# Peilun-Tommy-Li/pHNN-MPC

Measured on AMD Instinct MI355X. Metric: pHNN-MPC rollouts+grads/sec, cartpole H=50 batch=65536, higher is better.
Workload: dtype f32

## Files before the change

### phnn_mpc_amd/csrc/phnn_kernels.hip.h

```cpp
#pragma once
#include <hip/hip_runtime.h>

#include "../../include/phnn_mpc.h"

#define DEV __device__ __forceinline__
#ifdef PHNN_CACHED_TAPE
#define PHNN_NT_STORE(v, p) (*(p) = (v))
#define PHNN_NT_LOAD(p) (*(p))
#else
#define PHNN_NT_STORE(v, p) __builtin_nontemporal_store((v), (p))
#define PHNN_NT_LOAD(p) __builtin_nontemporal_load((p))
#endif

using f32x4 = __attribute__((ext_vector_type(4))) float;
using f32x2 = __attribute__((ext_vector_type(2))) float;

constexpr int kTileB = 16;
#ifndef PHNN_KMAXWAVES
#define PHNN_KMAXWAVES 8
#endif
constexpr int kMaxWaves = PHNN_KMAXWAVES;
constexpr int kScrFloats = 16 * 20;

struct Lane {
// ... 703 lines not shown
  static constexpr int SIZE = oV1T + 4 * LR;
};

constexpr int kRecSmall = 40;
template <int T, int NBIG>
struct WRec {
  static constexpr int VEC = T * 256;
  static constexpr int oSmall = NBIG * VEC;
  static constexpr int SIZE = oSmall + 16 * kRecSmall;
};

#ifdef PHNN_CACHED_RECORDS
#define PHNN_REC_STORE(v, p) (*(p) = (v))
#define PHNN_REC_LOAD(p) (*(p))
#else
#define PHNN_REC_STORE(v, p) __builtin_nontemporal_store((v), (p))
#define PHNN_REC_LOAD(p) __builtin_nontemporal_load((p))
#endif
template <int T>
DEV void store_rec(float* dst, Lane ln, const Act<T>& a) {
#pragma unroll
  for (int t = 0; t < T; ++t) PHNN_REC_STORE(a.v[t], reinterpret_cast<f32x4*>(dst) + t * 64 + ln.lane);
}
template <int T>
DEV void store_rec_scaled(float* dst, Lane ln, const Act<T>& a, float s) {
#pragma unroll
  for (int t = 0; t < T; ++t) PHNN_REC_STORE(a.v[t] * s, reinterpret_cast<f32x4*>(dst) + t * 64 + ln.lane);
}

constexpr int ACT_TANH = 0, ACT_SILU = 2, ACT_RELU = 3, ACT_ELU = 4, ACT_GELU = 5;

DEV float gelu_pdf(float z) { return 0.3989422804014327f * __builtin_amdgcn_exp2f(z * z * -0.7213475204444817f); }
DEV float gelu_cdf(float z) { return __builtin_fmaf(0.5f, erff(z * 0.7071067811865476f), 0.5f); }

template <int ACT>
DEV void act_eval(float z, float& a, float& d1) {
  if (ACT == ACT_RELU) {
    a = fmaxf(z, 0.f);
    d1 = z > 0.f ? 1.0f : 0.0f;
  } else if (ACT == ACT_ELU) {
    a = z > 0.f ? z : expm1f(z);
    d1 = z > 0.f ? 1.0f : __builtin_amdgcn_exp2f(z * 1.4426950408889634f);
  } else if (ACT == ACT_GELU) {
    const float c = gelu_cdf(z);
    a = z * c;
    d1 = __builtin_fmaf(z, gelu_pdf(z), c);
  } else {
    const float s = __builtin_amdgcn_rcpf(1.0f + __builtin_amdgcn_exp2f(z * -1.4426950408889634f));
    a = z * s;
    d1 = __builtin_fmaf(a, 1.0f - s, s);
  }
}
template <int ACT>
DEV float act_d2(float z) {
  if (ACT == ACT_RELU) return 0.0f;
  if (ACT == ACT_ELU) return z > 0.f ? 0.0f : __builtin_amdgcn_exp2f(z * 1.4426950408889634f);
  if (ACT == ACT_GELU) return gelu_pdf(z) * fmaxf(__builtin_fmaf(-z, z, 2.0f), -3.0e38f);
  const float s = __builtin_amdgcn_rcpf(1.0f + __builtin_amdgcn_exp2f(z * -1.4426950408889634f));
  return s * (1.0f - s) * __builtin_fmaf(z, 1.0f - 2.0f * s, 2.0f);
}
template <int ACT, int T>
DEV void act_of(const Act<T>& z, Act<T>& a) {
#pragma unroll
  for (int t = 0; t < T; ++t)
#pragma unroll
    for (int r = 0; r < 4; ++r) {
      float av, d;
      act_eval<ACT>(z.v[t][r], av, d);
      a.v[t][r] = av;
    }
}
template <int ACT, int T>
DEV void mul_d1(Act<T>& g, const Act<T>& z) {
#pragma unroll
  for (int t = 0; t < T; ++t)
#pragma unroll
    for (int r = 0; r < 4; ++r) {
      float a, d;
      act_eval<ACT>(z.v[t][r], a, d);
      g.v[t][r] *= d;
    }
}

template <int HID>
struct HTape {
  Act<HID / 16> a1, a2, q1;
};

template <int HID, bool WANT_H, int ACT>
DEV f32x4 hnet_grad_g(const float* L, Lane ln, f32x4 x, HTape<HID>& tp, float& Hval) {
  using Y = LayH2<HID, MM_F32>;
  constexpr int T = Y::T;
  load_vec<T>(tp.a1, L + Y::oB1, ln);
  in_layer<T>(tp.a1, L + Y::oW1f, ln, sel4(x, ln.q));
  {
    Act<T> a;
    act_of<ACT, T>(tp.a1, a);
    load_vec<T>(tp.a2, L + Y::oB2, ln);
    sq_fwd<T, T>(tp.a2, L + Y::oW2, ln, a);
  }
  Act<T> g;
  float s = 0.f;
  keep_lds_reads_local();
#pragma unroll
  for (int t = 0; t < T; ++t) {
    f32x4 w3 = *reinterpret_cast<const f32x4*>(L + Y::oW3 + 16 * t + 4 * ln.q);
#pragma unroll
    for (int r = 0; r < 4; ++r) {
      float a, d;
      act_eval<ACT>(tp.a2.v[t][r], a, d);
      if (WANT_H) s = __builtin_fmaf(w3[r], a, s);
      g.v[t][r] = w3[r] * d;
    }
  }
  if (WANT_H) Hval = reduce_q(s) + L[Y::oB3];
  zero_act<T>(tp.q1);
  sq_bwd<T, T>(tp.q1, L + Y::oW2, ln, g);
#pragma unroll
  for (int t = 0; t < T; ++t) g.v[t] = tp.q1.v[t];
  mul_d1<ACT, T>(g, tp.a1);
  return to4_rep<T>(L + Y::oW1T, ln, g);
}
template <int HID, int ACT>
DEV void hnet_layer1_g(const float* L, Lane ln, f32x4 x, Act<HID / 16>& z1) {
  using Y = LayH2<HID, MM_F32>;
  load_vec<Y::T>(z1, L + Y::oB1, ln);
  in_layer<Y::T>(z1, L + Y::oW1f, ln, sel4(x, ln.q));
}
template <int HID, int ACT>
DEV f32x4 hnet_hvp_g(const float* L, Lane ln, HTape<HID>& tp, f32x4 v) {
  using Y = LayH2<HID, MM_F32>;
  constexpr int T = Y::T;
  Act<T> ad1, w;
  zero_act<T>(ad1);
  in_layer<T>(ad1, L + Y::oW1f, ln, sel4(v, ln.q));
#pragma unroll
  for (int t = 0; t < T; ++t)
#pragma unroll
    for (int r = 0; r < 4; ++r) {
      const float z = tp.a1.v[t][r], zd = ad1.v[t][r];
      float a, d;
      act_eval<ACT>(z, a, d);
      tp.q1.v[t][r] = tp.q1.v[t][r] * (act_d2<ACT>(z) * zd);
      ad1.v[t][r] = d * zd;
    }
  zero_act<T>(w);
  sq_fwd<T, T>(w, L + Y::oW2, ln, ad1);
  keep_lds_reads_local();
#pragma unroll
  for (int t = 0; t < T; ++t) {
    f32x4 w3 = *reinterpret_cast<const f32x4*>(L + Y::oW3 + 16 * t + 4 * ln.q);
#pragma unroll
    for (int r = 0; r < 4; ++r) w.v[t][r] = w3[r] * (act_d2<ACT>(tp.a2.v[t][r]) * w.v[t][r]);
  }
  Act<T> qd;
  zero_act<T>(qd);
  sq_bwd<T, T>(qd, L + Y::oW2, ln, w);
  mul_d1<ACT, T>(qd, tp.a1);
#pragma unroll
  for (int t = 0; t < T; ++t) qd.v[t] = qd.v[t] + tp.q1.v[t];
  return to4_rep<T>(L + Y::oW1T, ln, qd);
}

template <int HID, bool WANT_H, int MM = MM_F32, int SITE = kInHFwd, int ACT = ACT_TANH>
DEV f32x4 hnet_grad(const float* L, Lane ln, f32x4 z, HTape<HID>& tp, float& Hval) {
  if constexpr (ACT != ACT_TANH) {
    static_assert(MM == MM_F32, "SiLU / ReLU run on the all-f32 kernels");
    return hnet_grad_g<HID, WANT_H, ACT>(L, ln, z, tp, Hval);
  }
  using Y = LayH2<HID, MM>;
  constexpr int T = Y::T;
  load_vec<T>(tp.a1, L + Y::oB1, ln);
  in_layer_mm<T, MM, SITE>(tp.a1, L, Y::oW1f, Y::oW1h, ln, z);
  tanh_act_pre<T>(tp.a1);
  load_vec<T>(tp.a2, L + Y::oB2, ln);
  if (MM == MM_BF16X3) {
    Split3<T> sp;
    split_act<T>(tp.a1, sp);
    sq_fwd_bf<T>(tp.a2, L + Y::oW2, ln, sp);
  } else if (MM == MM_F16X2) {
    Split2<T> sp;
    split_act_h<T>(tp.a1, sp);
    sq_fwd_h<T>(tp.a2, L + Y::oW2, ln, sp);
  } else {
    sq_fwd<T, T>(tp.a2, L + Y::oW2, ln, tp.a1);
  }
  if (MM == MM_F16X2 || kPreScaled<T>) {
    const float c = L[Y::oB3 + 1];
    if (kPreScaled<T> && c == 1.0f) {
      tanh_act_pre<T>(tp.a2);
    } else {
#pragma unroll
      for (int t = 0; t < T; ++t)
#pragma unroll
        for (int r = 0; r < 4; ++r) tp.a2.v[t][r] = tanh_scaled(tp.a2.v[t][r], c);
    }
  } else {
    tanh_act<T>(tp.a2);
  }
  Act<T> g;
  float s = 0.f;
  keep_lds_reads_local();
#pragma unroll
  for (int t = 0; t < T; ++t) {
    if (WANT_H) {
      f32x4 w3 = *reinterpret_cast<const f32x4*>(L + Y::oW3 + 16 * t + 4 * ln.q);
#pragma unroll
      for (int r = 0; r < 4; ++r) s = __builtin_fmaf(w3[r], tp.a2.v[t][r], s);
    }
    f32x4 w3b = *reinterpret_cast<const f32x4*>(L + Y::oW3B + 16 * t + 4 * ln.q);
    g.v[t] = w3b * dtanh(tp.a2.v[t]);
  }
  if (WANT_H) Hval = reduce_q(s) + L[Y::oB3];
  zero_act<T>(tp.q1);
  if (MM == MM_BF16X3) {
    Split3<T> sp;
    split_act<T>(g, sp);
    sq_bwd_bf<T>(tp.q1, L + Y::oW2, ln, sp);
  } else if (MM == MM_F16X2) {
    Split2<T> sp;
    split_act_h<T>(g, sp);
    sq_bwd_h<T>(tp.q1, L + Y::oW2, ln, sp);
  } else {
    sq_bwd<T, T>(tp.q1, L + Y::oW2, ln, g);
  }
#pragma unroll
  for (int t = 0; t < T; ++t) g.v[t] = tp.q1.v[t] * dtanh(tp.a1.v[t]);
  return to4_rep<T>(L + Y::oW1T, ln, g);
}

template <int HID, int MM, int ACT = ACT_TANH>
DEV void hnet_layer1(const float* L, Lane ln, f32x4 z, Act<HID / 16>& a1) {
  if constexpr (ACT != ACT_TANH) return hnet_layer1_g<HID, ACT>(L, ln, z, a1);
  using Y = LayH2<HID, MM>;
  load_vec<Y::T>(a1, L + Y::oB1, ln);
  in_layer_mm<Y::T, MM, kInHRecomp>(a1, L, Y::oW1f, Y::oW1h, ln, z);
  tanh_act_pre<Y::T>(a1);
}

template <int HID, int MM = MM_F32, bool WG = false, int ACT = ACT_TANH, int SITE = kInHHvp>
DEV f32x4 hnet_hvp(const float* L, Lane ln, HTape<HID>& tp, f32x4 v, float* rec = nullptr) {
  if constexpr (ACT != ACT_TANH) {
    static_assert(!WG, "weight-gradient kernels exist for Tanh models only");
    return hnet_hvp_g<HID, ACT>(L, ln, tp, v);
  }
  using Y = LayH2<HID, MM>;
  constexpr int T = Y::T;
  float unscale = 1.0f;
  if (MM == MM_F16X2) {
    float mx = fmaxf(fmaxf(__builtin_fabsf(v[0]), __builtin_fabsf(v[1])), fmaxf(__builtin_fabsf(v[2]), __builtin_fabsf(v[3])));
    int e = 0;
    (void)__builtin_frexpf(mx, &e);
    e = (mx > 0.f && mx < 3.0e38f) ? e : 0;
    v = v * __builtin_ldexpf(1.0f, -e);
    unscale = __builtin_ldexpf(1.0f, e);
  }
  Act<T> ad1, w;
  zero_act<T>(ad1);
  in_layer_mm<T, MM, SITE>(ad1, L, Y::oW1f, Y::oW1h, ln, v);
#pragma unroll
  for (int t = 0; t < T; ++t) ad1.v[t] = dtanh(tp.a1.v[t]) * ad1.v[t];
#pragma unroll
  for (int t = 0; t < T; ++t) tp.q1.v[t] = tp.q1.v[t] * (tp.a1.v[t] * ad1.v[t]);
  zero_act<T>(w);
  if (MM == MM_BF16X3) {
    Split3<T> sp;
    split_act<T>(ad1, sp);
    sq_fwd_bf<T>(w, L + Y::oW2, ln, sp);
  } else if (MM == MM_F16X2) {
    Split2<T> sp;
    split_act_h<T>(ad1, sp);
    sq_fwd_h<T>(w, L + Y::oW2, ln, sp);
  } else {
    sq_fwd<T, T>(w, L + Y::oW2, ln, ad1);
  }
  keep_lds_reads_local();
#pragma unroll
  for (int t = 0; t < T; ++t) {
    f32x4 w3 = *reinterpret_cast<const f32x4*>(L + Y::oW3S + 16 * t + 4 * ln.q);
    f32x4 a2 = tp.a2.v[t];
    f32x4 ad2 = dtanh(a2) * w.v[t];
    if (WG) PHNN_REC_STORE(ad2 * unscale, reinterpret_cast<f32x4*>(rec + 2 * T * 256) + t * 64 + ln.lane);
    w.v[t] = w3 * (a2 * ad2);
  }
  Act<T> qd;
  zero_act<T>(qd);
  if (MM == MM_BF16X3) {
    Split3<T> sp;
    split_act<T>(w, sp);
    sq_bwd_bf<T>(qd, L + Y::oW2, ln, sp);
  } else if (MM == MM_F16X2) {
    Split2<T> sp;
    split_act_h<T>(w, sp);
    sq_bwd_h<T>(qd, L + Y::oW2, ln, sp);
  } else {
    sq_bwd<T, T>(qd, L + Y::oW2, ln, w);
  }
  if (WG) store_rec_scaled<T>(rec + 3 * T * 256, ln, qd, unscale);
#pragma unroll
  for (int t = 0; t < T; ++t) {
    qd.v[t] = __builtin_elementwise_fma(qd.v[t], dtanh(tp.a1.v[t]), tp.q1.v[t]);
  }
  f32x4 Hv = to4_rep<T>(L + Y::oW1T, ln, qd);
  return Hv * (-2.0f * unscale * L[Y::oB3 + 2]);
}

template <int HID, int MM>
DEV f32x4 h1_out_hf(const float* L, Lane ln, const Split2<HID / 16>& sp) {
  using Y = LayH1<HID, MM>;
  constexpr int T = Y::T;
  keep_lds_reads_local();
  const char* base = reinterpret_cast<const char*>(L + Y::oV2) + ln.i * (Y::RS * 2) + ln.q * 16;
  f32x4 o0 = splat4(0.f), o1 = splat4(0.f), o2 = splat4(0.f);
#pragma unroll
  for (int s = 0; s < T / 2; ++s) {
    f16x8 ah = *reinterpret_cast<const f16x8*>(base + s * 64);
    f16x8 al = *reinterpret_cast<const f16x8*>(base + Y::FPART + s * 64);
    o0 = mfma_h(al, sp.h[s], o0);
    o1 = mfma_h(ah, sp.l[s], o1);
    o2 = mfma_h(ah, sp.h[s], o2);
  }
  const float inv = L[Y::oSc];
  f32x4 c2 = *reinterpret_cast<const f32x4*>(L + Y::oC2 + 4 * ln.q);
  return ((o0 + o1) + o2) * inv + c2;
}

template <int HID, int MM>
DEV void h1_bwd_operands(const float* L, Lane ln, const float (&obar)[16], f16x8& b1, f16x8& b2, float& unscale) {
  using Y = LayH1<HID, MM>;
  float mx = 0.f;
#pragma unroll
  for (int k = 0; k < 16; ++k) mx = fmaxf(mx, __builtin_fabsf(obar[k]));
  int e = 0;
  (void)__builtin_frexpf(mx, &e);
  e = (mx > 0.f && mx < 3.0e38f) ? e : 0;
  const float sc = __builtin_ldexpf(1.0f, -e);
  unscale = __builtin_ldexpf(1.0f, e) * L[Y::oSc];
  const bool second = (ln.q & 1) != 0, lo_half = ln.q >= 2;
  u32x4 B1, B2;
#pragma unroll
  for (int p = 0; p < 4; ++p) {
    f32x2 v = {(second ? obar[8 + 2 * p] : obar[2 * p]) * sc, (second ? obar[9 + 2 * p] : obar[2 * p + 1]) * sc};
    f16x2 hb2 = __builtin_convertvector(v, f16x2);
    f32x2 r = residual_h(hb2, v);
    unsigned hbits = __builtin_bit_cast(unsigned, hb2), lbits = __builtin_bit_cast(unsigned, __builtin_convertvector(r, f16x2));
    B1[p] = lo_half ? lbits : hbits;
    B2[p] = lo_half ? 0u : hbits;
  }
  b1 = __builtin_bit_cast(f16x8, B1);
  b2 = __builtin_bit_cast(f16x8, B2);
}

DEV void store_rf(float* dst, Lane ln, f32x4 o) {
  if (ln.w == 0) PHNN_NT_STORE(o, reinterpret_cast<f32x4*>(dst) + ln.i * 4 + ln.q);
}
DEV void load_rf(const float* src, Lane ln, float (&rf)[16]) {
  const f32x4* p = reinterpret_cast<const f32x4*>(src) + ln.i * 4;
#pragma unroll
  for (int k = 0; k < 4; ++k) {
    f32x4 v = PHNN_NT_LOAD(p + k);
#pragma unroll
    for (int e = 0; e < 4; ++e) rf[4 * k + e] = v[e];
  }
}
template <int HID, int MM = MM_F32, int SITE = kInHNet1, int ACT = ACT_TANH>
DEV void h1_hidden(const float* L, Lane ln, f32x4 x, Act<HID / 16>& h) {
  using Y = LayH1<HID, MM>;
  constexpr int T = Y::T;
  load_vec<T>(h, L + Y::oC1, ln);
  in_layer_mm<T, MM, SITE>(h, L, Y::oV1f, Y::oV1h, ln, x);
  if constexpr (ACT == ACT_TANH) tanh_act_pre<T>(h);
}

template <int HID, int MM = MM_F32, int SITE = kInHNet1, int ACT = ACT_TANH>
DEV void h1_fwd(const float* L, float* scr, Lane ln, f32x4 x, Act<HID / 16>& h, float (&out)[16], float* rf_stash = nullptr) {
  using Y = LayH1<HID, MM>;
  constexpr int T = Y::T;
  load_vec<T>(h, L + Y::oC1, ln);
  in_layer_mm<T, MM, SITE>(h, L, Y::oV1f, Y::oV1h, ln, x);
  if constexpr (ACT != ACT_TANH) {
    static_assert(MM == MM_F32, "SiLU / ReLU run on the all-f32 kernels");
    Act<T> a;
    act_of<ACT, T>(h, a);
    Act<1> og;
    og.v[0] = *reinterpret_cast<const f32x4*>(L + Y::oC2 + 4 * ln.q);
    sq_fwd<1, T>(og, L + Y::oV2, ln, a);
// ... 15 lines not shown
  gather16(scr, ln, o.v[0], out);
}

template <int HID, int MM = MM_F32, bool WG = false, int ACT = ACT_TANH>
DEV f32x4 h1_bwd(const float* L, Lane ln, const Act<HID / 16>& h, const float (&obar)[16], float* rec = nullptr) {
  using Y = LayH1<HID, MM>;
  constexpr int T = Y::T;
  Act<T> hb;
  if constexpr (ACT != ACT_TANH) {
    static_assert(MM == MM_F32 && !WG, "SiLU / ReLU: all-f32 kernels, no weight-gradient records");
    Act<1> ob;
#pragma unroll
    for (int r = 0; r < 4; ++r)
      ob.v[0][r] = ln.q == 0 ? obar[r] : (ln.q == 1 ? obar[4 + r] : (ln.q == 2 ? obar[8 + r] : obar[12 + r]));
    zero_act<T>(hb);
    sq_bwd<T, 1>(hb, L + Y::oV2, ln, ob);
    mul_d1<ACT, T>(hb, h);
    return to4_rep<T>(L + Y::oV1T, ln, hb);
  }
  float unscale = 1.0f;
  if (Y::HF) {
    f16x8 b1, b2;
    h1_bwd_operands<HID, MM>(L, ln, obar, b1, b2, unscale);
    keep_lds_reads_local();
    const char* base = reinterpret_cast<const char*>(L + Y::oV2T) + ln.i * 32 + (ln.q & 1) * 16;
#pragma unroll
    for (int nt = 0; nt < T; ++nt) {
      f16x8 ah = *reinterpret_cast<const f16x8*>(base + nt * 512);
      f16x8 al = *reinterpret_cast<const f16x8*>(base + Y::BPART + nt * 512);
      hb.v[nt] = mfma_h(ah, b1, mfma_h(al, b2, splat4(0.f)));
    }
  } else {
    Act<1> ob;
#pragma unroll
    for (int r = 0; r < 4; ++r)
      ob.v[0][r] = ln.q == 0 ? obar[r] : (ln.q == 1 ? obar[4 + r] : (ln.q == 2 ? obar[8 + r] : obar[12 + r]));
    zero_act<T>(hb);
    sq_bwd<T, 1>(hb, L + Y::oV2, ln, ob);
  }
#pragma unroll
  for (int t = 0; t < T; ++t) hb.v[t] = hb.v[t] * dtanh(h.v[t]);
  if (WG) store_rec_scaled<T>(rec, ln, hb, Y::HF ? unscale : 1.0f);
  f32x4 xb = to4_rep<T>(L + Y::oV1T, ln, hb);
  return Y::HF ? xb * unscale : xb;
}

template <int N>
DEV void sym_from_rf(const float (&rf)[16], float (&S)[N][N]) {
#pragma unroll
  for (int i = 0; i < N; ++i) {
    S[i][i] = rf[i * N + i];
#pragma unroll
    for (int j = i + 1; j < N; ++j) S[i][j] = S[j][i] = (rf[i * N + j] + rf[j * N + i]) * 0.5f;
  }
}
template <int N>
DEV void rbar_from(f32x4 lam, f32x4 dH, const float (&Stl)[N], const float (&StdH)[N], float (&rbar)[16]) {
  float m[N][N];
#pragma unroll
  for (int k = 0; k < 16; ++k) rbar[k] = 0.f;
#pragma unroll
  for (int i = 0; i < N; ++i)
#pragma unroll
    for (int j = 0; j < N; ++j) m[i][j] = __builtin_fmaf(lam[i], StdH[j], dH[i] * Stl[j]);
#pragma unroll
  for (int i = 0; i < N; ++i) {
    rbar[i * N + i] = -m[i][i];
#pragma unroll
    for (int j = i + 1; j < N; ++j) rbar[i * N + j] = rbar[j * N + i] = (m[i][j] + m[j][i]) * -0.5f;
  }
}

template <int N_, int HID_, bool FIXG_, int MM_ = MM_F32, int MI_ = 1, int ACT_ = ACT_TANH>
struct PhnnModel {
  static constexpr int N = N_, HID = HID_, T = HID / 16, MM = MM_, MI = MI_, ACT = ACT_;
  static constexpr bool FIXG = FIXG_, SPLIT = false;
  static_assert(N_ * MI_ <= 16 && MI_ <= 4, "G_net output n*m <= 16, m <= 4");
  static constexpr int SCR = kScrFloats;
  static constexpr int oH = 0;
  static constexpr int oR = oH + LayH2<HID, MM>::SIZE;
  static constexpr int oGn = oR + LayH1<HID, MM>::SIZE;
  static constexpr int oJ = oGn + (FIXG ? 0 : LayH1<HID, MM>::SIZE);
  static constexpr int oG = oJ + 16;
  static constexpr int IMG = oG + 16;

  static constexpr int oStashRf = 2 * T * 256 + 64;
  static constexpr int STASH = oStashRf + 256;

  template <bool WANT_H, bool ST = false>
  DEV static f32x4 f(const float* L, float* scr, Lane ln, f32x4 x, f32x4 u, float& Hval, float* stash = nullptr) {
    keep_lds_reads_local();
    HTape<HID> tp;
    f32x4 dH = hnet_grad<HID, WANT_H, MM, kInHFwd, ACT>(L + oH, ln, x, tp, Hval);
    if (ST) {
      store_act<T>(stash, ln, tp.a2);
      store_act<T>(stash + T * 256, ln, tp.q1);
      if (ln.q == 0) PHNN_NT_STORE(dH, reinterpret_cast<f32x4*>(stash + 2 * T * 256) + ln.i);
    }
    Act<T> hR;
    float rf[16];
    h1_fwd<HID, MM, kInHNet1, ACT>(L + oR, scr, ln, x, hR, rf, ST ? stash + oStashRf : nullptr);
    float G[N * MI];
    if (FIXG) {
#pragma unroll
      for (int i = 0; i < N * MI; ++i) G[i] = L[oG + i];
    } else {
      Act<T> hG;
      float gf[16];
      h1_fwd<HID, MM, kInHNet1, ACT>(L + oGn, scr, ln, x, hG, gf);
#pragma unroll
      for (int i = 0; i < N * MI; ++i) G[i] = gf[i];
    }
    return combine(L, rf, dH, G, u);
  }

  DEV static f32x4 combine(const float* L, const float (&rf)[16], f32x4 dH, const float (&G)[N * MI], f32x4 u) {
    float S[N][N], StdH[N];
    sym_from_rf<N>(rf, S);
#pragma unroll
    for (int k = 0; k < N; ++k) {
      float a = 0.f;
#pragma unroll
      for (int i = 0; i < N; ++i) a = __builtin_fmaf(S[i][k], dH[i], a);
      StdH[k] = a;
    }
    f32x4 dx = splat4(0.f);
#pragma unroll
    for (int i = 0; i < N; ++i) {
      float acc = 0.f;
#pragma unroll
      for (int j = 0; j < N; ++j) acc = __builtin_fmaf(L[oJ + i * N + j], dH[j], acc);
#pragma unroll
      for (int k = 0; k < N; ++k) acc = __builtin_fmaf(-S[i][k], StdH[k], acc);
      if (MI == 1) {
        dx[i] = __builtin_fmaf(G[i], u[0], acc);
      } else {
        float gu = 0.f;
#pragma unroll
        for (int k = 0; k < MI; ++k) gu = __builtin_fmaf(G[i * MI + k], u[k], gu);
        dx[i] = acc + gu;
      }
    }
    return dx;
  }

  static constexpr bool RECHB = !LayH1<HID, MM>::HF;
  static constexpr int NBIG = 4 + (RECHB ? (FIXG ? 1 : 2) : 0);
  using Rec = WRec<T, NBIG>;

  template <bool ST = false, bool WG = false, int INH = -1>
  DEV static void vjp(const float* L, float* scr, Lane ln, f32x4 x, f32x4 u, f32x4 lam, f32x4& xbar, f32x4& ubar,
                      const float* stash = nullptr, float* rec = nullptr, float Hbar = 0.f) {
    keep_lds_reads_local();
    HTape<HID> tp;
    float Hdummy;
    f32x4 dH;
    float rf[16];
    if (ST) {
      dH = PHNN_NT_LOAD(reinterpret_cast<const f32x4*>(stash + 2 * T * 256) + ln.i);
      load_rf(stash + oStashRf, ln, rf);
      load_act<T>(stash, ln, tp.a2);
      load_act<T>(stash + T * 256, ln, tp.q1);
    } else {
      dH = hnet_grad<HID, false, MM, INH & kInHRecomp, ACT>(L + oH, ln, x, tp, Hdummy);
    }
    if (WG && !ST) {
      store_rec<T>(rec, ln, tp.a2);
      store_rec<T>(rec + Rec::VEC, ln, tp.q1);
    }
    f32x4 xb = splat4(0.f);
    float S[N][N], Stl[N], StdH[N];
    {
      Act<T> hR;
      if (ST) {
        h1_hidden<HID, MM, INH & kInHNet1Adj, ACT>(L + oR, ln, x, hR);
      } else {
        h1_fwd<HID, MM, INH & kInHNet1Adj, ACT>(L + oR, scr, ln, x, hR, rf);
      }
      sym_from_rf<N>(rf, S);
#pragma unroll
      for (int k = 0; k < N; ++k) {
        float a = 0.f, c = 0.f;
#pragma unroll
        for (int i = 0; i < N; ++i) {
          a = __builtin_fmaf(S[i][k], lam[i], a);
          c = __builtin_fmaf(S[i][k], dH[i], c);
        }
        Stl[k] = a;
        StdH[k] = c;
      }
      float rbar[16];
      rbar_from<N>(lam, dH, Stl, StdH, rbar);
      xb += h1_bwd<HID, MM, WG && RECHB, ACT>(L + oR, ln, hR, rbar, WG && RECHB ? rec + 4 * Rec::VEC : nullptr);
      if (WG && ln.q == 0) {
        f32x4* sm = reinterpret_cast<f32x4*>(rec + Rec::oSmall + ln.i * kRecSmall);
#pragma unroll
        for (int k = 0; k < 4; ++k) sm[4 + k] = f32x4{rbar[4 * k], rbar[4 * k + 1], rbar[4 * k + 2], rbar[4 * k + 3]};
      }
    }
    ubar = splat4(0.f);
    if (FIXG) {
#pragma unroll
      for (int k = 0; k < MI; ++k)
#pragma unroll
        for (int i = 0; i < N; ++i) ubar[k] = __builtin_fmaf(L[oG + i * MI + k], lam[i], ubar[k]);
    } else {
      Act<T> hG;
      float gf[16], gbar[16];
      h1_fwd<HID, MM, INH & kInHNet1Adj, ACT>(L + oGn, scr, ln, x, hG, gf);
#pragma unroll
      for (int k = 0; k < 16; ++k) gbar[k] = 0.f;
#pragma unroll
      for (int i = 0; i < N; ++i)
#pragma unroll
        for (int k = 0; k < MI; ++k) {
          ubar[k] = __builtin_fmaf(gf[i * MI + k], lam[i], ubar[k]);
          gbar[i * MI + k] = lam[i] * u[k];
        }
      xb += h1_bwd<HID, MM, WG && RECHB, ACT>(L + oGn, ln, hG, gbar, WG && RECHB ? rec + 5 * Rec::VEC : nullptr);
    }
    f32x4 v = splat4(0.f);
#pragma unroll
    for (int j = 0; j < N; ++j) {
      float acc = 0.f;
#pragma unroll
      for (int i = 0; i < N; ++i) acc = __builtin_fmaf(L[oJ + i * N + j], lam[i], acc);
#pragma unroll
      for (int k = 0; k < N; ++k) acc = __builtin_fmaf(-S[j][k], Stl[k], acc);
      v[j] = acc;
    }
    if (WG && ln.q == 0) {
      f32x4* sm = reinterpret_cast<f32x4*>(rec + Rec::oSmall + ln.i * kRecSmall);
      sm[0] = x;
      sm[1] = v;
      sm[2] = lam;
      sm[3] = dH;
      sm[8] = u;
      sm[9] = f32x4{Hbar, 0.f, 0.f, 0.f};
    }
    if (ST) hnet_layer1<HID, MM, ACT>(L + oH, ln, x, tp.a1);
    xbar = xb + hnet_hvp<HID, MM, WG, ACT, INH & kInHHvp>(L + oH, ln, tp, v, rec);
    if (WG) xbar = xbar + Hbar * dH;
  }
};

struct LayM {
  static constexpr int HID = 64, T = 4, LD = HID + 4, LR = HID + 8;
  static constexpr int oW1f = 0;
  static constexpr int oB1 = oW1f + T * 64;
  static constexpr int oW2 = oB1 + HID;
  static constexpr int oB2 = oW2 + HID * LD;
  static constexpr int oWo = oB2 + HID;
  static constexpr int oBo = oWo + 4 * LR;
  static constexpr int oWoTf = oBo + 4;
  static constexpr int oW1T = oWoTf + T * 64;
  static constexpr int SIZE = oW1T + 4 * LR;
};

struct MTape {
  Act<4> a1, a2;
  f32x4 o;
};

DEV void mnet_fwd(const float* L, Lane ln, f32x4 q, MTape& tp) {
  using Y = LayM;
  keep_lds_reads_local();
  load_vec<4>(tp.a1, L + Y::oB1, ln);
  in_layer<4>(tp.a1, L + Y::oW1f, ln, sel4(q, ln.q));
  tanh_act<4>(tp.a1);
  load_vec<4>(tp.a2, L + Y::oB2, ln);
  sq_fwd<4, 4>(tp.a2, L + Y::oW2, ln, tp.a1);
  tanh_act<4>(tp.a2);
  tp.o = to4_rep<4>(L + Y::oWo, ln, tp.a2) + *reinterpret_cast<const f32x4*>(L + Y::oBo);
}

DEV f32x4 mnet_bwd(const float* L, Lane ln, const MTape& tp, f32x4 ob) {
  using Y = LayM;
  keep_lds_reads_local();
  Act<4> d, e;
  zero_act<4>(d);
  in_layer<4>(d, L + Y::oWoTf, ln, sel4(ob, ln.q));
#pragma unroll
  for (int t = 0; t < 4; ++t) d.v[t] = d.v[t] * dtanh(tp.a2.v[t]);
  zero_act<4>(e);
  sq_bwd<4, 4>(e, L + Y::oW2, ln, d);
#pragma unroll
  for (int t = 0; t < 4; ++t) e.v[t] = e.v[t] * dtanh(tp.a1.v[t]);
  return to4_rep<4>(L + Y::oW1T, ln, e);
}

DEV float softplus_dev(float x) { return x > 20.f ? x : log1pf(expf(x)); }
DEV float sigmoid_sp_dev(float x) { return x > 20.f ? 1.0f : 1.0f / (1.0f + expf(-x)); }

constexpr int MASS_CARTPOLE = 0, MASS_CONSTANT = 1, MASS_DIAGONAL = 2, MASS_FULL = 3;

template <int MT>
DEV void mass_from_outputs(f32x4 o, float (&m)[3], float (&w)[3]) {
  if (MT == MASS_DIAGONAL) {
    m[0] = expf(o[0]) + 1e-3f;
    m[2] = expf(o[1]) + 1e-3f;
    m[1] = 0.f;
    w[0] = 1.0f / m[0];
    w[2] = 1.0f / m[2];
    w[1] = 0.f;
  } else {
    const float l00 = softplus_dev(o[0]) + 1e-3f, l10 = o[1], l11 = softplus_dev(o[2]) + 1e-3f;
    m[0] = l00 * l00;
    m[1] = l00 * l10;
    m[2] = l10 * l10 + l11 * l11;
    const float det = m[0] * m[2] - m[1] * m[1];
    w[0] = m[2] / det;
    w[1] = -m[1] / det;
    w[2] = m[0] / det;
  }
}

template <int MT>
DEV f32x4 mass_outputs_bar(f32x4 o, const float (&Mb)[4]) {
  if (MT == MASS_DIAGONAL) return f32x4{Mb[0] * expf(o[0]), Mb[3] * expf(o[1]), 0.f, 0.f};
  const float l00 = softplus_dev(o[0]) + 1e-3f, l10 = o[1], l11 = softplus_dev(o[2]) + 1e-3f;
  const float s00 = 2.0f * Mb[0], s01 = Mb[1] + Mb[2], s11 = 2.0f * Mb[3];
  return f32x4{(s00 * l00 + s01 * l10) * sigmoid_sp_dev(o[0]), s01 * l00 + s11 * l10, (s11 * l11) * sigmoid_sp_dev(o[2]), 0.f};
}

template <int HID_, int MM_ = MM_F32, int MI_ = 1, int MT_ = MASS_CARTPOLE, int ACT_ = ACT_TANH>
struct CanonModel {
  static constexpr int N = 4, HID = HID_, T = HID / 16, MM = MM_, MI = MI_, MT = MT_, ACT = ACT_;
  static constexpr bool SPLIT = false;
  static constexpr int SCR = 0;
  static constexpr int oH = 0;
  static constexpr int oC = oH + LayH2<HID, MM>::SIZE;
  static constexpr int oCG = oC + 12;
  static constexpr int oCW = oC + 28;
  static constexpr int oMn = oC + 32;
  static constexpr int IMG = oMn + (MT_ >= MASS_DIAGONAL ? LayM::SIZE : 0);

  DEV static void mass_eval(const float* L, Lane ln, f32x4 y, float (&m)[3], float (&w)[3], MTape& mt) {
    if (MT == MASS_CONSTANT) {
      m[0] = L[oC + 0]; m[1] = L[oC + 1]; m[2] = L[oC + 2];
      w[0] = L[oCW + 0]; w[1] = L[oCW + 1]; w[2] = L[oCW + 2];
    } else {
      mnet_fwd(L + oMn, ln, f32x4{y[0], y[1], 0.f, 0.f}, mt);
      mass_from_outputs<MT>(mt.o, m, w);
    }
  }

  DEV static float Base_Gu(const float* L, int row, f32x4 u) {
    float s = 0.f;
#pragma unroll
    for (int k = 0; k < MI; ++k) s = __builtin_fmaf(L[oCG + row * MI + k], u[k], s);
    return s;
  }
  DEV static f32x4 Base_Gt(const float* L, float dpb0, float dpb1) {
    f32x4 ub = splat4(0.f);
#pragma unroll
    for (int k = 0; k < MI; ++k) ub[k] = L[oCG + 2 * MI + k] * dpb0 + L[oCG + 3 * MI + k] * dpb1;
    return ub;
  }

  static constexpr int STASH = 2 * T * 256 + 64;

  template <bool WANT_H, bool ST = false>
  DEV static f32x4 f(const float* L, float* scr, Lane ln, f32x4 y, f32x4 u, float& Hval, float* stash = nullptr) {
    keep_lds_reads_local();
    if constexpr (MT != MASS_CARTPOLE) {
      float m[3], w[3];
      MTape mt;
      mass_eval(L, ln, y, m, w, mt);
      f32x4 z = {y[0], y[1], m[0] * y[2] + m[1] * y[3], m[1] * y[2] + m[2] * y[3]};
      HTape<HID> tp;
      f32x4 dH = hnet_grad<HID, WANT_H, MM, kInHFwd, ACT>(L + oH, ln, z, tp, Hval);
      if (ST) {
        store_act<T>(stash, ln, tp.a2);
        store_act<T>(stash + T * 256, ln, tp.q1);
        if (ln.q == 0) PHNN_NT_STORE(dH, reinterpret_cast<f32x4*>(stash + 2 * T * 256) + ln.i);
      }
      float dp0 = (-dH[0] - L[oC + 6] * dH[2]) + Base_Gu(L, 2, u);
      float dp1 = (-dH[1] - L[oC + 7] * dH[3]) + Base_Gu(L, 3, u);
      return f32x4{w[0] * z[2] + w[1] * z[3], w[1] * z[2] + w[2] * z[3], w[0] * dp0 + w[1] * dp1, w[1] * dp0 + w[2] * dp1};
    }
    float a = L[oC + 0], b = L[oC + 1], c = L[oC + 2];
    float sn, cs;
    sincos_dev(y[1], sn, cs);
    float bc = b * cs;
    f32x4 z = {y[0], y[1], a * y[2] + bc * y[3], bc * y[2] + c * y[3]};
    HTape<HID> tp;
    f32x4 dH = hnet_grad<HID, WANT_H, MM, kInHFwd, ACT>(L + oH, ln, z, tp, Hval);
    if (ST) {
      store_act<T>(stash, ln, tp.a2);
      store_act<T>(stash + T * 256, ln, tp.q1);
      if (ln.q == 0) PHNN_NT_STORE(dH, reinterpret_cast<f32x4*>(stash + 2 * T * 256) + ln.i);
    }
    float dp0 = (-dH[0] - L[oC + 6] * dH[2]) + Base_Gu(L, 2, u);
    float dp1 = (-dH[1] - L[oC + 7] * dH[3]) + Base_Gu(L, 3, u);
    float det = (a * c - bc * bc) + 1e-6f;
    float mi00 = c / det, mi01 = -bc / det, mi11 = a / det;
    return f32x4{mi00 * z[2] + mi01 * z[3], mi01 * z[2] + mi11 * z[3], mi00 * dp0 + mi01 * dp1,
                 mi01 * dp0 + mi11 * dp1};
  }

  static constexpr int NBIG = 4;
  using Rec = WRec<T, NBIG>;

  template <bool ST = false, bool WG = false, int INH = -1>
  DEV static void vjp(const float* L, float* scr, Lane ln, f32x4 y, f32x4 u, f32x4 lam, f32x4& ybar, f32x4& ubar,
                      const float* stash = nullptr, float* rec = nullptr, float Hbar = 0.f) {
    keep_lds_reads_local();
    if constexpr (MT != MASS_CARTPOLE) {
      float m[3], w[3];
      MTape mt;
      mass_eval(L, ln, y, m, w, mt);
      f32x4 z = {y[0], y[1], m[0] * y[2] + m[1] * y[3], m[1] * y[2] + m[2] * y[3]};
      HTape<HID> tp;
      float Hdummy;
      f32x4 dH;
      if (ST) {
        dH = PHNN_NT_LOAD(reinterpret_cast<const f32x4*>(stash + 2 * T * 256) + ln.i);
        load_act<T>(stash, ln, tp.a2);
        load_act<T>(stash + T * 256, ln, tp.q1);
        hnet_layer1<HID, MM, ACT>(L + oH, ln, z, tp.a1);
      } else {
        dH = hnet_grad<HID, false, MM, INH & kInHRecomp, ACT>(L + oH, ln, z, tp, Hdummy);
      }
      const float Rd2 = L[oC + 6], Rd3 = L[oC + 7];
      const float dp0 = (-dH[0] - Rd2 * dH[2]) + Base_Gu(L, 2, u);
      const float dp1 = (-dH[1] - Rd3 * dH[3]) + Base_Gu(L, 3, u);
      const float pb0 = lam[0] * w[0] + lam[1] * w[1], pb1 = lam[0] * w[1] + lam[1] * w[2];
      const float dpb0 = lam[2] * w[0] + lam[3] * w[1], dpb1 = lam[2] * w[1] + lam[3] * w[2];
      f32x4 v = {-dpb0, -dpb1, -Rd2 * dpb0, -Rd3 * dpb1};
      ubar = Base_Gt(L, dpb0, dpb1);
      if (WG) {
        if (!ST) {
          store_rec<T>(rec, ln, tp.a2);
          store_rec<T>(rec + Rec::VEC, ln, tp.q1);
        }
        if (ln.q == 0) {
          f32x4* sm = reinterpret_cast<f32x4*>(rec + Rec::oSmall + ln.i * kRecSmall);
          sm[0] = z;
          sm[1] = v;
          sm[2] = lam;
          sm[3] = dH;
          sm[4] = f32x4{0.f, 0.f, -dpb0 * dH[2], -dpb1 * dH[3]};
          sm[8] = u;
          sm[9] = f32x4{Hbar, 0.f, 0.f, 0.f};
        }
      }
      f32x4 zb = hnet_hvp<HID, MM, WG, ACT, INH & kInHHvp>(L + oH, ln, tp, v, rec);
      if (WG) zb = zb + Hbar * dH;
      zb[2] += pb0;
      zb[3] += pb1;
      ybar = f32x4{zb[0], zb[1], zb[2] * m[0] + zb[3] * m[1], zb[2] * m[1] + zb[3] * m[2]};
      if (MT >= MASS_DIAGONAL || WG) {
        const float W4[4] = {w[0], w[1], w[1], w[2]};
        const float Wb[4] = {lam[0] * z[2] + lam[2] * dp0, lam[0] * z[3] + lam[2] * dp1,
                             lam[1] * z[2] + lam[3] * dp0, lam[1] * z[3] + lam[3] * dp1};
        float Tm[4], Um[4], Mb[4];
        Tm[0] = W4[0] * Wb[0] + W4[1] * Wb[2]; Tm[1] = W4[0] * Wb[1] + W4[1] * Wb[3];
        Tm[2] = W4[2] * Wb[0] + W4[3] * Wb[2]; Tm[3] = W4[2] * Wb[1] + W4[3] * Wb[3];
        Um[0] = Tm[0] * W4[0] + Tm[1] * W4[2]; Um[1] = Tm[0] * W4[1] + Tm[1] * W4[3];
        Um[2] = Tm[2] * W4[0] + Tm[3] * W4[2]; Um[3] = Tm[2] * W4[1] + Tm[3] * W4[3];
        Mb[0] = zb[2] * y[2] - Um[0];
        Mb[1] = zb[2] * y[3] - Um[1];
        Mb[2] = zb[3] * y[2] - Um[2];
        Mb[3] = zb[3] * y[3] - Um[3];
        if (WG && ln.q == 0) {
          f32x4* sm = reinterpret_cast<f32x4*>(rec + Rec::oSmall + ln.i * kRecSmall);
          sm[5] = f32x4{Mb[0], Mb[1], Mb[2], Mb[3]};
          sm[6] = f32x4{y[0], y[1], 0.f, 0.f};
        }
        if (MT >= MASS_DIAGONAL) {
          f32x4 qb = mnet_bwd(L + oMn, ln, mt, mass_outputs_bar<MT>(mt.o, Mb));
          ybar[0] += qb[0];
          ybar[1] += qb[1];
        }
      }
      return;
    }
    float a = L[oC + 0], b = L[oC + 1], c = L[oC + 2];
    float sn, cs;
    sincos_dev(y[1], sn, cs);
    float bc = b * cs;
    f32x4 z = {y[0], y[1], a * y[2] + bc * y[3], bc * y[2] + c * y[3]};
    HTape<HID> tp;
    float Hdummy;
    f32x4 dH;
    if (ST) {
      dH = PHNN_NT_LOAD(reinterpret_cast<const f32x4*>(stash + 2 * T * 256) + ln.i);
      load_act<T>(stash, ln, tp.a2);
      load_act<T>(stash + T * 256, ln, tp.q1);
      hnet_layer1<HID, MM, ACT>(L + oH, ln, z, tp.a1);
    } else {
      dH = hnet_grad<HID, false, MM, INH & kInHRecomp, ACT>(L + oH, ln, z, tp, Hdummy);
    }
    float Rd2 = L[oC + 6], Rd3 = L[oC + 7];
    float dp0 = (-dH[0] - Rd2 * dH[2]) + Base_Gu(L, 2, u);
    float dp1 = (-dH[1] - Rd3 * dH[3]) + Base_Gu(L, 3, u);
    float det = (a * c - bc * bc) + 1e-6f;
    float rdet = 1.0f / det;
    float mi00 = c * rdet, mi01 = -bc * rdet, mi11 = a * rdet;
    float pb0 = lam[0] * mi00 + lam[1] * mi01, pb1 = lam[0] * mi01 + lam[1] * mi11;
    float dpb0 = lam[2] * mi00 + lam[3] * mi01, dpb1 = lam[2] * mi01 + lam[3] * mi11;
    float mb00 = lam[0] * z[2] + lam[2] * dp0;
    float mb01 = lam[0] * z[3] + lam[1] * z[2] + lam[2] * dp1 + lam[3] * dp0;
    float mb11 = lam[1] * z[3] + lam[3] * dp1;
    f32x4 v = {-dpb0, -dpb1, -Rd2 * dpb0, -Rd3 * dpb1};
    ubar = Base_Gt(L, dpb0, dpb1);
    if (WG) {
      if (!ST) {
        store_rec<T>(rec, ln, tp.a2);
        store_rec<T>(rec + Rec::VEC, ln, tp.q1);
      }
      if (ln.q == 0) {
        f32x4* sm = reinterpret_cast<f32x4*>(rec + Rec::oSmall + ln.i * kRecSmall);
        sm[0] = z;
        sm[1] = v;
        sm[2] = lam;
        sm[3] = dH;
        sm[4] = f32x4{0.f, 0.f, -dpb0 * dH[2], -dpb1 * dH[3]};
        sm[8] = u;
        sm[9] = f32x4{Hbar, 0.f, 0.f, 0.f};
      }
    }
    f32x4 zb = hnet_hvp<HID, MM, WG, ACT, INH & kInHHvp>(L + oH, ln, tp, v, rec);
    if (WG) zb = zb + Hbar * dH;
    zb[2] += pb0;
    zb[3] += pb1;
    float bcb = zb[2] * y[3] + zb[3] * y[2];
    float detb = (-(mb00 * c + mb11 * a) + mb01 * bc) * (rdet * rdet);
    bcb += -mb01 * rdet;
    bcb += -2.0f * bc * detb;
    ybar = f32x4{zb[0], zb[1] + bcb * (-b * sn), zb[2] * a + zb[3] * bc, zb[2] * bc + zb[3] * c};
  }
};

constexpr int kXR0 = 0, kXR1 = 2048, kXR2 = 4096, kXP0 = 6144, kXP1 = 7168, kXchFloats = 8192;
using ActW = Act<2>;

DEV void xch_put(float* region, Lane ln, const Split2<2>& sp) {
  f16x8* p = reinterpret_cast<f16x8*>(region);
  p[ln.w * 64 + ln.lane] = sp.h[0];
  p[(4 + ln.w) * 64 + ln.lane] = sp.l[0];
}
DEV void xch_get(const float* region, Lane ln, Split2<8>& o) {
  const f16x8* p = reinterpret_cast<const f16x8*>(region);
#pragma unroll
  for (int s = 0; s < 4; ++s) {
    o.h[s] = p[s * 64 + ln.lane];
    o.l[s] = p[(4 + s) * 64 + ln.lane];
  }
}
DEV void xch_put_partial(float* set, Lane ln, f32x4 v) { reinterpret_cast<f32x4*>(set)[ln.w * 64 + ln.lane] = v; }
DEV f32x4 xch_sum_partials(const float* set, Lane ln) {
  const f32x4* p = reinterpret_cast<const f32x4*>(set) + ln.lane;
  return to4_kslots(((p[0] + p[64]) + p[128]) + p[192]);
}

DEV void tanh_pre_w(ActW& a) {
#pragma unroll
  for (int t = 0; t < 2; ++t)
#pragma unroll
    for (int r = 0; r < 4; ++r) a.v[t][r] = __builtin_fmaf(-2.0f, __builtin_amdgcn_rcpf(__builtin_amdgcn_exp2f(a.v[t][r]) + 1.0f), 1.0f);
}

DEV void sq_fwd_h_w(ActW& o, const float* Wimg, Lane ln, const Split2<8>& in) {
  using I = HfImg<128>;
  keep_lds_reads_local();
  matrix_phase_begin();
  const char* base = reinterpret_cast<const char*>(Wimg) + ln.i * (I::RS * 2) + ln.q * 16 + (2 * ln.w) * 16 * (I::RS * 2);
#pragma unroll
  for (int s = 0; s < 4; ++s) {
    f16x8 a[2][2];
#pragma unroll
    for (int g = 0; g < 2; ++g)
#pragma unroll
      for (int p = 0; p < 2; ++p) a[g][p] = *reinterpret_cast<const f16x8*>(base + p * I::PART + g * 16 * (I::RS * 2) + s * 64);
    mfma3x2(o.v[0], o.v[1], a, in.h[s], in.l[s]);
  }
  matrix_phase_end();
}

DEV void sq_bwd_h_w(ActW& o, const float* Wimg, Lane ln, const Split2<8>& in) {
  using I = HfImg<128>;
  keep_lds_reads_local();
  matrix_phase_begin();
  typedef fp16x4_t __attribute__((address_space(3))) * lds_h4;
  typedef char __attribute__((address_space(3))) * lds_cp;
  const int a4 = (ln.lane & 15) >> 2, pp = ln.lane & 3;
  lds_cp base = (lds_cp) const_cast<char*>(reinterpret_cast<const char*>(Wimg)) + (4 * ln.q + a4) * (I::RS * 2) + 16 * pp + 64 * ln.w;
#pragma unroll
  for (int s = 0; s < 4; ++s) {
    f16x8 a[2][2];
#pragma unroll
    for (int g = 0; g < 2; ++g)
#pragma unroll
      for (int p = 0; p < 2; ++p) {
        lds_cp off = base + p * I::PART + 32 * s * (I::RS * 2) + 8 * g;
        f16x4 lo = __builtin_bit_cast(f16x4, __builtin_amdgcn_ds_read_tr16_b64_v4f16((lds_h4)off));
        f16x4 hi = __builtin_bit_cast(f16x4, __builtin_amdgcn_ds_read_tr16_b64_v4f16((lds_h4)(off + 16 * (I::RS * 2))));
        a[g][p] = __builtin_shufflevector(lo, hi, 0, 1, 2, 3, 4, 5, 6, 7);
      }
    mfma3x2(o.v[0], o.v[1], a, in.h[s], in.l[s]);
  }
  matrix_phase_end();
}

struct HTapeW {
  ActW a1, a2, q1;
};

template <int SITE = kInHFwd, class PreBarrier>
DEV f32x4 hnet_grad_w(const float* L, Lane ln, f32x4 z, HTapeW& tp, PreBarrier pre_barrier) {
  using Y = LayH2<128, MM_F16X2>;
  const int t0 = 2 * ln.w;
  load_vec<2>(tp.a1, L + Y::oB1 + 16 * t0, ln);
  in_layer_mm<2, MM_F16X2, SITE>(tp.a1, L, Y::oW1f, Y::oW1h, ln, z, t0);
  tanh_pre_w(tp.a1);
  {
    Split2<2> sp;
    split_act_h<2>(tp.a1, sp);
    xch_put(ln.xch + kXR0, ln, sp);
  }
  pre_barrier();
  __syncthreads();
  {
    Split2<8> all;
    xch_get(ln.xch + kXR0, ln, all);
    load_vec<2>(tp.a2, L + Y::oB2 + 16 * t0, ln);
    sq_fwd_h_w(tp.a2, L + Y::oW2, ln, all);
  }
  const float c = L[Y::oB3 + 1];
  if (c == 1.0f) {
    tanh_pre_w(tp.a2);
  } else {
#pragma unroll
    for (int t = 0; t < 2; ++t)
#pragma unroll
      for (int r = 0; r < 4; ++r) tp.a2.v[t][r] = tanh_scaled(tp.a2.v[t][r], c);
  }
  ActW g;
  keep_lds_reads_local();
#pragma unroll
  for (int t = 0; t < 2; ++t) {
    f32x4 w3b = *reinterpret_cast<const f32x4*>(L + Y::oW3B + 16 * (t0 + t) + 4 * ln.q);
    g.v[t] = w3b * dtanh(tp.a2.v[t]);
  }
  {
    Split2<2> sp;
    split_act_h<2>(g, sp);
    xch_put(ln.xch + kXR1, ln, sp);
  }
  __syncthreads();
  {
    Split2<8> all;
    xch_get(ln.xch + kXR1, ln, all);
    zero_act<2>(tp.q1);
    sq_bwd_h_w(tp.q1, L + Y::oW2, ln, all);
  }
#pragma unroll
  for (int t = 0; t < 2; ++t) g.v[t] = tp.q1.v[t] * dtanh(tp.a1.v[t]);
  keep_lds_reads_local();
  return to4_group<2>(L + Y::oW1T + (ln.i & 3) * Y::LR + 16 * t0, ln, g.v);
}

DEV f32x4 hnet_hvp_w(const float* L, Lane ln, HTapeW& tp, f32x4 v, float& scale) {
  using Y = LayH2<128, MM_F16X2>;
  const int t0 = 2 * ln.w;
  float mx = fmaxf(fmaxf(__builtin_fabsf(v[0]), __builtin_fabsf(v[1])), fmaxf(__builtin_fabsf(v[2]), __builtin_fabsf(v[3])));
  int e = 0;
  (void)__builtin_frexpf(mx, &e);
  e = (mx > 0.f && mx < 3.0e38f) ? e : 0;
  v = v * __builtin_ldexpf(1.0f, -e);
  const float unscale = __builtin_ldexpf(1.0f, e);
  ActW ad1, w;
  zero_act<2>(ad1);
  in_layer_mm<2, MM_F16X2, kInHHvp>(ad1, L, Y::oW1f, Y::oW1h, ln, v, t0);
#pragma unroll
  for (int t = 0; t < 2; ++t) ad1.v[t] = dtanh(tp.a1.v[t]) * ad1.v[t];
#pragma unroll
  for (int t = 0; t < 2; ++t) tp.q1.v[t] = tp.q1.v[t] * (tp.a1.v[t] * ad1.v[t]);
  {
    Split2<2> sp;
    split_act_h<2>(ad1, sp);
    xch_put(ln.xch + kXR0, ln, sp);
  }
  __syncthreads();
  {
    Split2<8> all;
    xch_get(ln.xch + kXR0, ln, all);
    zero_act<2>(w);
    sq_fwd_h_w(w, L + Y::oW2, ln, all);
  }
  keep_lds_reads_local();
#pragma unroll
  for (int t = 0; t < 2; ++t) {
    f32x4 w3 = *reinterpret_cast<const f32x4*>(L + Y::oW3S + 16 * (t0 + t) + 4 * ln.q);
    f32x4 a2 = tp.a2.v[t];
    f32x4 ad2 = dtanh(a2) * w.v[t];
    w.v[t] = w3 * (a2 * ad2);
  }
  {
    Split2<2> sp;
    split_act_h<2>(w, sp);
    xch_put(ln.xch + kXR1, ln, sp);
  }
  __syncthreads();
  ActW qd;
  {
    Split2<8> all;
    xch_get(ln.xch + kXR1, ln, all);
    zero_act<2>(qd);
    sq_bwd_h_w(qd, L + Y::oW2, ln, all);
  }
#pragma unroll
  for (int t = 0; t < 2; ++t) qd.v[t] = __builtin_elementwise_fma(qd.v[t], dtanh(tp.a1.v[t]), tp.q1.v[t]);
  scale = -2.0f * unscale * L[Y::oB3 + 2];
  keep_lds_reads_local();
  return to4_group<2>(L + Y::oW1T + (ln.i & 3) * Y::LR + 16 * t0, ln, qd.v);
}

template <int N_>
struct PhnnSplit {
  using Base = PhnnModel<N_, 128, true, MM_F16X2>;
  static constexpr int N = N_, HID = 128, T = 8, MM = MM_F16X2;
  static constexpr bool FIXG = true, SPLIT = true;
  static constexpr int SCR = Base::SCR, IMG = Base::IMG, STASH = Base::STASH, MI = 1;
  static constexpr int oH = Base::oH, oR = Base::oR, oJ = Base::oJ, oG = Base::oG;
  using YR = LayH1<128, MM_F16X2>;

  template <int SITE = kInHNet1>
  DEV static void rnet_hidden(const float* L, Lane ln, f32x4 x, ActW& hR) {
    const int t0 = 2 * ln.w;
    load_vec<2>(hR, L + oR + YR::oC1 + 16 * t0, ln);
    in_layer_mm<2, MM_F16X2, SITE>(hR, L + oR, YR::oV1f, YR::oV1h, ln, x, t0);
    tanh_pre_w(hR);
  }
  template <int SITE = kInHNet1>
  DEV static void rnet_layer1(const float* L, Lane ln, f32x4 x, ActW& hR) {
    rnet_hidden<SITE>(L, ln, x, hR);
    Split2<2> sp;
    split_act_h<2>(hR, sp);
    xch_put(ln.xch + kXR2, ln, sp);
  }
  DEV static void rnet_out(const float* L, float* scr, Lane ln, float (&rf)[16], float* rf_stash = nullptr) {
    Split2<8> all;
    xch_get(ln.xch + kXR2, ln, all);
    f32x4 o = h1_out_hf<128, MM_F16X2>(L + oR, ln, all);
    if (rf_stash) store_rf(rf_stash, ln, o);
    gather16(scr, ln, o, rf);
  }

  template <bool WANT_H, bool ST = false>
  DEV static f32x4 f(const float* L, float* scr, Lane ln, f32x4 x, f32x4 u, float& Hval, float* stash = nullptr) {
    static_assert(!WANT_H, "the split-tile kernels are rollout kernels");
    keep_lds_reads_local();
    HTapeW tp;
    ActW hR;
    f32x4 P = hnet_grad_w(L + oH, ln, x, tp, [&]() { rnet_layer1(L, ln, x, hR); });
    xch_put_partial(ln.xch + kXP0, ln, P);
    float rf[16];
    rnet_out(L, scr, ln, rf, ST ? stash + Base::oStashRf : nullptr);
    if (ST) {
      store_act<2>(stash + 2 * ln.w * 256, ln, tp.a2);
      store_act<2>(stash + T * 256 + 2 * ln.w * 256, ln, tp.q1);
    }
    __syncthreads();
    f32x4 dH = xch_sum_partials(ln.xch + kXP0, ln);
    if (ST && ln.q == 0 && ln.w == 0) PHNN_NT_STORE(dH, reinterpret_cast<f32x4*>(stash + 2 * T * 256) + ln.i);
    float G[N];
#pragma unroll
    for (int i = 0; i < N; ++i) G[i] = L[oG + i];
    return Base::combine(L, rf, dH, G, u);
  }

  template <bool ST = false, bool WG = false, int INH = -1>
  DEV static void vjp(const float* L, float* scr, Lane ln, f32x4 x, f32x4 u, f32x4 lam, f32x4& xbar, f32x4& ubar,
                      const float* stash = nullptr, float* rec = nullptr, float Hbar = 0.f) {
    static_assert(!WG, "weight-gradient records come from the whole-tile kernels");
    keep_lds_reads_local();
    const int t0 = 2 * ln.w;
    HTapeW tp;
    ActW hR;
    f32x4 dH;
    float rf[16];
    if (ST) {
      dH = PHNN_NT_LOAD(reinterpret_cast<const f32x4*>(stash + 2 * T * 256) + ln.i);
      load_rf(stash + Base::oStashRf, ln, rf);
      load_act<2>(stash + t0 * 256, ln, tp.a2);
      load_act<2>(stash + T * 256 + t0 * 256, ln, tp.q1);
      using Y = LayH2<128, MM_F16X2>;
      load_vec<2>(tp.a1, L + oH + Y::oB1 + 16 * t0, ln);
      in_layer_mm<2, MM_F16X2, kInHRecomp>(tp.a1, L + oH, Y::oW1f, Y::oW1h, ln, x, t0);
      tanh_pre_w(tp.a1);
      rnet_hidden<kInHNet1Adj>(L, ln, x, hR);
    } else {
      f32x4 P = hnet_grad_w<kInHRecomp>(L + oH, ln, x, tp, [&]() { rnet_layer1<kInHNet1Adj>(L, ln, x, hR); });
      xch_put_partial(ln.xch + kXP0, ln, P);
      rnet_out(L, scr, ln, rf);
      __syncthreads();
      dH = xch_sum_partials(ln.xch + kXP0, ln);
    }
    float S[N][N], Stl[N], StdH[N];
    sym_from_rf<N>(rf, S);
#pragma unroll
    for (int k = 0; k < N; ++k) {
      float a = 0.f, c = 0.f;
#pragma unroll
      for (int i = 0; i < N; ++i) {
        a = __builtin_fmaf(S[i][k], lam[i], a);
        c = __builtin_fmaf(S[i][k], dH[i], c);
      }
      Stl[k] = a;
      StdH[k] = c;
    }
    float rbar[16];
    rbar_from<N>(lam, dH, Stl, StdH, rbar);
    float unscaleR;
    f32x4 PR;
    {
      f16x8 b1, b2;
      h1_bwd_operands<128, MM_F16X2>(L + oR, ln, rbar, b1, b2, unscaleR);
      keep_lds_reads_local();
      const char* base = reinterpret_cast<const char*>(L + oR + YR::oV2T) + ln.i * 32 + (ln.q & 1) * 16;
      ActW hb;
#pragma unroll
      for (int t = 0; t < 2; ++t) {
        f16x8 ah = *reinterpret_cast<const f16x8*>(base + (t0 + t) * 512);
        f16x8 al = *reinterpret_cast<const f16x8*>(base + YR::BPART + (t0 + t) * 512);
        hb.v[t] = mfma_h(ah, b1, mfma_h(al, b2, splat4(0.f)));
      }
#pragma unroll
      for (int t = 0; t < 2; ++t) hb.v[t] = hb.v[t] * dtanh(hR.v[t]);
      keep_lds_reads_local();
      PR = to4_group<2>(L + oR + YR::oV1T + (ln.i & 3) * YR::LR + 16 * t0, ln, hb.v);
    }
    ubar = splat4(0.f);
#pragma unroll
    for (int i = 0; i < N; ++i) ubar[0] = __builtin_fmaf(L[oG + i], lam[i], ubar[0]);
    f32x4 v = splat4(0.f);
#pragma unroll
    for (int j = 0; j < N; ++j) {
      float acc = 0.f;
#pragma unroll
      for (int i = 0; i < N; ++i) acc = __builtin_fmaf(L[oJ + i * N + j], lam[i], acc);
#pragma unroll
      for (int k = 0; k < N; ++k) acc = __builtin_fmaf(-S[j][k], Stl[k], acc);
      v[j] = acc;
    }
    float scaleH;
    f32x4 PH = hnet_hvp_w(L + oH, ln, tp, v, scaleH);
    xch_put_partial(ln.xch + kXP0, ln, PR);
    xch_put_partial(ln.xch + kXP1, ln, PH);
    __syncthreads();
    f32x4 xb = splat4(0.f);
    xb += xch_sum_partials(ln.xch + kXP0, ln) * unscaleR;
    xbar = xb + xch_sum_partials(ln.xch + kXP1, ln) * scaleH;
  }
};

template <int DUMMY = 0>
struct CanonSplit {
  using Base = CanonModel<128, MM_F16X2>;
  static constexpr int N = 4, HID = 128, T = 8, MM = MM_F16X2;
  static constexpr bool SPLIT = true;
  static constexpr int SCR = 0, IMG = Base::IMG, STASH = Base::STASH, oH = Base::oH, oC = Base::oC, MI = 1;
  DEV static float Base_Gu(const float* L, int row, f32x4 u) { return Base::Base_Gu(L, row, u); }
  DEV static f32x4 Base_Gt(const float* L, float dpb0, float dpb1) { return Base::Base_Gt(L, dpb0, dpb1); }

  template <bool WANT_H, bool ST = false>
  DEV static f32x4 f(const float* L, float* scr, Lane ln, f32x4 y, f32x4 u, float& Hval, float* stash = nullptr) {
    static_assert(!WANT_H, "the split-tile kernels are rollout kernels");
    keep_lds_reads_local();
    float a = L[oC + 0], b = L[oC + 1], c = L[oC + 2];
    float sn, cs;
    sincos_dev(y[1], sn, cs);
    float bc = b * cs;
    f32x4 z = {y[0], y[1], a * y[2] + bc * y[3], bc * y[2] + c * y[3]};
    HTapeW tp;
    f32x4 P = hnet_grad_w(L + oH, ln, z, tp, []() {});
    xch_put_partial(ln.xch + kXP0, ln, P);
    if (ST) {
      store_act<2>(stash + 2 * ln.w * 256, ln, tp.a2);
      store_act<2>(stash + T * 256 + 2 * ln.w * 256, ln, tp.q1);
    }
    __syncthreads();
    f32x4 dH = xch_sum_partials(ln.xch + kXP0, ln);
    if (ST && ln.q == 0 && ln.w == 0) PHNN_NT_STORE(dH, reinterpret_cast<f32x4*>(stash + 2 * T * 256) + ln.i);
    float dp0 = (-dH[0] - L[oC + 6] * dH[2]) + Base_Gu(L, 2, u);
    float dp1 = (-dH[1] - L[oC + 7] * dH[3]) + Base_Gu(L, 3, u);
    float det = (a * c - bc * bc) + 1e-6f;
    float mi00 = c / det, mi01 = -bc / det, mi11 = a / det;
    return f32x4{mi00 * z[2] + mi01 * z[3], mi01 * z[2] + mi11 * z[3], mi00 * dp0 + mi01 * dp1,
                 mi01 * dp0 + mi11 * dp1};
  }

  template <bool ST = false, bool WG = false, int INH = -1>
  DEV static void vjp(const float* L, float* scr, Lane ln, f32x4 y, f32x4 u, f32x4 lam, f32x4& ybar, f32x4& ubar,
                      const float* stash = nullptr, float* rec = nullptr, float Hbar = 0.f) {
    static_assert(!WG, "weight-gradient records come from the whole-tile kernels");
    keep_lds_reads_local();
    const int t0 = 2 * ln.w;
    float a = L[oC + 0], b = L[oC + 1], c = L[oC + 2];
    float sn, cs;
    sincos_dev(y[1], sn, cs);
    float bc = b * cs;
    f32x4 z = {y[0], y[1], a * y[2] + bc * y[3], bc * y[2] + c * y[3]};
    HTapeW tp;
    f32x4 dH;
    if (ST) {
      dH = PHNN_NT_LOAD(reinterpret_cast<const f32x4*>(stash + 2 * T * 256) + ln.i);
      load_act<2>(stash + t0 * 256, ln, tp.a2);
      load_act<2>(stash + T * 256 + t0 * 256, ln, tp.q1);
      using Y = LayH2<128, MM_F16X2>;
      load_vec<2>(tp.a1, L + oH + Y::oB1 + 16 * t0, ln);
      in_layer_mm<2, MM_F16X2, kInHRecomp>(tp.a1, L + oH, Y::oW1f, Y::oW1h, ln, z, t0);
      tanh_pre_w(tp.a1);
    } else {
      f32x4 P = hnet_grad_w<kInHRecomp>(L + oH, ln, z, tp, []() {});
      xch_put_partial(ln.xch + kXP0, ln, P);
      __syncthreads();
      dH = xch_sum_partials(ln.xch + kXP0, ln);
    }
    float Rd2 = L[oC + 6], Rd3 = L[oC + 7];
    float dp0 = (-dH[0] - Rd2 * dH[2]) + Base_Gu(L, 2, u);
    float dp1 = (-dH[1] - Rd3 * dH[3]) + Base_Gu(L, 3, u);
    float det = (a * c - bc * bc) + 1e-6f;
    float rdet = 1.0f / det;
    float mi00 = c * rdet, mi01 = -bc * rdet, mi11 = a * rdet;
    float pb0 = lam[0] * mi00 + lam[1] * mi01, pb1 = lam[0] * mi01 + lam[1] * mi11;
    float dpb0 = lam[2] * mi00 + lam[3] * mi01, dpb1 = lam[2] * mi01 + lam[3] * mi11;
    float mb00 = lam[0] * z[2] + lam[2] * dp0;
    float mb01 = lam[0] * z[3] + lam[1] * z[2] + lam[2] * dp1 + lam[3] * dp0;
    float mb11 = lam[1] * z[3] + lam[3] * dp1;
    f32x4 v = {-dpb0, -dpb1, -Rd2 * dpb0, -Rd3 * dpb1};
    ubar = Base_Gt(L, dpb0, dpb1);
    float scaleH;
    f32x4 PH = hnet_hvp_w(L + oH, ln, tp, v, scaleH);
    xch_put_partial(ln.xch + kXP1, ln, PH);
    __syncthreads();
    f32x4 zb = xch_sum_partials(ln.xch + kXP1, ln) * scaleH;
    zb[2] += pb0;
    zb[3] += pb1;
    float bcb = zb[2] * y[3] + zb[3] * y[2];
    float detb = (-(mb00 * c + mb11 * a) + mb01 * bc) * (rdet * rdet);
    bcb += -mb01 * rdet;
    bcb += -2.0f * bc * detb;
    ybar = f32x4{zb[0], zb[1] + bcb * (-b * sn), zb[2] * a + zb[3] * bc, zb[2] * bc + zb[3] * c};
  }
};

template <int N_, int HID_, int MM_ = MM_F32, int ACT_ = ACT_TANH>
struct OdeModel {
  static constexpr int N = N_, HID = HID_, T = HID / 16, LD = HID + 4, LR = HID + 8, MM = MM_, MI = 1, ACT = ACT_;
  static_assert(ACT_ == ACT_TANH || MM_ == MM_F32, "SiLU / ReLU run on the all-f32 kernels");
  static constexpr bool SPLIT = false;
  static constexpr int SCR = 0;
  static constexpr int WF = MM == MM_F16X2 ? HfImg<HID>::FLOATS : HID * LD;
  static constexpr int oW1f = 0;
  static constexpr int oB1 = oW1f + T * 64;
  static constexpr int oW2 = oB1 + HID;
  static constexpr int oB2 = oW2 + WF;
  static constexpr int oW3 = oB2 + HID;
  static constexpr int oB3 = oW3 + WF;
  static constexpr int oW4r = oB3 + HID;
  static constexpr int oB4 = oW4r + 4 * LR;
  static constexpr int oW4f = oB4 + 4;
  static constexpr int oW1T = oW4f + T * 64;
  static constexpr int oSC = oW1T + 4 * LR;
  static constexpr bool WIDE = N + 1 > 4;
  static constexpr int oW1fu = oSC + 4;
  static constexpr int oW1Tu = oW1fu + (WIDE ? T * 64 : 0);
  static constexpr int IMG = oW1Tu + (WIDE ? 4 * LR : 0);
  static_assert(MM != MM_BF16X3, "ODEFunc has an f32 and an f16x2 variant");
  static_assert(N <= 4, "state dimension up to 4");

  struct Tape {
    Act<T> a1, a2, a3;
  };

  DEV static void layer1(const float* L, Lane ln, f32x4 x, float u, Act<T>& a1) {
    f32x4 in = x;
    if (!WIDE) in[N & 3] = u;
    load_vec<T>(a1, L + oB1, ln);
    in_layer<T>(a1, L + oW1f, ln, sel4(in, ln.q));
    if (WIDE) in_layer<T>(a1, L + oW1fu, ln, ln.q == 0 ? u : 0.f);
    if constexpr (ACT == ACT_TANH) tanh_act<T>(a1);
  }

  DEV static void hidden(const float* L, Lane ln, int oW, int oB, float c, const Act<T>& a, Act<T>& o) {
    load_vec<T>(o, L + oB, ln);
    if constexpr (ACT != ACT_TANH) {
      Act<T> act;
      act_of<ACT, T>(a, act);
      sq_fwd<T, T>(o, L + oW, ln, act);
      return;
    }
    if (MM == MM_F16X2) {
      Split2<T> sp;
      split_act_h<T>(a, sp);
      sq_fwd_h<T>(o, L + oW, ln, sp);
#pragma unroll
      for (int t = 0; t < T; ++t)
#pragma unroll
        for (int r = 0; r < 4; ++r) o.v[t][r] = tanh_scaled(o.v[t][r], c);
    } else {
      sq_fwd<T, T>(o, L + oW, ln, a);
      tanh_act<T>(o);
    }
  }

  DEV static void hidden_T(const float* L, Lane ln, int oW, const Act<T>& d, Act<T>& o) {
    zero_act<T>(o);
    if (MM == MM_F16X2) {
      Split2<T> sp;
      split_act_h<T>(d, sp);
      sq_bwd_h<T>(o, L + oW, ln, sp);
    } else {
      sq_bwd<T, T>(o, L + oW, ln, d);
    }
  }

  DEV static f32x4 fwd(const float* L, Lane ln, f32x4 x, float u, Tape& tp) {
    keep_lds_reads_local();
    layer1(L, ln, x, u, tp.a1);
    hidden(L, ln, oW2, oB2, L[oSC + 0], tp.a1, tp.a2);
    hidden(L, ln, oW3, oB3, L[oSC + 1], tp.a2, tp.a3);
    f32x4 b4 = *reinterpret_cast<const f32x4*>(L + oB4);
    if constexpr (ACT != ACT_TANH) {
      Act<T> act;
      act_of<ACT, T>(tp.a3, act);
      return to4_rep<T>(L + oW4r, ln, act) + b4;
    }
    return to4_rep<T>(L + oW4r, ln, tp.a3) + b4;
  }

  static constexpr int VEC24 = ACT == ACT_TANH ? T * 192 : T * 256;
  static constexpr int STASH = 2 * VEC24;

  template <bool WANT_H, bool ST = false>
  DEV static f32x4 f(const float* L, float* scr, Lane ln, f32x4 x, f32x4 uv, float& Hval, float* stash = nullptr) {
    const float u = uv[0];
    Tape tp;
    if (WANT_H) Hval = 0.f;
    f32x4 dx = fwd(L, ln, x, u, tp);
    if (ST) {
      if constexpr (ACT == ACT_TANH) {
        store_act24<T>(stash, ln, tp.a2);
        store_act24<T>(stash + VEC24, ln, tp.a3);
      } else {
        store_act<T>(stash, ln, tp.a2);
        store_act<T>(stash + VEC24, ln, tp.a3);
      }
    }
    return dx;
  }

  template <bool ST = false, bool WG = false, int INH = -1>
  DEV static void vjp(const float* L, float* scr, Lane ln, f32x4 x, f32x4 uv, f32x4 lam, f32x4& xbar, f32x4& ubar4,
                      const float* stash = nullptr, float* rec = nullptr, float Hbar = 0.f) {
    static_assert(!WG, "ODEFunc has no weight-gradient kernels");
    const float u = uv[0];
    float ubar;
    Tape tp;
    if (ST) {
      if constexpr (ACT == ACT_TANH) {
        load_act24<T>(stash + VEC24, ln, tp.a3);
        load_act24<T>(stash, ln, tp.a2);
      } else {
        load_act<T>(stash + VEC24, ln, tp.a3);
        load_act<T>(stash, ln, tp.a2);
      }
      keep_lds_reads_local();
      layer1(L, ln, x, u, tp.a1);
    } else {
      (void)fwd(L, ln, x, u, tp);
    }
    float unscale = 1.0f;
    if (MM == MM_F16X2) {
      float mx = fmaxf(fmaxf(__builtin_fabsf(lam[0]), __builtin_fabsf(lam[1])), fmaxf(__builtin_fabsf(lam[2]), __builtin_fabsf(lam[3])));
      int e = 0;
      (void)__builtin_frexpf(mx, &e);
      e = (mx > 0.f && mx < 3.0e38f) ? e : 0;
      lam = lam * __builtin_ldexpf(1.0f, -e);
      unscale = __builtin_ldexpf(1.0f, e);
    }
    Act<T> d, e;
    zero_act<T>(d);
    in_layer<T>(d, L + oW4f, ln, sel4(lam, ln.q));
    if constexpr (ACT != ACT_TANH) {
      mul_d1<ACT, T>(d, tp.a3);
      hidden_T(L, ln, oW3, d, e);
      mul_d1<ACT, T>(e, tp.a2);
      hidden_T(L, ln, oW2, e, d);
      mul_d1<ACT, T>(d, tp.a1);
    } else {
#pragma unroll
      for (int t = 0; t < T; ++t) d.v[t] = d.v[t] * dtanh(tp.a3.v[t]);
      hidden_T(L, ln, oW3, d, e);
#pragma unroll
      for (int t = 0; t < T; ++t) e.v[t] = e.v[t] * dtanh(tp.a2.v[t]);
      hidden_T(L, ln, oW2, e, d);
#pragma unroll
      for (int t = 0; t < T; ++t) d.v[t] = d.v[t] * dtanh(tp.a1.v[t]);
    }
    f32x4 inb = to4_rep<T>(L + oW1T, ln, d);
    if (MM == MM_F16X2) inb = inb * unscale;
    if (WIDE) {
      ubar = to4_rep<T>(L + oW1Tu, ln, d)[0] * unscale;
    } else {
      ubar = inb[N & 3];
      inb[N & 3] = 0.f;
    }
    xbar = inb;
    ubar4 = f32x4{ubar, 0.f, 0.f, 0.f};
  }
};

DEV void no_speculation() { asm volatile("" ::: "memory"); }

template <int N, class Tgt>
DEV float state_cost(const phnn_cost& c, f32x4 x, const Tgt& tgt) {
  float e[N], cost = 0.f;
#pragma unroll
// ... 69 lines not shown
  const float* dx_bar;
  float* dx_out;
  float* wrec;
  int no_cost;
  long long B;
  int H;
  float dt, half_dt, sixth_dt;
  phnn_cost c;
  float Qs[16];
  const float* x_ref;
  long long ref_bs, ref_ts;
  int ref_rows;
  const int* ref_off_dev;
  int ref_off_host;
};

struct PointParams {
  const float* img;
  const float* x;
  const float* u;
  const float* lam;
  float* dx;
  float* Hout;
  long long B;
  const float* Hbar;
  float* wrec;
};

template <int IMG>
DEV void stage_image(float* lds, const float* img) {
  const f32x4* src = reinterpret_cast<const f32x4*>(img);
  f32x4* dst = reinterpret_cast<f32x4*>(lds);
  for (int k = threadIdx.x; k < IMG / 4; k += blockDim.x) dst[k] = src[k];
  __syncthreads();
}

template <int N>
DEV f32x4 load_state(const float* p) {
  if (N == 4) return *reinterpret_cast<const f32x4*>(p);
  f32x4 x = splat4(0.f);
#pragma unroll
  for (int i = 0; i < N; ++i) x[i] = p[i];
  return x;
}
template <int N>
DEV void store_state(float* p, f32x4 x) {
  if (N == 4) {
    *reinterpret_cast<f32x4*>(p) = x;
  } else {
#pragma unroll
    for (int i = 0; i < N; ++i) p[i] = x[i];
  }
}

DEV float clamp_u(const phnn_cost& c, float u) { return c.has_u_bounds ? fminf(fmaxf(u, c.u_min), c.u_max) : u; }

template <int MI>
DEV f32x4 load_u(const float* up, int t) {
  f32x4 u = splat4(0.f);
#pragma unroll
  for (int k = 0; k < MI; ++k) u[k] = up[t * MI + k];
  return u;
}
template <int MI>
DEV f32x4 clamp_u4(const phnn_cost& c, f32x4 u) {
#pragma unroll
  for (int k = 0; k < MI; ++k) u[k] = clamp_u(c, u[k]);
  return u;
}
template <int MI>
DEV float control_cost(const phnn_cost& c, f32x4 u) {
  if (MI == 1) return (u[0] * c.R[0]) * u[0];
  float cost = 0.f;
#pragma unroll
  for (int j = 0; j < MI; ++j) {
    float s = 0.f;
#pragma unroll
    for (int i = 0; i < MI; ++i) s = __builtin_fmaf(u[i], c.R[i * MI + j], s);
    cost = __builtin_fmaf(s, u[j], cost);
  }
  return cost;
}

template <class M, int INTEG>
struct StashStep {
  static constexpr int SLOT = M::STASH + 64;
  static constexpr int FLOATS = INTEG == PHNN_INTEG_EULER ? M::STASH : 4 * SLOT;
};
DEV void store_stage(float* dst, Lane ln, f32x4 y) {
  if (ln.q == 0 && ln.w == 0) PHNN_NT_STORE(y, reinterpret_cast<f32x4*>(dst) + ln.i);
}
DEV f32x4 load_stage(const float* src, Lane ln) {
  return PHNN_NT_LOAD(reinterpret_cast<const f32x4*>(src) + ln.i);
}

struct TileCtx {
  Lane ln;
  float* scr;
  long long tile, b;
  bool valid, writer;
};
template <class M>
DEV bool tile_ctx(TileCtx& c, float* lds, long long B) {
  const int wave = threadIdx.x >> 6, nwaves = blockDim.x >> 6;
  static_prio(wave);
  c.ln.lane = threadIdx.x & 63;
  c.ln.i = c.ln.lane & 15;
  c.ln.q = c.ln.lane >> 4;
  c.ln.w = M::SPLIT ? wave : 0;
  c.ln.xch = M::SPLIT ? lds + M::IMG + nwaves * M::SCR : nullptr;
  c.scr = lds + M::IMG + wave * M::SCR;
  c.tile = M::SPLIT ? (long long)blockIdx.x : (long long)blockIdx.x * nwaves + wave;
  if (c.tile * kTileB >= B) return false;
  c.b = c.tile * kTileB + c.ln.i;
  c.valid = c.b < B;
  if (!c.valid) c.b = B - 1;
  c.writer = c.valid && c.ln.q == 0 && (!M::SPLIT || wave == 0);
  return true;
}

template <int N>
struct RefRows {
  const float* base;
  long long ts;
  int off, last;
  DEV void init(const RollParams& p, long long b) {
    base = p.x_ref + b * p.ref_bs;
    ts = p.ref_ts;
    last = p.ref_rows - 1;
    const int o = p.ref_off_dev ? *p.ref_off_dev : p.ref_off_host;
    off = o < 0 ? 0 : (o > last ? last : o);
  }
  DEV f32x4 row(int t) const {
    const int r = t < last - off ? off + t : last;
    const float* q = base + r * ts;
    f32x4 v = splat4(0.f);
#pragma unroll
    for (int i = 0; i < N; ++i) v[i] = q[i];
    return v;
  }
};

template <class M, int INTEG, bool STASH, bool REF = false>
DEV void fwd_march(const RollParams& p, const float* L, const TileCtx& tc) {
  constexpr int N = M::N;
  const Lane ln = tc.ln;
  float* scr = tc.scr;
  const long long tile = tc.tile, b = tc.b;
  const bool writer = tc.writer;
  f32x4 x = load_state<N>(p.x0 + b * N);
  if (p.traj && writer) store_state<N>(p.traj + (b * (p.H + 1)) * N, x);
  RefRows<N> rr;
  float cost;
  if constexpr (REF) {
    rr.init(p, b);
    cost = state_cost<N>(p.c, x, rr.row(0));
  } else {
    cost = state_cost<N>(p.c, x, p.c.x_target);
  }
  constexpr int MI = M::MI;
  const float* up = p.u + b * p.H * MI;
  float Hd;
  for (int t = 0; t < p.H; ++t) {
    f32x4 tgt;
    if constexpr (REF) tgt = rr.row(t + 1);
    f32x4 u = clamp_u4<MI>(p.c, load_u<MI>(up, t));
    if (MI == 1) cost = __builtin_fmaf(u[0] * p.c.R[0], u[0], cost);
    else cost += control_cost<MI>(p.c, u);
    float* sl = STASH ? p.stash + (tile * p.H + t) * (long long)StashStep<M, INTEG>::FLOATS : nullptr;
    f32x4 k1 = M::template f<false, STASH>(L, scr, ln, x, u, Hd, sl);
    if (p.dx_out && writer) store_state<N>(p.dx_out + (b * p.H + t) * N, k1);
    if (INTEG == PHNN_INTEG_EULER) {
      x = x + p.dt * k1;
    } else {
      constexpr int SLOT = StashStep<M, INTEG>::SLOT;
      f32x4 acc = k1, kp = k1;
#pragma unroll 1
      for (int s = 1; s < 4; ++s) {
        const f32x4 y = x + (s == 3 ? p.dt : p.half_dt) * kp;
        float* ss = STASH ? sl + s * SLOT : nullptr;
        if (STASH) store_stage(ss + M::STASH, ln, y);
        kp = M::template f<false, STASH>(L, scr, ln, y, u, Hd, ss);
        acc = acc + (s == 3 ? 1.0f : 2.0f) * kp;
      }
      x = x + p.sixth_dt * acc;
    }
    if constexpr (REF) cost += state_cost<N>(p.c, x, tgt);
    else cost += state_cost<N>(p.c, x, p.c.x_target);
    if (p.traj && writer) store_state<N>(p.traj + (b * (p.H + 1) + t + 1) * N, x);
  }
  if (writer && p.cost) p.cost[b] = cost;
}

template <class M, int INTEG, bool STASH, bool REF = false>
__global__ __launch_bounds__(64 * kMaxWaves) void k_rollout_fwd(RollParams p) {
  extern __shared__ __attribute__((aligned(16))) float lds[];
  stage_image<M::IMG>(lds, p.img);
  TileCtx tc;
  if (!tile_ctx<M>(tc, lds, p.B)) return;
  fwd_march<M, INTEG, STASH, REF>(p, lds, tc);
}

template <class M, int INTEG, bool STASH, bool WG = false, bool REF = false>
DEV void grad_march(const RollParams& p, const float* L, const TileCtx& tc) {
  constexpr int N = M::N;
  const Lane ln = tc.ln;
  float* scr = tc.scr;
  const long long tile = tc.tile, b = tc.b;
  const bool valid = tc.valid, writer = tc.writer;
  const float* tr = p.traj_in + (b * (p.H + 1)) * N;
  constexpr int MI = M::MI;
  const float* up = p.u + b * p.H * MI;
  const float cb = p.no_cost ? 0.0f : (p.cost_bar ? p.cost_bar[b] : 1.0f);
  const float* tb = p.traj_bar ? p.traj_bar + (b * (p.H + 1)) * N : nullptr;
  const float* db = p.dx_bar ? p.dx_bar + (b * p.H) * N : nullptr;
  const float live = valid ? 1.0f : 0.0f;
  RefRows<N> rr;
  f32x4 lam;
  if constexpr (REF) {
    rr.init(p, b);
    lam = cb * state_cost_grad<N>(p.c, p.Qs, load_state<N>(tr + (long long)p.H * N), rr.row(p.H));
  } else {
    lam = cb * state_cost_grad<N>(p.c, p.Qs, load_state<N>(tr + (long long)p.H * N), p.c.x_target);
  }
  if (tb) lam = lam + load_state<N>(tb + (long long)p.H * N);
  if (WG) lam = lam * live;
  constexpr int STAGES = INTEG == PHNN_INTEG_EULER ? 1 : 4;
  float Hd;
  for (int t = p.H - 1; t >= 0; --t) {
    f32x4 x = load_state<N>(tr + (long long)t * N);
    f32x4 tgt;
    if constexpr (REF && INTEG == PHNN_INTEG_EULER) tgt = rr.row(t);
    f32x4 uraw = load_u<MI>(up, t);
    f32x4 u = p.no_cost ? uraw : clamp_u4<MI>(p.c, uraw);
    f32x4 dxb = splat4(0.f);
    if (INTEG == PHNN_INTEG_EULER && db) dxb = load_state<N>(db + (long long)t * N) * live;
    f32x4 xb, ub, utot;
    float* rec = nullptr;
    if constexpr (WG) rec = p.wrec + ((tile * p.H + t) * STAGES) * (long long)M::Rec::SIZE;
    if constexpr (INTEG == PHNN_INTEG_EULER) {
      if constexpr (WG) {
        M::template vjp<STASH, true>(L, scr, ln, x, u, p.dt * lam + dxb, xb, ub,
                                     STASH ? p.stash + (tile * p.H + t) * (long long)M::STASH : nullptr, rec);
      } else {
        M::template vjp<STASH>(L, scr, ln, x, u, p.dt * lam + dxb, xb, ub,
                               STASH ? p.stash + (tile * p.H + t) * (long long)M::STASH : nullptr);
      }
      lam = lam + xb;
      utot = ub;
    } else {
      constexpr int SLOT = StashStep<M, INTEG>::SLOT;
      const float* sl = STASH ? p.stash + (tile * p.H + t) * (long long)StashStep<M, INTEG>::FLOATS : nullptr;
      f32x4 y2 = x, y3 = x, y4 = x;
      if constexpr (!STASH) {
        f32x4 y = x;
#pragma unroll 1
        for (int s = 0; s < 3; ++s) {
          const f32x4 k = M::template f<false>(L, scr, ln, y, u, Hd);
          y = x + (s == 2 ? p.dt : p.half_dt) * k;
          y2 = s == 0 ? y : y2;
          y3 = s == 1 ? y : y3;
          y4 = s == 2 ? y : y4;
        }
      }
      f32x4 ysum = splat4(0.f), ybn = ysum;
      utot = splat4(0.f);
#pragma unroll 1
      for (int s = 3; s >= 0; --s) {
        f32x4 y;
        if constexpr (STASH) y = s == 0 ? load_state<N>(tr + (long long)t * N) : load_stage(sl + s * SLOT + M::STASH, ln);
        else y = s == 0 ? load_state<N>(tr + (long long)t * N) : (s == 1 ? y2 : (s == 2 ? y3 : y4));
        const f32x4 us = p.no_cost ? load_u<MI>(up, t) : clamp_u4<MI>(p.c, load_u<MI>(up, t));
        f32x4 in = ((s == 0 || s == 3) ? p.sixth_dt : 2.0f * p.sixth_dt) * lam;
        if (s != 3) in = in + (s == 2 ? p.dt : p.half_dt) * ybn;
        if (s == 0 && db) in = in + load_state<N>(db + (long long)t * N) * live;
        f32x4 yb;
        if constexpr (WG) M::template vjp<STASH, true>(L, scr, ln, y, us, in, yb, ub, STASH ? sl + s * SLOT : nullptr, rec + s * M::Rec::SIZE);
        else M::template vjp<STASH>(L, scr, ln, y, us, in, yb, ub, STASH ? sl + s * SLOT : nullptr);
        utot = s == 3 ? ub : utot + ub;
        ybn = yb;
        ysum = s == 3 ? yb : ysum + yb;
      }
      lam = lam + ysum;
      x = load_state<N>(tr + (long long)t * N);
      if constexpr (REF) tgt = rr.row(t);
      uraw = load_u<MI>(up, t);
      u = p.no_cost ? uraw : clamp_u4<MI>(p.c, uraw);
    }
    if constexpr (REF) lam = lam + cb * state_cost_grad<N>(p.c, p.Qs, x, tgt);
    else lam = lam + cb * state_cost_grad<N>(p.c, p.Qs, x, p.c.x_target);
    if (tb) lam = lam + load_state<N>(tb + (long long)t * N) * (WG ? live : 1.0f);
#pragma unroll
    for (int k = 0; k < MI; ++k) {
      float g;
      if (MI == 1) {
        g = __builtin_fmaf(cb * (2.0f * p.c.R[0]), u[0], utot[0]);
      } else {
        float s = 0.f;
#pragma unroll
        for (int j = 0; j < MI; ++j) s = __builtin_fmaf(p.c.R[k * MI + j] + p.c.R[j * MI + k], u[j], s);
        g = __builtin_fmaf(cb, s, utot[k]);
      }
      if (!p.no_cost && p.c.has_u_bounds && !(uraw[k] >= p.c.u_min && uraw[k] <= p.c.u_max)) g = 0.f;
      if (writer && p.grad_u) p.grad_u[(b * p.H + t) * MI + k] = g;
    }
  }
  if (p.grad_x0 && writer) store_state<N>(p.grad_x0 + b * N, lam);
}

template <class M, int INTEG, bool STASH, bool WG = false, bool REF = false>
__global__ __launch_bounds__(64 * kMaxWaves) void k_rollout_grad(RollParams p) {
  extern __shared__ __attribute__((aligned(16))) float lds[];
  stage_image<M::IMG>(lds, p.img);
  TileCtx tc;
  if (!tile_ctx<M>(tc, lds, p.B)) return;
  grad_march<M, INTEG, STASH, WG, REF>(p, lds, tc);
}


template <class M>
__global__ __launch_bounds__(64 * kMaxWaves) void k_model_forward(PointParams p) {
  extern __shared__ __attribute__((aligned(16))) float lds[];
  constexpr int N = M::N;
  stage_image<M::IMG>(lds, p.img);
  const int wave = threadIdx.x >> 6, nwaves = blockDim.x >> 6;
  Lane ln;
  ln.lane = threadIdx.x & 63;
  ln.i = ln.lane & 15;
  ln.q = ln.lane >> 4;
  ln.w = 0;
  ln.xch = nullptr;
  float* scr = lds + M::IMG + wave * M::SCR;
  const long long ntiles = (p.B + kTileB - 1) / kTileB;
  for (long long tile = (long long)blockIdx.x * nwaves + wave; tile < ntiles; tile += (long long)gridDim.x * nwaves) {
    long long b = tile * kTileB + ln.i;
    const bool valid = b < p.B;
    if (!valid) b = p.B - 1;
    f32x4 x = load_state<N>(p.x + b * N);
    float Hval = 0.f;
    f32x4 dx = M::template f<true>(lds, scr, ln, x, load_u<M::MI>(p.u + b * M::MI, 0), Hval);
    if (valid && ln.q == 0) {
      store_state<N>(p.dx + b * N, dx);
      if (p.Hout) p.Hout[b] = Hval;
    }
  }
}

template <class M, bool WG = false>
__global__ __launch_bounds__(64 * kMaxWaves) void k_model_vjp(PointParams p) {
  extern __shared__ __attribute__((aligned(16))) float lds[];
  constexpr int N = M::N;
  stage_image<M::IMG>(lds, p.img);
  const int wave = threadIdx.x >> 6, nwaves = blockDim.x >> 6;
// ... 580 lines not shown
```

### phnn_mpc_amd/csrc/phnn_mpc.hip

```cpp
#include <hip/hip_runtime.h>

#include <algorithm>
#include <cmath>
#include <cstdio>
#include <cstdint>
#include <cstdlib>
#include <cstring>
#include <string>
#include <vector>

#define PHNN_PREFETCH_BF
#include "phnn_lbfgs.h"
#include "phnn_mppi.h"
#include "phnn_cem.h"
#include "phnn_pack.h"

namespace {

thread_local std::string g_create_error;

struct KernelSet {
  RollTable fwd, grad;
  int stash_floats[2];
  int scr_floats;
  void (*mfwd)(PointParams);
  void (*mvjp)(PointParams);
  int img_floats;
  const char* name;
};

template <class M>
KernelSet make_set(const char* name) {
  KernelSet k;
  fill_fwd<M>(k.fwd);
  k.stash_floats[0] = StashStep<M, PHNN_INTEG_EULER>::FLOATS;
  k.stash_floats[1] = StashStep<M, PHNN_INTEG_RK4>::FLOATS;
  k.scr_floats = M::SCR;
  k.mfwd = k_model_forward<M>;
  k.img_floats = M::IMG;
  k.name = name;
  return k;
}

bool kernel_set(int v, KernelSet* k) {
  GradSet g;
  if (!phnn_grad_kernels(v, &g)) return false;
  switch (v) {
#define PHNN_CASE(V, M, NAME) \
  case V: *k = make_set<M>(NAME); break;
    PHNN_FOR_EACH_VARIANT(PHNN_CASE)
#undef PHNN_CASE
    default: return false;
  }
  memcpy(k->grad, g.grad, sizeof k->grad);
  k->mvjp = g.mvjp;
  return true;
}

size_t mlp_count(const phnn_mlp_shape& s, int in, int out) {
  if (s.depth < 1 || s.depth > PHNN_MAX_LAYERS) return 0;
  size_t c = 0;
  int last = in;
  for (int l = 0; l <= s.depth; ++l) {
    int o = l < s.depth ? s.hidden[l] : out;
    if (o < 1) return 0;
    c += (size_t)o * last + o;
    last = o;
  }
  return c;
}

size_t mass_block_count(const phnn_desc* d) {
  switch (d->mass_type) {
    case PHNN_MASS_CARTPOLE: return 3;
    case PHNN_MASS_CONSTANT: return 4;
    case PHNN_MASS_DIAGONAL: return mlp_count(d->m_net, 2, 2);
    case PHNN_MASS_FULL: return mlp_count(d->m_net, 2, 3);
    default: return 0;
  }
}

size_t weight_count(const phnn_desc* d) {
  if (!d || d->n < 1 || d->n > PHNN_MAX_N || d->m < 1 || d->m > PHNN_MAX_M) return 0;
  int n = d->n, m = d->m;
  if (d->kind == PHNN_MODEL_PHNN) {
    size_t h = mlp_count(d->h_net, n, 1), r = mlp_count(d->r_net, n, n * n);
    size_t g = d->fixed_G ? (size_t)n * m : mlp_count(d->g_net, n, n * m);
    if (!h || !r || !g) return 0;
    return (size_t)n * n + h + r + g;
  }
  if (d->kind == PHNN_MODEL_CANONICAL) {
    size_t h = mlp_count(d->h_net, n, 1);
    if (!h || n != 4) return 0;
    size_t mass = mass_block_count(d);
    if (!mass) return 0;
    return (size_t)n + (size_t)n * m + mass + h;
  }
  if (d->kind == PHNN_MODEL_ODEFUNC) return mlp_count(d->h_net, n + m, n);
  return 0;
}

bool same_hidden(const phnn_mlp_shape& s, int depth, int hid) {
  if (s.depth != depth) return false;
  for (int l = 0; l < depth; ++l)
    if (s.hidden[l] != hid) return false;
  return true;
}

int matmul_mode(const phnn_options& o, int hid) {
  const int dflt = hid >= 128 ? MM_F16X2 : MM_F32;
  switch (o.matmul_mode) {
    case PHNN_MATMUL_F32: return MM_F32;
    case PHNN_MATMUL_BF16X3: return MM_BF16X3;
    case PHNN_MATMUL_F16X2: return MM_F16X2;
    default: return dflt;
  }
}

int pick_variant(const phnn_desc* d, const phnn_options& opt, std::string* why) {
// ... 246 lines not shown
  }
}

bool pad_source_map(const phnn_desc* d, std::vector<int>* map) {
  const size_t n = weight_count(d);
  if (n == 0 || n >= (1u << 24)) return false;
  std::vector<float> probe(n), padded;
  for (size_t k = 0; k < n; ++k) probe[k] = (float)(k + 1);
  phnn_desc pd;
  std::string why;
  if (!pad_model(d, probe.data(), &pd, &padded, &why)) return false;
  const float* src = padded.empty() ? probe.data() : padded.data();
  const size_t np = padded.empty() ? n : padded.size();
  map->resize(np);
  for (size_t k = 0; k < np; ++k) (*map)[k] = src[k] > 0.f ? (int)src[k] - 1 : -1;
  return true;
}

}

struct phnn_handle {
  phnn_desc desc;
  phnn_desc pdesc;
  phnn_options opt;
  int device;
  int variant;
  KernelSet ks;
  WgradSet wg;
  bool has_wgrad;
  SplitSet sp;
  bool has_split;
  int* d_unpad;
  int* d_padsrc;
  float* d_pblob;
  int n_pad;
  int n_params;
  float* d_img;
  float* h_img;
  hipEvent_t up_done;
  size_t img_floats;
  int n_cu;
  int max_waves;
  std::string err;
};

namespace {

int fail(phnn_handle* h, int code, const std::string& msg) {
  if (h) h->err = msg;
  else g_create_error = msg;
  return code;
}

int hip_fail(phnn_handle* h, hipError_t e, const char* what) {
  return fail(h, PHNN_ERR_HIP, std::string(what) + ": " + hipGetErrorString(e));
}

int pick_waves(long long tiles, int n_cu, int max_waves) {
  int w = (max_waves >= 1 && max_waves <= kMaxWaves) ? max_waves : kMaxWaves;
  while (w > 1 && (tiles + w - 1) / w < n_cu) w >>= 1;
  return w;
}

template <class P>
int launch(phnn_handle* h, void (*kern)(P), const P& p, long long tiles, bool grid_stride, hipStream_t st) {
  int waves = pick_waves(tiles, h->n_cu, h->max_waves);
  long long grid = (tiles + waves - 1) / waves;
  if (grid_stride && grid > 4LL * h->n_cu) grid = 4LL * h->n_cu;
  if (grid < 1) grid = 1;
  size_t shmem = sizeof(float) * ((size_t)h->ks.img_floats + (size_t)waves * h->ks.scr_floats);
  if (shmem > 160 * 1024) return fail(h, PHNN_ERR_UNSUPPORTED, "weight image does not fit the 160 KiB of LDS");
  hipLaunchKernelGGL(kern, dim3((unsigned)grid), dim3(64 * waves), shmem, st, p);
  hipError_t e = hipGetLastError();
  if (e != hipSuccess) return hip_fail(h, e, "kernel launch");
  return PHNN_OK;
}

bool use_split(const phnn_handle* h, long long tiles) {
  if (!h->has_split || h->opt.split_tiles == 1) return false;
  return h->opt.split_tiles == 2 || tiles <= 2LL * h->n_cu;
}

int launch_roll(phnn_handle* h, bool grad, bool ref, bool stash, int integrator, const RollParams& p, long long tiles,
                hipStream_t st) {
  if (!use_split(h, tiles)) return launch(h, (grad ? h->ks.grad : h->ks.fwd)[ref][stash][integrator], p, tiles, false, st);
  RollKernel kern = (grad ? h->sp.grad : h->sp.fwd)[ref][stash][integrator];
  hipLaunchKernelGGL(kern, dim3((unsigned)tiles), dim3(256), sizeof(float) * (size_t)h->sp.lds_floats, st, p);
  hipError_t e = hipGetLastError();
  if (e != hipSuccess) return hip_fail(h, e, "kernel launch (split-tile)");
  return PHNN_OK;
}

struct DeviceGuard {
  int prev = -1, rc = PHNN_OK;
  bool switched = false;
  DeviceGuard(phnn_handle* h, int device) {
    hipError_t e = hipGetDevice(&prev);
    if (e != hipSuccess) { rc = hip_fail(h, e, "hipGetDevice"); return; }
    if (prev != device) {
      e = hipSetDevice(device);
      if (e != hipSuccess) { rc = hip_fail(h, e, "hipSetDevice"); return; }
      switched = true;
    }
  }
  ~DeviceGuard() {
    if (switched) (void)hipSetDevice(prev);
  }
};
#define PHNN_ON_DEVICE(h)            \
  DeviceGuard guard_((h), (h)->device); \
  if (guard_.rc) return guard_.rc

template <class P>
hipError_t allow_big_lds(void (*kern)(P)) {
  if (!kern) return hipSuccess;
  return hipFuncSetAttribute(reinterpret_cast<const void*>(kern), hipFuncAttributeMaxDynamicSharedMemorySize, 160 * 1024);
}

int check_cost(phnn_handle* h, const phnn_cost* c) {
  if (!c) return fail(h, PHNN_ERR_INVALID_ARG, "cost is NULL");
  if (c->has_u_bounds && !(c->u_min <= c->u_max)) return fail(h, PHNN_ERR_INVALID_ARG, "u_min > u_max");
  return PHNN_OK;
}

}

extern "C" {

int phnn_version(void) { return 260; }

const char* phnn_variant_name(const phnn_handle* h) { return h ? h->ks.name : ""; }

size_t phnn_weight_count(const phnn_desc* desc) { return weight_count(desc); }

const char* phnn_last_error(const phnn_handle* h) { return h ? h->err.c_str() : g_create_error.c_str(); }

int phnn_create(const phnn_desc* desc, const float* weights_host, size_t n_floats, int device, phnn_handle** out) {
  return phnn_create_ex(desc, weights_host, n_floats, device, nullptr, out);
}

static int build_image(const phnn_desc* desc, const float* weights_host, size_t n_floats, const phnn_options& opt,
                       phnn_desc* pdesc, int* variant, std::vector<float>* img, std::string* why, int* code) {
  size_t need = weight_count(desc);
  *code = PHNN_ERR_INVALID_ARG;
  if (need == 0) { *why = "invalid model description"; return 1; }
  if (need != n_floats) {
    char buf[128];
    snprintf(buf, sizeof buf, "weight blob has %zu floats, description needs %zu", n_floats, need);
    *why = buf;
    return 1;
  }
  *code = PHNN_ERR_UNSUPPORTED;
  std::vector<float> pblob;
  if (!pad_model(desc, weights_host, pdesc, &pblob, why)) return 1;
  int v = pick_variant(pdesc, opt, why);
  if (v == V_NONE) return 1;
  *variant = v;
  pack_image(v, *img, pdesc, pblob.data());
  *code = PHNN_OK;
  return 0;
}

int phnn_create_ex(const phnn_desc* desc, const float* weights_host, size_t n_floats, int device,
                   const phnn_options* opt_in, phnn_handle** out) {
  if (!desc || !weights_host || !out) return fail(nullptr, PHNN_ERR_INVALID_ARG, "NULL argument");
  *out = nullptr;
  phnn_options opt;
  memset(&opt, 0, sizeof opt);
  if (opt_in) opt = *opt_in;
  if (opt.matmul_mode < PHNN_MATMUL_DEFAULT || opt.matmul_mode > PHNN_MATMUL_F16X2 || opt.max_waves < 0 ||
      opt.max_waves > kMaxWaves || opt.split_tiles < 0 || opt.split_tiles > 2)
    return fail(nullptr, PHNN_ERR_INVALID_ARG, "phnn_options: matmul_mode, max_waves or split_tiles out of range");
  std::string why;
  phnn_desc pdesc;
  std::vector<float> img;
  int v = V_NONE, code = PHNN_OK;
  if (build_image(desc, weights_host, n_floats, opt, &pdesc, &v, &img, &why, &code)) return fail(nullptr, code, why);
  int ndev = 0;
  hipError_t e = hipGetDeviceCount(&ndev);
  if (e != hipSuccess || ndev == 0)
    return fail(nullptr, PHNN_ERR_HIP, "no HIP device available (the rollout engine has no CPU fallback)");
  if (device < 0 || device >= ndev) return fail(nullptr, PHNN_ERR_INVALID_ARG, "device index out of range");
  DeviceGuard guard(nullptr, device);
  if (guard.rc) return guard.rc;
  phnn_handle* h = new phnn_handle();
  h->desc = *desc;
  h->pdesc = pdesc;
  h->opt = opt;
  h->device = device;
  h->variant = v;
  h->max_waves = opt.max_waves > 0 ? opt.max_waves : kMaxWaves;
  h->d_img = nullptr;
  h->h_img = nullptr;
  h->up_done = nullptr;
  h->d_unpad = nullptr;
  h->d_padsrc = nullptr;
  h->d_pblob = nullptr;
  h->n_pad = 0;
  h->n_params = (int)n_floats;
  kernel_set(v, &h->ks);
  h->has_wgrad = phnn_wgrad_kernels(v, &h->wg);
  h->has_split = phnn_split_kernels(v, &h->sp);
  hipDeviceProp_t prop;
  e = hipGetDeviceProperties(&prop, device);
  h->n_cu = (e == hipSuccess && prop.multiProcessorCount > 0) ? prop.multiProcessorCount : 256;
  h->img_floats = img.size();
  if (sizeof(float) * (img.size() + (size_t)kMaxWaves * h->ks.scr_floats) > 160 * 1024) {
    delete h;
    return fail(nullptr, PHNN_ERR_UNSUPPORTED, "weight image does not fit the 160 KiB of LDS");
  }
  e = hipSuccess;
  RollKernel* tables[] = {&h->ks.fwd[0][0][0], &h->ks.grad[0][0][0], h->has_split ? &h->sp.fwd[0][0][0] : nullptr,
                          h->has_split ? &h->sp.grad[0][0][0] : nullptr};
  for (RollKernel* t : tables)
    for (int i = 0; t && i < 8; ++i)
      if (e == hipSuccess) e = allow_big_lds(t[i]);
  if (e == hipSuccess) e = allow_big_lds(h->ks.mfwd);
  if (e == hipSuccess) e = allow_big_lds(h->ks.mvjp);
  if (h->has_wgrad) {
    if (e == hipSuccess) e = allow_big_lds(h->wg.grad[0]);
    if (e == hipSuccess) e = allow_big_lds(h->wg.grad[1]);
    if (e == hipSuccess) e = allow_big_lds(h->wg.mvjp);
    if (e == hipSuccess) e = allow_big_lds(h->wg.reduce);
    if (e == hipSuccess) e = allow_big_lds(h->wg.grad_t[0]);
    if (e == hipSuccess) e = allow_big_lds(h->wg.grad_t[1]);
    if (e == hipSuccess) e = allow_big_lds(h->wg.reduce_t);
  }
  if (h->has_split && (size_t)h->sp.lds_floats * sizeof(float) > 160 * 1024) h->has_split = false;
  if (e != hipSuccess) {
    delete h;
    return hip_fail(nullptr, e, "hipFuncSetAttribute(MaxDynamicSharedMemorySize)");
  }
  e = hipMalloc(reinterpret_cast<void**>(&h->d_img), sizeof(float) * img.size());
  if (e != hipSuccess) {
    delete h;
    return hip_fail(nullptr, e, "hipMalloc(weights image)");
  }
  e = hipHostMalloc(reinterpret_cast<void**>(&h->h_img), sizeof(float) * img.size(), hipHostMallocDefault);
  if (e == hipSuccess) {
    memcpy(h->h_img, img.data(), sizeof(float) * img.size());
    e = hipMemcpy(h->d_img, h->h_img, sizeof(float) * img.size(), hipMemcpyHostToDevice);
  }
  if (e == hipSuccess && h->has_wgrad) {
    std::vector<int> map = unpad_map(desc, &pdesc);
    e = hipMalloc(reinterpret_cast<void**>(&h->d_unpad), sizeof(int) * map.size());
    if (e == hipSuccess) e = hipMemcpy(h->d_unpad, map.data(), sizeof(int) * map.size(), hipMemcpyHostToDevice);
  }
  if (e == hipSuccess) {
    std::vector<int> src;
    if (pad_source_map(desc, &src)) {
      h->n_pad = (int)src.size();
      e = hipMalloc(reinterpret_cast<void**>(&h->d_padsrc), sizeof(int) * src.size());
      if (e == hipSuccess) e = hipMemcpy(h->d_padsrc, src.data(), sizeof(int) * src.size(), hipMemcpyHostToDevice);
      if (e == hipSuccess) e = hipMalloc(reinterpret_cast<void**>(&h->d_pblob), sizeof(float) * src.size());
    }
  }
  if (e != hipSuccess) {
    if (h->h_img) (void)hipHostFree(h->h_img);
    if (h->d_unpad) (void)hipFree(h->d_unpad);
    if (h->d_padsrc) (void)hipFree(h->d_padsrc);
    if (h->d_pblob) (void)hipFree(h->d_pblob);
    (void)hipFree(h->d_img);
    delete h;
    return hip_fail(nullptr, e, "upload of the weights image");
  }
  *out = h;
  return PHNN_OK;
}

int phnn_update_weights(phnn_handle* h, const float* weights_host, size_t n_floats, void* stream) {
  if (!h) return PHNN_ERR_INVALID_ARG;
  if (!weights_host) return fail(h, PHNN_ERR_INVALID_ARG, "weights_host is NULL");
  std::string why;
  phnn_desc pdesc;
  std::vector<float> img;
  int v = V_NONE, code = PHNN_OK;
  if (build_image(&h->desc, weights_host, n_floats, h->opt, &pdesc, &v, &img, &why, &code)) return fail(h, code, why);
  if (v != h->variant || img.size() != h->img_floats) return fail(h, PHNN_ERR_INVALID_ARG, "weights select another kernel variant");
  PHNN_ON_DEVICE(h);
  hipStream_t st = (hipStream_t)stream;
  hipStreamCaptureStatus cap = hipStreamCaptureStatusNone;
  if (hipStreamIsCapturing(st, &cap) == hipSuccess && cap != hipStreamCaptureStatusNone)
    return fail(h, PHNN_ERR_INVALID_ARG, "phnn_update_weights packs on the host and cannot be captured into a graph");
  hipError_t e;
  if (h->up_done) {
    e = hipEventSynchronize(h->up_done);
    if (e != hipSuccess) return hip_fail(h, e, "hipEventSynchronize(previous weight upload)");
  } else {
    e = hipEventCreateWithFlags(&h->up_done, hipEventDisableTiming);
    if (e != hipSuccess) return hip_fail(h, e, "hipEventCreate");
  }
  memcpy(h->h_img, img.data(), sizeof(float) * img.size());
  e = hipMemcpyAsync(h->d_img, h->h_img, sizeof(float) * img.size(), hipMemcpyHostToDevice, st);
  if (e != hipSuccess) return hip_fail(h, e, "hipMemcpyAsync(weights image)");
  e = hipEventRecord(h->up_done, st);
  if (e != hipSuccess) return hip_fail(h, e, "hipEventRecord");
  return PHNN_OK;
}

int phnn_update_weights_dev(phnn_handle* h, const float* weights_dev, size_t n_floats, void* stream) {
  if (!h) return PHNN_ERR_INVALID_ARG;
  if (!weights_dev) return fail(h, PHNN_ERR_INVALID_ARG, "weights_dev is NULL");
  if (n_floats != (size_t)h->n_params) {
    char buf[128];
    snprintf(buf, sizeof buf, "weight blob has %zu floats, the handle's model needs %d", n_floats, h->n_params);
    return fail(h, PHNN_ERR_INVALID_ARG, buf);
  }
  if (!h->d_padsrc || !h->d_pblob) return fail(h, PHNN_ERR_UNSUPPORTED, "no device-side packer for this handle");
  PHNN_ON_DEVICE(h);
// ... 157 lines not shown
  return rollout_vjp(h, x0_dev, u_dev, B, H, cost, integrator, dt, traj_dev, workspace_dev, nullptr, nullptr,
                     grad_u_dev, grad_x0_dev, ref, stream);
}

int phnn_rollout_vjp(phnn_handle* h, const float* x0_dev, const float* u_dev, int64_t B, int32_t H,
                     const phnn_cost* cost, int32_t integrator, float dt, const float* traj_dev,
                     const void* workspace_dev, const float* traj_bar_dev, const float* cost_bar_dev,
                     float* grad_u_dev, float* grad_x0_dev, void* stream) {
  return rollout_vjp(h, x0_dev, u_dev, B, H, cost, integrator, dt, traj_dev, workspace_dev, traj_bar_dev, cost_bar_dev,
                     grad_u_dev, grad_x0_dev, nullptr, stream);
}

static long long wgrad_records(int64_t B, int32_t H, int32_t integrator) {
  long long tiles = (B + kTileB - 1) / kTileB;
  if (H <= 0) return tiles;
  return tiles * (long long)H * (integrator == PHNN_INTEG_RK4 ? 4 : 1);
}
static int wgrad_rows(const phnn_handle* h, long long n_rec) {
  long long rows = n_rec < (long long)h->n_cu ? n_rec : (long long)h->n_cu;
  return (int)(rows < 1 ? 1 : rows);
}

static size_t wgrad_tape_offset(const phnn_handle* h, long long n_rec) {
  size_t o = (size_t)n_rec * (size_t)h->wg.rec_floats + (size_t)wgrad_rows(h, n_rec) * (size_t)h->wg.blob_floats;
  return (o + 63) / 64 * 64;
}
size_t phnn_wgrad_workspace_bytes(const phnn_handle* h, int64_t B, int32_t H, int32_t integrator) {
  if (!h || !h->has_wgrad || B <= 0 || H < 0) return 0;
  if (H > 0 && integrator != PHNN_INTEG_EULER && integrator != PHNN_INTEG_RK4) return 0;
  long long n_rec = wgrad_records(B, H, integrator);
  size_t floats = wgrad_tape_offset(h, n_rec);
  if (H > 0) floats += (size_t)n_rec * (size_t)h->wg.tape_floats[integrator];
  return sizeof(float) * floats;
}

static int wgrad_reduce(phnn_handle* h, void* workspace_dev, long long n_rec, float* grad_theta_dev, int accumulate,
                        hipStream_t st, int tape_floats = 0) {
  float* rec = (float*)workspace_dev;
  float* slab = rec + (size_t)n_rec * (size_t)h->wg.rec_floats;
  const int rows = wgrad_rows(h, n_rec);
  WgradParams wp{h->d_img, rec, n_rec, slab, h->wg.blob_floats, tape_floats ? rec + wgrad_tape_offset(h, n_rec) : nullptr,
                 tape_floats};
  hipLaunchKernelGGL(tape_floats ? h->wg.reduce_t : h->wg.reduce, dim3((unsigned)rows), dim3(64 * h->wg.reduce_waves),
                     (size_t)h->wg.reduce_lds_bytes, st, wp);
  hipError_t e = hipGetLastError();
  if (e != hipSuccess) return hip_fail(h, e, "wgrad reduce launch");
  e = phnn_wgrad_finish(slab, rows, h->wg.blob_floats, h->d_unpad, h->n_params, grad_theta_dev, accumulate, st);
  if (e != hipSuccess) return hip_fail(h, e, "wgrad finish launch");
  return PHNN_OK;
}

int phnn_wgrad_record_info(const phnn_handle* h, int32_t* record_floats, int32_t* small_offset, int32_t* small_stride) {
  if (!h || !h->has_wgrad) return PHNN_ERR_UNSUPPORTED;
  if (record_floats) *record_floats = h->wg.rec_floats;
  if (small_offset) *small_offset = h->wg.rec_floats - kTileB * kRecSmall;
  if (small_stride) *small_stride = kRecSmall;
  return PHNN_OK;
}

int phnn_rollout_trajectory(phnn_handle* h, const float* x0_dev, const float* u_dev, int64_t B, int32_t H,
                            int32_t integrator, float dt, float* traj_dev, float* dx_dev, void* stream) {
  return phnn_rollout_trajectory_ws(h, x0_dev, u_dev, B, H, integrator, dt, traj_dev, dx_dev, nullptr, stream);
}

int phnn_rollout_trajectory_ws(phnn_handle* h, const float* x0_dev, const float* u_dev, int64_t B, int32_t H,
                               int32_t integrator, float dt, float* traj_dev, float* dx_dev, void* wgrad_workspace_dev,
                               void* stream) {
  if (!h) return PHNN_ERR_INVALID_ARG;
  if (wgrad_workspace_dev && !h->has_wgrad)
    return fail(h, PHNN_ERR_UNSUPPORTED, "no weight-gradient kernels for this model variant: pass a NULL workspace");
  phnn_cost neutral;
  memset(&neutral, 0, sizeof neutral);
  RollParams p;
  if (int rc = fill_roll(h, &p, x0_dev, u_dev, B, H, &neutral, integrator, dt)) return rc;
  if (B == 0) return PHNN_OK;
  if (!traj_dev) return fail(h, PHNN_ERR_INVALID_ARG, "traj_dev is NULL");
  PHNN_ON_DEVICE(h);
  p.traj = traj_dev;
  p.dx_out = dx_dev;
  p.no_cost = 1;
  const long long tiles = (B + kTileB - 1) / kTileB;
  const bool tapes = wgrad_workspace_dev != nullptr;
  if (tapes) p.stash = (float*)wgrad_workspace_dev + wgrad_tape_offset(h, wgrad_records(B, H, integrator));
  return launch_roll(h, false, false, tapes, integrator, p, tiles, (hipStream_t)stream);
}

int phnn_rollout_wgrad(phnn_handle* h, const float* x0_dev, const float* u_dev, int64_t B, int32_t H, int32_t integrator,
                       float dt, const float* traj_dev, const float* traj_bar_dev, const float* dx_bar_dev,
                       void* workspace_dev, float* grad_theta_dev, int32_t flags, float* grad_u_dev,
                       float* grad_x0_dev, void* stream) {
  if (!h) return PHNN_ERR_INVALID_ARG;
  const int accumulate = (flags & PHNN_WGRAD_ACCUMULATE) != 0;
  const bool tapes = (flags & PHNN_WGRAD_TAPES) != 0;
  if (!h->has_wgrad)
    return fail(h, PHNN_ERR_UNSUPPORTED, "no weight-gradient kernels for this model variant (pHNN and canonical pHNN have them)");
  phnn_cost neutral;
  memset(&neutral, 0, sizeof neutral);
  RollParams p;
  if (int rc = fill_roll(h, &p, x0_dev, u_dev, B, H, &neutral, integrator, dt)) return rc;
  if (!grad_theta_dev) return fail(h, PHNN_ERR_INVALID_ARG, "grad_theta_dev is NULL");
  PHNN_ON_DEVICE(h);
  hipStream_t st = (hipStream_t)stream;
  if (B == 0) {
    if (!accumulate) {
      hipError_t e = hipMemsetAsync(grad_theta_dev, 0, sizeof(float) * (size_t)h->n_params, st);
      if (e != hipSuccess) return hip_fail(h, e, "hipMemsetAsync");
    }
    return PHNN_OK;
  }
  if (!traj_dev || !workspace_dev) return fail(h, PHNN_ERR_INVALID_ARG, "traj_dev / workspace_dev is NULL");
  p.traj_in = traj_dev;
  p.traj_bar = traj_bar_dev;
  p.dx_bar = dx_bar_dev;
  p.grad_u = grad_u_dev;
  p.grad_x0 = grad_x0_dev;
  p.no_cost = 1;
  p.wrec = (float*)workspace_dev;
  const long long n_rec = wgrad_records(B, H, integrator);
  if (tapes) p.stash = (float*)workspace_dev + wgrad_tape_offset(h, n_rec);
  if (int rc = launch(h, tapes ? h->wg.grad_t[integrator] : h->wg.grad[integrator], p, (B + kTileB - 1) / kTileB, false, st))
    return rc;
  return wgrad_reduce(h, workspace_dev, n_rec, grad_theta_dev, accumulate, st, tapes ? h->wg.tape_floats[integrator] : 0);
}

int phnn_model_wgrad(phnn_handle* h, const float* x_dev, const float* u_dev, const float* lam_dev, const float* Hbar_dev,
                     int64_t N, void* workspace_dev, float* grad_theta_dev, int32_t accumulate, float* xbar_dev,
                     float* ubar_dev, void* stream) {
  if (!h) return PHNN_ERR_INVALID_ARG;
  if (!h->has_wgrad)
    return fail(h, PHNN_ERR_UNSUPPORTED, "no weight-gradient kernels for this model variant (pHNN and canonical pHNN have them)");
  if (N < 0 || !grad_theta_dev) return fail(h, PHNN_ERR_INVALID_ARG, "negative batch or grad_theta_dev is NULL");
  PHNN_ON_DEVICE(h);
  hipStream_t st = (hipStream_t)stream;
  if (N == 0) {
    if (!accumulate) {
      hipError_t e = hipMemsetAsync(grad_theta_dev, 0, sizeof(float) * (size_t)h->n_params, st);
      if (e != hipSuccess) return hip_fail(h, e, "hipMemsetAsync");
    }
    return PHNN_OK;
  }
  if (!x_dev || !u_dev || !lam_dev || !workspace_dev || !xbar_dev || !ubar_dev)
    return fail(h, PHNN_ERR_INVALID_ARG, "NULL tensor");
  PointParams p{h->d_img, x_dev, u_dev, lam_dev, xbar_dev, ubar_dev, (long long)N, Hbar_dev, (float*)workspace_dev};
  if (int rc = launch(h, h->wg.mvjp, p, (N + kTileB - 1) / kTileB, true, st)) return rc;
  return wgrad_reduce(h, workspace_dev, wgrad_records(N, 0, 0), grad_theta_dev, accumulate, st);
}

int phnn_adam_step(phnn_handle* h, float* u_dev, const float* grad_dev, float* exp_avg_dev, float* exp_avg_sq_dev,
                   int64_t count, float lr, float beta1, float beta2, float eps, int32_t step, const float* cost_dev,
                   float* best_cost_dev, float* best_u_dev, int64_t per, float u_min, float u_max, int32_t has_u_bounds,
                   void* stream) {
  if (!h) return PHNN_ERR_INVALID_ARG;
  if (!u_dev || !grad_dev || !exp_avg_dev || !exp_avg_sq_dev || count < 0 || step < 1)
    return fail(h, PHNN_ERR_INVALID_ARG, "NULL tensor, negative count or step < 1");
  if (best_cost_dev && (!cost_dev || !best_u_dev || per < 1 || count % per != 0))
    return fail(h, PHNN_ERR_INVALID_ARG, "best-iterate tracking needs cost_dev, best_u_dev and per | count");
  if (count == 0) return PHNN_OK;
  PHNN_ON_DEVICE(h);
  AdamParams p;
  memset(&p, 0, sizeof p);
  p.u = u_dev;
  p.g = grad_dev;
  p.m = exp_avg_dev;
  p.v = exp_avg_sq_dev;
  p.count = count;
  p.per = per > 0 ? per : 1;
  double b1 = (double)beta1, b2 = (double)beta2;
// ... 513 lines not shown
```

### phnn_mpc_amd/csrc/phnn_pack.h

```cpp
#pragma once
#include "phnn_variants.h"

#define PK_HD __host__ __device__ inline
#if defined(__HIP_DEVICE_COMPILE__)
#define PK_FOR(k, n) for (int k = (int)threadIdx.x; k < (int)(n); k += (int)blockDim.x)
#define PK_SYNC() __syncthreads()
#else
#define PK_FOR(k, n) for (int k = 0; k < (int)(n); ++k)
#define PK_SYNC() ((void)0)
#endif

constexpr int kPackThreads = 1024;

template <class F>
PK_HD float pk_max(int n, float* red, F f) {
  float m = 0.f;
  PK_FOR(k, n) m = fmaxf(m, f(k));
#if defined(__HIP_DEVICE_COMPILE__)
  red[threadIdx.x] = m;
  __syncthreads();
  for (int s = (int)blockDim.x / 2; s > 0; s >>= 1) {
    if ((int)threadIdx.x < s) red[threadIdx.x] = fmaxf(red[threadIdx.x], red[threadIdx.x + s]);
    __syncthreads();
  }
// ... 20 lines not shown
template <int HID>
PK_HD void pack_in_frag_h(float* dstf, const float* W, int nin, float sc) {
  _Float16* dst = reinterpret_cast<_Float16*>(dstf);
  PK_FOR(e, (HID / 16) * 64 * 8) {
    const int j = e & 7, lane = (e >> 3) & 63, nt = e >> 9, i = lane & 15, q = lane >> 4, c = j & 3;
    const float x = (q < 2 && c < nin) ? W[(size_t)(16 * nt + i) * nin + c] * sc : 0.f;
    const _Float16 h = (_Float16)x;
    const _Float16 l = (_Float16)(x - (float)h);
    dst[e] = q == 0 ? h : (q == 1 ? l : (_Float16)0.f);
  }
}
template <int HID>
PK_HD void pack_in_frag_T(float* dst, const float* W, int nout) {
  PK_FOR(e, (HID / 16) * 64) {
    const int nt = e >> 6, lane = e & 63, i = lane & 15, q = lane >> 4;
    dst[e] = q < nout ? W[(size_t)q * HID + 16 * nt + i] : 0.f;
  }
}
PK_HD void pack_rows(float* dst, const float* W, int rows, int cols, int ld, float sc = 1.0f) {
  PK_FOR(e, rows * cols) {
    const int r = e / cols, c = e % cols;
    dst[(size_t)r * ld + c] = W[e] * sc;
  }
}
PK_HD void pack_cols_as_rows(float* dst, const float* W, int rows, int cols, int ld, float div = 1.0f) {
  PK_FOR(e, rows * cols) {
    const int r = e / cols, c = e % cols;
    dst[(size_t)c * ld + r] = W[e] / div;
  }
}
PK_HD void pack_copy(float* dst, const float* src, int n, float sc = 1.0f) {
  PK_FOR(k, n) dst[k] = src[k] * sc;
}

PK_HD uint16_t pk_bf16_rne(float x) {
  const uint32_t u = __builtin_bit_cast(uint32_t, x);
  return (uint16_t)((u + 0x7FFFu + ((u >> 16) & 1u)) >> 16);
}
PK_HD float pk_bf16_to_f32(uint16_t b) { return __builtin_bit_cast(float, ((uint32_t)b) << 16); }

template <int HID>
PK_HD void pack_bf16x3(float* dstf, const float* W, float sc) {
  using I = BfImg<HID>;
  uint16_t* dst = reinterpret_cast<uint16_t*>(dstf);
  PK_FOR(e, HID * HID) {
    const int r = e / HID, pos = e % HID, u = pk_unit_of_pos(pos);
    const float x = W[(size_t)r * HID + u] * sc;
    const uint16_t h = pk_bf16_rne(x);
    const float r1 = x - pk_bf16_to_f32(h);
    const uint16_t m = pk_bf16_rne(r1);
    const uint16_t l = pk_bf16_rne(r1 - pk_bf16_to_f32(m));
    const size_t at = (size_t)r * I::RS + pos;
    dst[at] = h;
    dst[(size_t)I::PART / 2 + at] = m;
    dst[(size_t)I::PART + at] = l;
  }
}

PK_HD float pk_pow2_scale(float mx, bool always) {
  int e = 0;
  if (mx > 0.f && (always || mx < 0.5f || mx >= 1024.0f)) (void)__builtin_frexpf(mx, &e);
  return __builtin_ldexpf(1.0f, -e);
}

template <int HID>
PK_HD float pack_f16x2(float* dstf, const float* W, float sc, float* red) {
  using I = HfImg<HID>;
  const float mx = pk_max(HID * HID, red, [&](int k) { return __builtin_fabsf(W[k] * sc); });
  const float S = pk_pow2_scale(mx, false);
  _Float16* dst = reinterpret_cast<_Float16*>(dstf);
  PK_FOR(e, HID * HID) {
    const int r = e / HID, pos = e % HID, u = pk_unit_of_pos(pos);
    const float x = (W[(size_t)r * HID + u] * sc) * S;
    const _Float16 h = (_Float16)x;
    const _Float16 l = (_Float16)(x - (float)h);
    const size_t at = (size_t)r * I::RS + pos;
    dst[at] = h;
    dst[(size_t)I::PART / 2 + at] = l;
  }
  return S;
}

template <int HID, int MM, bool FOLD = true>
PK_HD const float* pack_h2(float* dst, const float* p, int nin, float* red) {
  using Y = LayH2<HID, MM>;
  const float* W1 = p; p += (size_t)HID * nin;
  const float* b1 = p; p += HID;
  const float* W2 = p; p += (size_t)HID * HID;
  const float* b2 = p; p += HID;
  const float* W3 = p; p += HID;
  const float* b3 = p; p += 1;
  const float k1 = (FOLD && kPreScaled<HID / 16>) ? 2.8853900817779268f : 1.0f;
  float S = 1.0f;
  if (MM == MM_BF16X3) pack_bf16x3<HID>(dst + Y::oW2, W2, k1);
  else if (MM == MM_F16X2) S = pack_f16x2<HID>(dst + Y::oW2, W2, k1, red);
  else pack_rows(dst + Y::oW2, W2, HID, HID, Y::LD, k1);
  S *= k1;
  pack_in_frag<HID>(dst + Y::oW1f, W1, nin, k1);
  if (MM == MM_F16X2) pack_in_frag_h<HID>(dst + Y::oW1h, W1, nin, k1);
  pack_copy(dst + Y::oB1, b1, HID, k1);
  pack_copy(dst + Y::oW3, W3, HID);
  float Sb = 1.0f;
  if (MM == MM_F16X2) {
    const float w3max = pk_max(HID, red, [&](int k) { return __builtin_fabsf(W3[k]); });
    const float n1 = pk_max(HID, red, [&](int r) {
      float a = 0.f;
      for (int c = 0; c < nin; ++c) a += __builtin_fabsf(W1[(size_t)r * nin + c]);
      return a;
    });
    const float n2 = pk_max(HID, red, [&](int r) {
      float b = 0.f;
      for (int c = 0; c < HID; ++c) b += __builtin_fabsf(W2[(size_t)r * HID + c]);
      return b;
    });
    const float bound = fmaxf(w3max, 0.77f * w3max * n1 * n2);
    while (bound * Sb > 1024.0f) Sb *= 0.5f;
  }
  PK_FOR(k, HID) {
    dst[Y::oB2 + k] = b2[k] * S;
    dst[Y::oW3B + k] = W3[k] * Sb;
    dst[Y::oW3S + k] = W3[k] * Sb / S;
  }
  pack_cols_as_rows(dst + Y::oW1T, W1, HID, nin, Y::LR, S * Sb);
  PK_FOR(k, 1) {
    dst[Y::oB3] = b3[0];
    dst[Y::oB3 + 1] = 2.8853900817779268f / S;
    dst[Y::oB3 + 2] = 1.0f / k1;
    dst[Y::oB3 + 3] = Sb;
  }
  return p;
}

template <int HID, int MM, bool FOLD = true>
PK_HD const float* pack_h1(float* dst, const float* p, int nin, int nout, float* red) {
  using Y = LayH1<HID, MM>;
  const float* V1 = p; p += (size_t)HID * nin;
  const float* c1 = p; p += HID;
  const float* V2 = p; p += (size_t)nout * HID;
  const float* c2 = p; p += nout;
  if (Y::HF) {
    const float mx = pk_max(nout * HID, red, [&](int k) { return __builtin_fabsf(V2[k]); });
    const float Sr = pk_pow2_scale(mx, true);
    _Float16* fw = reinterpret_cast<_Float16*>(dst + Y::oV2);
    _Float16* bw = reinterpret_cast<_Float16*>(dst + Y::oV2T);
    PK_FOR(e, nout * HID) {
      const int o = e / HID, pos = e % HID, u = pk_unit_of_pos(pos);
      const float x = V2[(size_t)o * HID + u] * Sr;
      const _Float16 h = (_Float16)x, l = (_Float16)(x - (float)h);
      fw[(size_t)o * Y::RS + pos] = h;
      fw[(size_t)Y::FPART / 2 + (size_t)o * Y::RS + pos] = l;
      bw[(size_t)u * 16 + o] = h;
      bw[(size_t)Y::BPART / 2 + (size_t)u * 16 + o] = l;
    }
    PK_FOR(k, 1) dst[Y::oSc] = 1.0f / Sr;
  } else {
    pack_rows(dst + Y::oV2, V2, nout, HID, Y::LD);
    PK_FOR(k, 1) dst[Y::oSc] = 1.0f;
  }
  const float k1 = (FOLD && kPreScaled<HID / 16>) ? 2.8853900817779268f : 1.0f;
  pack_in_frag<HID>(dst + Y::oV1f, V1, nin, k1);
  if (Y::HF) pack_in_frag_h<HID>(dst + Y::oV1h, V1, nin, k1);
  pack_copy(dst + Y::oC1, c1, HID, k1);
  pack_copy(dst + Y::oC2, c2, nout);
  pack_cols_as_rows(dst + Y::oV1T, V1, HID, nin, Y::LR);
  return p;
}

PK_HD float pk_softplus(float x) { return x > 20.f ? x : log1pf(expf(x)); }

template <class M>
struct PackOf;

template <int N, int HID, bool FIXG, int MM, int MI, int ACT>
struct PackOf<PhnnModel<N, HID, FIXG, MM, MI, ACT>> {
  using M = PhnnModel<N, HID, FIXG, MM, MI, ACT>;
  PK_HD static void run(float* img, const phnn_desc* d, const float* p, float* red) {
    PK_FOR(k, M::IMG) img[k] = 0.f;
    PK_SYNC();
    const float* J = p; p += N * N;
    const float* G = nullptr;
    if (d->fixed_G) { G = p; p += N * MI; }
    constexpr bool FOLD = ACT == ACT_TANH;
    p = pack_h1<HID, MM, FOLD>(img + M::oR, p, N, N * N, red);
    p = pack_h2<HID, MM, FOLD>(img + M::oH, p, N, red);
    if (!d->fixed_G) p = pack_h1<HID, MM, FOLD>(img + M::oGn, p, N, N * MI, red);
    PK_FOR(e, N * N) {
      const int i = e / N, j = e % N;
      img[M::oJ + e] = J[i * N + j] - J[j * N + i];
    }
    if (G) pack_copy(img + M::oG, G, N * MI);
  }
};

template <int HID, int MM, int MI, int MT, int ACT>
struct PackOf<CanonModel<HID, MM, MI, MT, ACT>> {
  using M = CanonModel<HID, MM, MI, MT, ACT>;
  PK_HD static void run(float* img, const phnn_desc* d, const float* p, float* red) {
    PK_FOR(k, M::IMG) img[k] = 0.f;
    PK_SYNC();
    const float* Rd = p; p += 4;
    const float* G = p; p += 4 * MI;
    float* c = img + M::oC;
    if (MT == MASS_CARTPOLE) {
      const float log_a = p[0], b = p[1], log_c = p[2];
      p += 3;
      PK_FOR(k, 1) {
        c[0] = expf(log_a) + 1e-3f;
        c[1] = b;
        c[2] = expf(log_c) + 1e-3f;
      }
    } else if (MT == MASS_CONSTANT) {
      const float l00 = pk_softplus(p[0]) + 1e-3f, l10 = p[2], l11 = pk_softplus(p[3]) + 1e-3f;
      p += 4;
      const float i00 = 1.0f / l00, i11 = 1.0f / l11, i10 = -l10 / (l00 * l11);
      float* cw = img + M::oCW;
      PK_FOR(k, 1) {
        c[0] = l00 * l00;
        c[1] = l00 * l10;
        c[2] = l10 * l10 + l11 * l11;
        cw[0] = i00 * i00 + i10 * i10;
        cw[1] = i10 * i11;
        cw[2] = i11 * i11;
      }
    } else {
      const int nout = MT == MASS_DIAGONAL ? 2 : 3;
      float* dm = img + M::oMn;
      const float* W1 = p; p += 64 * 2;
      const float* b1 = p; p += 64;
      const float* W2 = p; p += 64 * 64;
      const float* b2 = p; p += 64;
      const float* Wo = p; p += (size_t)nout * 64;
      const float* bo = p; p += nout;
      pack_in_frag<64>(dm + LayM::oW1f, W1, 2, 1.0f);
      pack_copy(dm + LayM::oB1, b1, 64);
      pack_rows(dm + LayM::oW2, W2, 64, 64, LayM::LD);
      pack_copy(dm + LayM::oB2, b2, 64);
      pack_rows(dm + LayM::oWo, Wo, nout, 64, LayM::LR);
      pack_copy(dm + LayM::oBo, bo, nout);
      pack_in_frag_T<64>(dm + LayM::oWoTf, Wo, nout);
      pack_cols_as_rows(dm + LayM::oW1T, W1, 64, 2, LayM::LR);
    }
    p = pack_h2<HID, MM, ACT == ACT_TANH>(img + M::oH, p, 4, red);
    PK_FOR(i, 4) {
      c[4 + i] = pk_softplus(Rd[i]) + 1e-4f;
      c[8 + i] = Rd[i] > 20.f ? 1.0f : (float)(1.0 / (1.0 + exp(-(double)Rd[i])));
    }
    pack_copy(c + 12, G, 4 * MI);
    (void)d;
  }
};

template <int N, int HID, int MM, int ACT>
struct PackOf<OdeModel<N, HID, MM, ACT>> {
  using M = OdeModel<N, HID, MM, ACT>;
  PK_HD static void run(float* img, const phnn_desc* d, const float* p, float* red) {
    const int nin = N + 1;
    PK_FOR(k, M::IMG) img[k] = 0.f;
    PK_SYNC();
    const float* W1 = p; p += (size_t)HID * nin;
    const float* b1 = p; p += HID;
    const float* W2 = p; p += (size_t)HID * HID;
    const float* b2 = p; p += HID;
    const float* W3 = p; p += (size_t)HID * HID;
    const float* b3 = p; p += HID;
    const float* W4 = p; p += (size_t)N * HID;
    const float* b4 = p; p += N;
    float S2 = 1.0f, S3 = 1.0f;
    pack_in_frag<HID>(img + M::oW1f, W1, nin, 1.0f);
    pack_copy(img + M::oB1, b1, HID);
    if (MM == MM_F16X2) {
      S2 = pack_f16x2<HID>(img + M::oW2, W2, 1.0f, red);
      S3 = pack_f16x2<HID>(img + M::oW3, W3, 1.0f, red);
    } else {
      pack_rows(img + M::oW2, W2, HID, HID, M::LD);
      pack_rows(img + M::oW3, W3, HID, HID, M::LD);
    }
    pack_copy(img + M::oB2, b2, HID, S2);
    pack_copy(img + M::oB3, b3, HID, S3);
    pack_rows(img + M::oW4r, W4, N, HID, M::LR);
    pack_copy(img + M::oB4, b4, N);
    pack_in_frag_T<HID>(img + M::oW4f, W4, N);
    const float S23 = S2 * S3;
    PK_FOR(e, HID * 4) {
      const int r = e >> 2, c = e & 3;
      if (c < nin) img[M::oW1T + (size_t)c * M::LR + r] = W1[(size_t)r * nin + c] / S23;
    }
    if (M::WIDE) {
      PK_FOR(e, (HID / 16) * 16) {
        const int nt = e >> 4, lane = e & 15;
        img[M::oW1fu + nt * 64 + lane] = W1[(size_t)(16 * nt + lane) * nin + N];
      }
      PK_FOR(r, HID) img[M::oW1Tu + r] = W1[(size_t)r * nin + N] / S23;
    }
    PK_FOR(k, 1) {
      img[M::oSC + 0] = 2.8853900817779268f / S2;
      img[M::oSC + 1] = 2.8853900817779268f / S3;
    }
    (void)d;
  }
};

struct PackParams {
  const float* orig;
  const int* pad_src;
  int n_pad;
  float* pblob;
  float* img;
  phnn_desc pdesc;
};
int phnn_pack_launch(int variant, const PackParams& p, hipStream_t st);
```

### phnn_mpc_amd/csrc/phnn_split.hip

```cpp
#define PHNN_ADJOINT_UNIT
#include "phnn_variants.h"

template <class M>
static SplitSet split_set() {
  SplitSet g;
  fill_fwd<M>(g.fwd);
  fill_grad<M>(g.grad);
  g.lds_floats = M::IMG + 4 * M::SCR + kXchFloats;
  return g;
}

bool phnn_split_kernels(int variant, SplitSet* g) {
  switch (variant) {
    case V_PHNN_4_128_FIX_H: *g = split_set<PhnnSplit<4>>(); return true;
    case V_PHNN_2_128_FIX_H: *g = split_set<PhnnSplit<2>>(); return true;
    case V_CANON_128_H: *g = split_set<CanonSplit<>>(); return true;
    default: return false;
  }
}
```

### phnn_mpc_amd/csrc/phnn_variants.h

```cpp
#pragma once
#include "phnn_kernels.hip.h"

enum Variant {
  V_NONE = 0,
  V_PHNN_4_128_FIX,
  V_PHNN_4_64_FIX,
  V_PHNN_2_64_GNET,
  V_PHNN_2_64_FIX,
  V_CANON_128,
  V_CANON_64,
  V_ODE_2_128,
  V_ODE_2_64,
  V_ODE_3_128,
  V_PHNN_4_128_FIX_BF,
  V_CANON_128_BF,
  V_PHNN_4_128_FIX_H,
  V_CANON_128_H,
  V_ODE_2_128_H,
  V_ODE_3_128_H,
  V_ODE_4_128,
  V_PHNN_4_128_GNET_H,
  V_PHNN_2_128_GNET_H,
  V_PHNN_2_128_FIX_H,
  V_PHNN_4_64_FIX_H,
// ... 5 lines not shown
  V_PHNN_4_128_GNET_H_M2,
  V_CANON_128_H_M2,
  V_PHNN_4_128_FIX_H_M3,
  V_PHNN_4_128_GNET_H_M3,
  V_CANON_128_H_M3,
  V_PHNN_4_128_FIX_H_M4,
  V_PHNN_4_128_GNET_H_M4,
  V_CANON_128_H_M4,
  V_CANON_128_H_MCONST,
  V_CANON_128_H_MDIAG,
  V_CANON_128_H_MFULL,
  V_PHNN_4_128_FIX_SILU,
  V_PHNN_4_128_FIX_RELU,
  V_CANON_128_SILU,
  V_CANON_128_RELU,
  V_ODE_2_128_RELU,
  V_ODE_4_128_RELU,
  V_PHNN_4_128_FIX_ELU,
  V_PHNN_4_128_FIX_GELU,
  V_CANON_128_ELU,
  V_CANON_128_GELU,
  V_ODE_2_128_ELU,
  V_ODE_2_128_GELU,
  V_ODE_4_128_ELU,
  V_ODE_4_128_GELU,
};

using M_PHNN_4_128_FIX = PhnnModel<4, 128, true>;
using M_PHNN_4_64_FIX = PhnnModel<4, 64, true>;
using M_PHNN_2_64_GNET = PhnnModel<2, 64, false>;
using M_PHNN_2_64_FIX = PhnnModel<2, 64, true>;
using M_CANON_128 = CanonModel<128>;
using M_CANON_64 = CanonModel<64>;
using M_ODE_2_128 = OdeModel<2, 128>;
using M_ODE_2_64 = OdeModel<2, 64>;
using M_ODE_3_128 = OdeModel<3, 128>;
using M_PHNN_4_128_FIX_BF = PhnnModel<4, 128, true, MM_BF16X3>;
using M_CANON_128_BF = CanonModel<128, MM_BF16X3>;
using M_PHNN_4_128_FIX_H = PhnnModel<4, 128, true, MM_F16X2>;
using M_CANON_128_H = CanonModel<128, MM_F16X2>;
using M_ODE_2_128_H = OdeModel<2, 128, MM_F16X2>;
using M_ODE_3_128_H = OdeModel<3, 128, MM_F16X2>;
using M_ODE_4_128 = OdeModel<4, 128>;
using M_PHNN_4_128_GNET_H = PhnnModel<4, 128, false, MM_F16X2>;
using M_PHNN_2_128_GNET_H = PhnnModel<2, 128, false, MM_F16X2>;
using M_PHNN_2_128_FIX_H = PhnnModel<2, 128, true, MM_F16X2>;
using M_PHNN_4_64_FIX_H = PhnnModel<4, 64, true, MM_F16X2>;
using M_PHNN_2_64_GNET_H = PhnnModel<2, 64, false, MM_F16X2>;
using M_PHNN_2_64_FIX_H = PhnnModel<2, 64, true, MM_F16X2>;
using M_CANON_64_H = CanonModel<64, MM_F16X2>;
using M_ODE_2_64_H = OdeModel<2, 64, MM_F16X2>;
using M_PHNN_4_128_FIX_H_M2 = PhnnModel<4, 128, true, MM_F16X2, 2>;
using M_PHNN_4_128_GNET_H_M2 = PhnnModel<4, 128, false, MM_F16X2, 2>;
using M_CANON_128_H_M2 = CanonModel<128, MM_F16X2, 2>;
using M_PHNN_4_128_FIX_H_M3 = PhnnModel<4, 128, true, MM_F16X2, 3>;
using M_PHNN_4_128_GNET_H_M3 = PhnnModel<4, 128, false, MM_F16X2, 3>;
using M_CANON_128_H_M3 = CanonModel<128, MM_F16X2, 3>;
using M_PHNN_4_128_FIX_H_M4 = PhnnModel<4, 128, true, MM_F16X2, 4>;
using M_PHNN_4_128_GNET_H_M4 = PhnnModel<4, 128, false, MM_F16X2, 4>;
using M_CANON_128_H_M4 = CanonModel<128, MM_F16X2, 4>;
using M_CANON_128_H_MCONST = CanonModel<128, MM_F16X2, 1, MASS_CONSTANT>;
using M_CANON_128_H_MDIAG = CanonModel<128, MM_F16X2, 1, MASS_DIAGONAL>;
using M_CANON_128_H_MFULL = CanonModel<128, MM_F16X2, 1, MASS_FULL>;
using M_PHNN_4_128_FIX_SILU = PhnnModel<4, 128, true, MM_F32, 1, ACT_SILU>;
using M_PHNN_4_128_FIX_RELU = PhnnModel<4, 128, true, MM_F32, 1, ACT_RELU>;
using M_CANON_128_SILU = CanonModel<128, MM_F32, 1, MASS_CARTPOLE, ACT_SILU>;
using M_CANON_128_RELU = CanonModel<128, MM_F32, 1, MASS_CARTPOLE, ACT_RELU>;
using M_ODE_2_128_RELU = OdeModel<2, 128, MM_F32, ACT_RELU>;
using M_ODE_4_128_RELU = OdeModel<4, 128, MM_F32, ACT_RELU>;
using M_PHNN_4_128_FIX_ELU = PhnnModel<4, 128, true, MM_F32, 1, ACT_ELU>;
using M_PHNN_4_128_FIX_GELU = PhnnModel<4, 128, true, MM_F32, 1, ACT_GELU>;
using M_CANON_128_ELU = CanonModel<128, MM_F32, 1, MASS_CARTPOLE, ACT_ELU>;
using M_CANON_128_GELU = CanonModel<128, MM_F32, 1, MASS_CARTPOLE, ACT_GELU>;
using M_ODE_2_128_ELU = OdeModel<2, 128, MM_F32, ACT_ELU>;
using M_ODE_2_128_GELU = OdeModel<2, 128, MM_F32, ACT_GELU>;
using M_ODE_4_128_ELU = OdeModel<4, 128, MM_F32, ACT_ELU>;
using M_ODE_4_128_GELU = OdeModel<4, 128, MM_F32, ACT_GELU>;

using RollKernel = void (*)(RollParams);
using RollTable = RollKernel[2][2][2];

template <class M>
void fill_fwd(RollTable t) {
  t[0][0][0] = k_rollout_fwd<M, PHNN_INTEG_EULER, false>;
  t[0][0][1] = k_rollout_fwd<M, PHNN_INTEG_RK4, false>;
  t[0][1][0] = k_rollout_fwd<M, PHNN_INTEG_EULER, true>;
  t[0][1][1] = k_rollout_fwd<M, PHNN_INTEG_RK4, true>;
  t[1][0][0] = k_rollout_fwd<M, PHNN_INTEG_EULER, false, true>;
  t[1][0][1] = k_rollout_fwd<M, PHNN_INTEG_RK4, false, true>;
  t[1][1][0] = k_rollout_fwd<M, PHNN_INTEG_EULER, true, true>;
  t[1][1][1] = k_rollout_fwd<M, PHNN_INTEG_RK4, true, true>;
}

template <class M>
void fill_grad(RollTable t) {
  t[0][0][0] = k_rollout_grad<M, PHNN_INTEG_EULER, false>;
  t[0][0][1] = k_rollout_grad<M, PHNN_INTEG_RK4, false>;
  t[0][1][0] = k_rollout_grad<M, PHNN_INTEG_EULER, true>;
  t[0][1][1] = k_rollout_grad<M, PHNN_INTEG_RK4, true>;
  t[1][0][0] = k_rollout_grad<M, PHNN_INTEG_EULER, false, false, true>;
  t[1][0][1] = k_rollout_grad<M, PHNN_INTEG_RK4, false, false, true>;
  t[1][1][0] = k_rollout_grad<M, PHNN_INTEG_EULER, true, false, true>;
  t[1][1][1] = k_rollout_grad<M, PHNN_INTEG_RK4, true, false, true>;
}

struct GradSet {
  RollTable grad;
  void (*mvjp)(PointParams);
};

bool phnn_grad_kernels(int variant, GradSet* g);

struct SplitSet {
  RollTable fwd, grad;
  int lds_floats;
};
bool phnn_split_kernels(int variant, SplitSet* g);

struct WgradSet {
  void (*grad[2])(RollParams);
  void (*grad_t[2])(RollParams);
  void (*mvjp)(PointParams);
  void (*reduce)(WgradParams);
  void (*reduce_t)(WgradParams);
  int tape_floats[2];
  int rec_floats;
  int blob_floats;
  int reduce_waves;
  int reduce_lds_bytes;
};
bool phnn_wgrad_kernels(int variant, WgradSet* g);
hipError_t phnn_wgrad_finish(const float* slab, int rows, int PP, const int* map, int P, float* out, int accumulate,
                             hipStream_t stream);

#define PHNN_FOR_EACH_VARIANT(X)                                                                                       \
  X(V_PHNN_4_128_FIX, M_PHNN_4_128_FIX, "phnn<n=4,hid=128,fixedG>") \
  X(V_PHNN_4_64_FIX, M_PHNN_4_64_FIX, "phnn<n=4,hid=64,fixedG>") \
  X(V_PHNN_2_64_GNET, M_PHNN_2_64_GNET, "phnn<n=2,hid=64,Gnet>") \
  X(V_PHNN_2_64_FIX, M_PHNN_2_64_FIX, "phnn<n=2,hid=64,fixedG>") \
  X(V_CANON_128, M_CANON_128, "canonical<hid=128>") \
  X(V_CANON_64, M_CANON_64, "canonical<hid=64>") \
  X(V_ODE_2_128, M_ODE_2_128, "odefunc<n=2,hid=128>") \
  X(V_ODE_2_64, M_ODE_2_64, "odefunc<n=2,hid=64>") \
  X(V_ODE_3_128, M_ODE_3_128, "odefunc<n=3,hid=128>") \
  X(V_PHNN_4_128_FIX_BF, M_PHNN_4_128_FIX_BF, "phnn<n=4,hid=128,fixedG,bf16x3>") \
  X(V_CANON_128_BF, M_CANON_128_BF, "canonical<hid=128,bf16x3>") \
  X(V_PHNN_4_128_FIX_H, M_PHNN_4_128_FIX_H, "phnn<n=4,hid=128,fixedG,f16x2>") \
  X(V_CANON_128_H, M_CANON_128_H, "canonical<hid=128,f16x2>") \
  X(V_ODE_2_128_H, M_ODE_2_128_H, "odefunc<n=2,hid=128,f16x2>") \
  X(V_ODE_3_128_H, M_ODE_3_128_H, "odefunc<n=3,hid=128,f16x2>") \
  X(V_ODE_4_128, M_ODE_4_128, "odefunc<n=4,hid=128>") \
  X(V_PHNN_4_128_GNET_H, M_PHNN_4_128_GNET_H, "phnn<n=4,hid=128,Gnet,f16x2>") \
  X(V_PHNN_2_128_GNET_H, M_PHNN_2_128_GNET_H, "phnn<n=2,hid=128,Gnet,f16x2>") \
  X(V_PHNN_2_128_FIX_H, M_PHNN_2_128_FIX_H, "phnn<n=2,hid=128,fixedG,f16x2>") \
  X(V_PHNN_4_64_FIX_H, M_PHNN_4_64_FIX_H, "phnn<n=4,hid=64,fixedG,f16x2>") \
  X(V_PHNN_2_64_GNET_H, M_PHNN_2_64_GNET_H, "phnn<n=2,hid=64,Gnet,f16x2>") \
  X(V_PHNN_2_64_FIX_H, M_PHNN_2_64_FIX_H, "phnn<n=2,hid=64,fixedG,f16x2>") \
  X(V_CANON_64_H, M_CANON_64_H, "canonical<hid=64,f16x2>") \
  X(V_ODE_2_64_H, M_ODE_2_64_H, "odefunc<n=2,hid=64,f16x2>") \
  X(V_PHNN_4_128_FIX_H_M2, M_PHNN_4_128_FIX_H_M2, "phnn<n=4,m=2,hid=128,fixedG,f16x2>") \
  X(V_PHNN_4_128_GNET_H_M2, M_PHNN_4_128_GNET_H_M2, "phnn<n=4,m=2,hid=128,Gnet,f16x2>") \
  X(V_CANON_128_H_M2, M_CANON_128_H_M2, "canonical<m=2,hid=128,f16x2>") \
  X(V_PHNN_4_128_FIX_H_M3, M_PHNN_4_128_FIX_H_M3, "phnn<n=4,m=3,hid=128,fixedG,f16x2>") \
  X(V_PHNN_4_128_GNET_H_M3, M_PHNN_4_128_GNET_H_M3, "phnn<n=4,m=3,hid=128,Gnet,f16x2>") \
  X(V_CANON_128_H_M3, M_CANON_128_H_M3, "canonical<m=3,hid=128,f16x2>") \
  X(V_PHNN_4_128_FIX_H_M4, M_PHNN_4_128_FIX_H_M4, "phnn<n=4,m=4,hid=128,fixedG,f16x2>") \
  X(V_PHNN_4_128_GNET_H_M4, M_PHNN_4_128_GNET_H_M4, "phnn<n=4,m=4,hid=128,Gnet,f16x2>") \
  X(V_CANON_128_H_M4, M_CANON_128_H_M4, "canonical<m=4,hid=128,f16x2>") \
  X(V_CANON_128_H_MCONST, M_CANON_128_H_MCONST, "canonical<hid=128,f16x2,mass=constant>") \
  X(V_CANON_128_H_MDIAG, M_CANON_128_H_MDIAG, "canonical<hid=128,f16x2,mass=diagonal>") \
  X(V_CANON_128_H_MFULL, M_CANON_128_H_MFULL, "canonical<hid=128,f16x2,mass=full>") \
  X(V_PHNN_4_128_FIX_SILU, M_PHNN_4_128_FIX_SILU, "phnn<n=4,hid=128,fixedG,silu>") \
  X(V_PHNN_4_128_FIX_RELU, M_PHNN_4_128_FIX_RELU, "phnn<n=4,hid=128,fixedG,relu>") \
  X(V_CANON_128_SILU, M_CANON_128_SILU, "canonical<hid=128,silu>") \
  X(V_CANON_128_RELU, M_CANON_128_RELU, "canonical<hid=128,relu>") \
  X(V_ODE_2_128_RELU, M_ODE_2_128_RELU, "odefunc<n=2,hid=128,relu>") \
  X(V_ODE_4_128_RELU, M_ODE_4_128_RELU, "odefunc<n=4,hid=128,relu>") \
  X(V_PHNN_4_128_FIX_ELU, M_PHNN_4_128_FIX_ELU, "phnn<n=4,hid=128,fixedG,elu>") \
  X(V_PHNN_4_128_FIX_GELU, M_PHNN_4_128_FIX_GELU, "phnn<n=4,hid=128,fixedG,gelu>") \
  X(V_CANON_128_ELU, M_CANON_128_ELU, "canonical<hid=128,elu>") \
  X(V_CANON_128_GELU, M_CANON_128_GELU, "canonical<hid=128,gelu>") \
  X(V_ODE_2_128_ELU, M_ODE_2_128_ELU, "odefunc<n=2,hid=128,elu>") \
  X(V_ODE_2_128_GELU, M_ODE_2_128_GELU, "odefunc<n=2,hid=128,gelu>") \
  X(V_ODE_4_128_ELU, M_ODE_4_128_ELU, "odefunc<n=4,hid=128,elu>") \
  X(V_ODE_4_128_GELU, M_ODE_4_128_GELU, "odefunc<n=4,hid=128,gelu>")
```

### phnn_mpc_amd/csrc/phnn_wgrad.hip

```cpp
#define PHNN_ADJOINT_UNIT
#define PHNN_WGRAD_UNIT
#include "phnn_variants.h"

template <class M>
static WgradSet wgrad_set() {
  WgradSet g;
  g.grad[0] = k_rollout_grad<M, PHNN_INTEG_EULER, false, true>;
  g.grad[1] = k_rollout_grad<M, PHNN_INTEG_RK4, false, true>;
  g.grad_t[0] = k_rollout_grad<M, PHNN_INTEG_EULER, true, true>;
  g.grad_t[1] = k_rollout_grad<M, PHNN_INTEG_RK4, true, true>;
  g.mvjp = k_model_vjp<M, true>;
  g.reduce = k_wgrad_reduce<M, false>;
  g.reduce_t = k_wgrad_reduce<M, true>;
  g.tape_floats[0] = StashStep<M, PHNN_INTEG_EULER>::FLOATS;
  g.tape_floats[1] = StashStep<M, PHNN_INTEG_RK4>::SLOT;
  g.rec_floats = M::Rec::SIZE;
  g.blob_floats = BlobOf<M>::SIZE;
  g.reduce_waves = M::T;
  g.reduce_lds_bytes = (int)sizeof(float) * WgGeom<M>::LDS_FLOATS;
  return g;
}

bool phnn_wgrad_kernels(int variant, WgradSet* g) {
  switch (variant) {
#define PHNN_WCASE(V, M) \
  case V: *g = wgrad_set<M>(); return true;
    PHNN_WCASE(V_PHNN_4_128_FIX, M_PHNN_4_128_FIX)
    PHNN_WCASE(V_PHNN_4_128_FIX_H, M_PHNN_4_128_FIX_H)
    PHNN_WCASE(V_PHNN_4_64_FIX, M_PHNN_4_64_FIX)
    PHNN_WCASE(V_PHNN_2_64_GNET, M_PHNN_2_64_GNET)
    PHNN_WCASE(V_PHNN_2_64_FIX, M_PHNN_2_64_FIX)
    PHNN_WCASE(V_PHNN_4_128_GNET_H, M_PHNN_4_128_GNET_H)
    PHNN_WCASE(V_PHNN_2_128_GNET_H, M_PHNN_2_128_GNET_H)
    PHNN_WCASE(V_PHNN_2_128_FIX_H, M_PHNN_2_128_FIX_H)
    PHNN_WCASE(V_CANON_128, M_CANON_128)
    PHNN_WCASE(V_CANON_128_H, M_CANON_128_H)
    PHNN_WCASE(V_CANON_64, M_CANON_64)
    PHNN_WCASE(V_PHNN_4_128_FIX_H_M2, M_PHNN_4_128_FIX_H_M2)
    PHNN_WCASE(V_PHNN_4_128_GNET_H_M2, M_PHNN_4_128_GNET_H_M2)
    PHNN_WCASE(V_CANON_128_H_M2, M_CANON_128_H_M2)
    PHNN_WCASE(V_PHNN_4_128_FIX_H_M3, M_PHNN_4_128_FIX_H_M3)
    PHNN_WCASE(V_PHNN_4_128_GNET_H_M3, M_PHNN_4_128_GNET_H_M3)
    PHNN_WCASE(V_CANON_128_H_M3, M_CANON_128_H_M3)
    PHNN_WCASE(V_PHNN_4_128_FIX_H_M4, M_PHNN_4_128_FIX_H_M4)
    PHNN_WCASE(V_PHNN_4_128_GNET_H_M4, M_PHNN_4_128_GNET_H_M4)
    PHNN_WCASE(V_CANON_128_H_M4, M_CANON_128_H_M4)
    PHNN_WCASE(V_CANON_128_H_MCONST, M_CANON_128_H_MCONST)
    PHNN_WCASE(V_CANON_128_H_MDIAG, M_CANON_128_H_MDIAG)
    PHNN_WCASE(V_CANON_128_H_MFULL, M_CANON_128_H_MFULL)
#undef PHNN_WCASE
    default: return false;
  }
}

hipError_t phnn_wgrad_finish(const float* slab, int rows, int PP, const int* map, int P, float* out, int accumulate,
                             hipStream_t stream) {
  const int threads = 256;
  hipLaunchKernelGGL(k_wgrad_finish, dim3((unsigned)((P + threads - 1) / threads)), dim3(threads), 0, stream, slab, rows,
                     PP, map, P, out, accumulate);
  return hipGetLastError();
}
```

Baseline: 30.52 million.

## Precompute per-sample Hessian curvature block to shrink MPC tape and HVP work

Splits the tanh-network Hessian-vector product into two parts. The diagonal second-derivative term (W1ᵀ diag(q1·dtanh·a1) W1) becomes a 4x4 curvature matrix built from packed f16x2 products of W1 columns, computed in the forward pass and stored in the tape instead of the full q1 activation vector. The backward pass then applies this small matrix rather than reloading q1 and doing the extra elementwise fused multiply-add. Training-tape kernels keep the old layout through a new TAPE_TRAIN variant. The cost is extra MFMA work and LDS space for the packed products, plus f16-split rounding in the curvature term.

New measurement: 32.38 million (median of 6 runs). +6.1%, better.

```diff
diff --git a/phnn_mpc_amd/csrc/phnn_kernels.hip.h b/phnn_mpc_amd/csrc/phnn_kernels.hip.h
--- a/phnn_mpc_amd/csrc/phnn_kernels.hip.h
+++ b/phnn_mpc_amd/csrc/phnn_kernels.hip.h
@@ -809,6 +809,13 @@
     }
 }
 
+constexpr int TAPE_NONE = 0, TAPE_MPC = 1, TAPE_TRAIN = 2;
+template <class M, int TK>
+constexpr int tape_floats() {
+  if constexpr (TK == TAPE_MPC && M::CURV) return M::TAPE_C;
+  else return M::STASH;
+}
+
 template <int HID>
 struct HTape {
   Act<HID / 16> a1, a2, q1;
@@ -965,8 +972,97 @@
   tanh_act_pre<Y::T>(a1);
 }
 
-template <int HID, int MM = MM_F32, bool WG = false, int ACT = ACT_TANH, int SITE = kInHHvp>
-DEV f32x4 hnet_hvp(const float* L, Lane ln, HTape<HID>& tp, f32x4 v, float* rec = nullptr) {
+template <int HID>
+struct CurvImg {
+  static constexpr int RS = HID + 16, PART = 10 * RS * 2;
+  static constexpr int oConst = 2 * PART / 4;
+  static constexpr int FLOATS = oConst + 4;
+};
+struct Curv {
+  float m[16];
+};
+template <int T>
+DEV void hnet_curv_operand(const Act<T>& q1, const Act<T>& a1, Split2<T>& sp) {
+  Act<T> c;
+#pragma unroll
+  for (int t = 0; t < T; ++t) c.v[t] = (q1.v[t] * dtanh(a1.v[t])) * a1.v[t];
+  split_act_h<T>(c, sp);
+}
+template <int HID>
+DEV f32x4 hnet_curv_kstep(const float* P, Lane ln, int s, f16x8 ch, f16x8 cl) {
+  using I = CurvImg<HID>;
+  keep_lds_reads_local();
+  const int a = ln.i >> 2, b = ln.i & 3, lo = a < b ? a : b, hi = a < b ? b : a;
+  const int row = (lo * (9 - lo)) / 2 + (hi - lo);
+  const char* base = reinterpret_cast<const char*>(P) + row * (I::RS * 2) + ln.q * 16 + s * 64;
+  const f16x8 ah = *reinterpret_cast<const f16x8*>(base);
+  const f16x8 al = *reinterpret_cast<const f16x8*>(base + I::PART);
+  return mfma_h(ah, ch, mfma_h(ah, cl, mfma_h(al, ch, splat4(0.f))));
+}
+template <int HID>
+DEV f32x4 hnet_curv(const float* P, Lane ln, const HTape<HID>& tp) {
+  constexpr int T = HID / 16;
+  Split2<T> sp;
+  hnet_curv_operand<T>(tp.q1, tp.a1, sp);
+  f32x4 tot = hnet_curv_kstep<HID>(P, ln, 0, sp.h[0], sp.l[0]);
+#pragma unroll
+  for (int s = 1; s < T / 2; ++s) tot = tot + hnet_curv_kstep<HID>(P, ln, s, sp.h[s], sp.l[s]);
+  return tot * P[CurvImg<HID>::oConst];
+}
+DEV void spread_curv(f32x4 mine, Lane ln, Curv& c) {
+#pragma unroll
+  for (int r = 0; r < 4; ++r)
+#pragma unroll
+    for (int j = 0; j < 4; ++j) c.m[4 * r + j] = __shfl(mine[j], 16 * r + ln.i);
+}
+DEV f32x4 curv_apply(const Curv& c, f32x4 v) {
+  f32x4 o;
+#pragma unroll
+  for (int r = 0; r < 4; ++r) {
+    float s = 0.f;
+#pragma unroll
+    for (int j = 0; j < 4; ++j) s = __builtin_fmaf(c.m[4 * r + j], v[j], s);
+    o[r] = s;
+  }
+  return o;
+}
+
+template <int HID, bool COMPACT>
+DEV void hnet_tape_store(float* stash, int oC, const float* P, Lane ln, const HTape<HID>& tp, f32x4 dH) {
+  constexpr int T = HID / 16;
+  store_act<T>(stash, ln, tp.a2);
+  if constexpr (COMPACT) {
+    if (ln.q == 0) PHNN_NT_STORE(dH, reinterpret_cast<f32x4*>(stash + T * 256) + ln.i);
+    PHNN_NT_STORE(hnet_curv<HID>(P, ln, tp), reinterpret_cast<f32x4*>(stash + oC) + ln.i * 4 + ln.q);
+  } else {
+    store_act<T>(stash + T * 256, ln, tp.q1);
+    if (ln.q == 0) PHNN_NT_STORE(dH, reinterpret_cast<f32x4*>(stash + 2 * T * 256) + ln.i);
+  }
+}
+template <int T, bool COMPACT>
+DEV f32x4 tape_load_dH(const float* stash, Lane ln) {
+  return PHNN_NT_LOAD(reinterpret_cast<const f32x4*>(stash + (COMPACT ? 1 : 2) * T * 256) + ln.i);
+}
+DEV void load_curv(const float* src, Lane ln, Curv& c) {
+  const f32x4* p = reinterpret_cast<const f32x4*>(src) + ln.i * 4;
+#pragma unroll
+  for (int k = 0; k < 4; ++k) {
+    f32x4 v = PHNN_NT_LOAD(p + k);
+#pragma unroll
+    for (int e = 0; e < 4; ++e) c.m[4 * k + e] = v[e];
+  }
+}
+template <int HID, bool COMPACT>
+DEV void hnet_tape_load(const float* stash, int oC, Lane ln, HTape<HID>& tp, Curv& cv) {
+  constexpr int T = HID / 16;
+  load_act<T>(stash, ln, tp.a2);
+  if constexpr (COMPACT) load_curv(stash + oC, ln, cv);
+  else load_act<T>(stash + T * 256, ln, tp.q1);
+}
+
+template <int HID, int MM = MM_F32, bool WG = false, int ACT = ACT_TANH, int SITE = kInHHvp, bool CQ = false>
+DEV f32x4 hnet_hvp(const float* L, Lane ln, HTape<HID>& tp, f32x4 v, float* rec = nullptr, const Curv* cv = nullptr) {
+  static_assert(!CQ || (MM == MM_F16X2 && ACT == ACT_TANH && !WG), "the curvature block exists for f16x2 Tanh MPC kernels");
   if constexpr (ACT != ACT_TANH) {
     static_assert(!WG, "weight-gradient kernels exist for Tanh models only");
     return hnet_hvp_g<HID, ACT>(L, ln, tp, v);
@@ -987,8 +1083,10 @@
   in_layer_mm<T, MM, SITE>(ad1, L, Y::oW1f, Y::oW1h, ln, v);
 #pragma unroll
   for (int t = 0; t < T; ++t) ad1.v[t] = dtanh(tp.a1.v[t]) * ad1.v[t];
-#pragma unroll
-  for (int t = 0; t < T; ++t) tp.q1.v[t] = tp.q1.v[t] * (tp.a1.v[t] * ad1.v[t]);
+  if constexpr (!CQ) {
+#pragma unroll
+    for (int t = 0; t < T; ++t) tp.q1.v[t] = tp.q1.v[t] * (tp.a1.v[t] * ad1.v[t]);
+  }
   zero_act<T>(w);
   if (MM == MM_BF16X3) {
     Split3<T> sp;
@@ -1026,9 +1124,11 @@
   if (WG) store_rec_scaled<T>(rec + 3 * T * 256, ln, qd, unscale);
 #pragma unroll
   for (int t = 0; t < T; ++t) {
-    qd.v[t] = __builtin_elementwise_fma(qd.v[t], dtanh(tp.a1.v[t]), tp.q1.v[t]);
+    if constexpr (CQ) qd.v[t] = qd.v[t] * dtanh(tp.a1.v[t]);
+    else qd.v[t] = __builtin_elementwise_fma(qd.v[t], dtanh(tp.a1.v[t]), tp.q1.v[t]);
   }
   f32x4 Hv = to4_rep<T>(L + Y::oW1T, ln, qd);
+  if constexpr (CQ) return (Hv * (-2.0f * L[Y::oB3 + 2]) + curv_apply(*cv, v)) * unscale;
   return Hv * (-2.0f * unscale * L[Y::oB3 + 2]);
 }
 
@@ -1210,24 +1310,25 @@
   static constexpr int oGn = oR + LayH1<HID, MM>::SIZE;
   static constexpr int oJ = oGn + (FIXG ? 0 : LayH1<HID, MM>::SIZE);
   static constexpr int oG = oJ + 16;
-  static constexpr int IMG = oG + 16;
+  static constexpr int oP = oG + 16;
+  static constexpr bool CURV = MM == MM_F16X2 && ACT == ACT_TANH &&
+                               4 * (oP + CurvImg<HID>::FLOATS + kMaxWaves * SCR) <= 160 * 1024;
+  static constexpr int IMG = oP + (CURV ? CurvImg<HID>::FLOATS : 0);
 
   static constexpr int oStashRf = 2 * T * 256 + 64;
   static constexpr int STASH = oStashRf + 256;
-
-  template <bool WANT_H, bool ST = false>
+  static constexpr int oTapeRf = T * 256 + 64, oTapeC = oTapeRf + 256, TAPE_C = oTapeC + 256;
+
+  template <bool WANT_H, int TK = TAPE_NONE>
   DEV static f32x4 f(const float* L, float* scr, Lane ln, f32x4 x, f32x4 u, float& Hval, float* stash = nullptr) {
+    constexpr bool ST = TK != TAPE_NONE, CT = TK == TAPE_MPC && CURV;
     keep_lds_reads_local();
     HTape<HID> tp;
     f32x4 dH = hnet_grad<HID, WANT_H, MM, kInHFwd, ACT>(L + oH, ln, x, tp, Hval);
-    if (ST) {
-      store_act<T>(stash, ln, tp.a2);
-      store_act<T>(stash + T * 256, ln, tp.q1);
-      if (ln.q == 0) PHNN_NT_STORE(dH, reinterpret_cast<f32x4*>(stash + 2 * T * 256) + ln.i);
-    }
+    if (ST) hnet_tape_store<HID, CT>(stash, oTapeC, L + oP, ln, tp, dH);
     Act<T> hR;
     float rf[16];
-    h1_fwd<HID, MM, kInHNet1, ACT>(L + oR, scr, ln, x, hR, rf, ST ? stash + oStashRf : nullptr);
+    h1_fwd<HID, MM, kInHNet1, ACT>(L + oR, scr, ln, x, hR, rf, ST ? stash + (CT ? oTapeRf : oStashRf) : nullptr);
     float G[N * MI];
     if (FIXG) {
 #pragma unroll
@@ -1279,18 +1380,20 @@
   template <bool ST = false, bool WG = false, int INH = -1>
   DEV static void vjp(const float* L, float* scr, Lane ln, f32x4 x, f32x4 u, f32x4 lam, f32x4& xbar, f32x4& ubar,
                       const float* stash = nullptr, float* rec = nullptr, float Hbar = 0.f) {
+    constexpr bool CQ = CURV && !WG;
     keep_lds_reads_local();
     HTape<HID> tp;
+    Curv cv;
     float Hdummy;
     f32x4 dH;
     float rf[16];
     if (ST) {
-      dH = PHNN_NT_LOAD(reinterpret_cast<const f32x4*>(stash + 2 * T * 256) + ln.i);
-      load_rf(stash + oStashRf, ln, rf);
-      load_act<T>(stash, ln, tp.a2);
-      load_act<T>(stash + T * 256, ln, tp.q1);
+      dH = tape_load_dH<T, CQ>(stash, ln);
+      load_rf(stash + (CQ ? oTapeRf : oStashRf), ln, rf);
+      hnet_tape_load<HID, CQ>(stash, oTapeC, ln, tp, cv);
     } else {
       dH = hnet_grad<HID, false, MM, INH & kInHRecomp, ACT>(L + oH, ln, x, tp, Hdummy);
+      if constexpr (CQ) spread_curv(hnet_curv<HID>(L + oP, ln, tp), ln, cv);
     }
     if (WG && !ST) {
       store_rec<T>(rec, ln, tp.a2);
@@ -1367,7 +1470,7 @@
       sm[9] = f32x4{Hbar, 0.f, 0.f, 0.f};
     }
     if (ST) hnet_layer1<HID, MM, ACT>(L + oH, ln, x, tp.a1);
-    xbar = xb + hnet_hvp<HID, MM, WG, ACT, INH & kInHHvp>(L + oH, ln, tp, v, rec);
+    xbar = xb + hnet_hvp<HID, MM, WG, ACT, INH & kInHHvp, CQ>(L + oH, ln, tp, v, rec, &cv);
     if (WG) xbar = xbar + Hbar * dH;
   }
 };
@@ -1461,7 +1564,9 @@
   static constexpr int oCG = oC + 12;
   static constexpr int oCW = oC + 28;
   static constexpr int oMn = oC + 32;
-  static constexpr int IMG = oMn + (MT_ >= MASS_DIAGONAL ? LayM::SIZE : 0);
+  static constexpr int oP = oMn + (MT_ >= MASS_DIAGONAL ? LayM::SIZE : 0);
+  static constexpr bool CURV = MM_ == MM_F16X2 && ACT_ == ACT_TANH;
+  static constexpr int IMG = oP + (CURV ? CurvImg<HID>::FLOATS : 0);
 
   DEV static void mass_eval(const float* L, Lane ln, f32x4 y, float (&m)[3], float (&w)[3], MTape& mt) {
     if (MT == MASS_CONSTANT) {
@@ -1487,9 +1592,11 @@
   }
 
   static constexpr int STASH = 2 * T * 256 + 64;
-
-  template <bool WANT_H, bool ST = false>
+  static constexpr int oTapeC = T * 256 + 64, TAPE_C = oTapeC + 256;
+
+  template <bool WANT_H, int TK = TAPE_NONE>
   DEV static f32x4 f(const float* L, float* scr, Lane ln, f32x4 y, f32x4 u, float& Hval, float* stash = nullptr) {
+    constexpr bool ST = TK != TAPE_NONE, CT = TK == TAPE_MPC && CURV;
     keep_lds_reads_local();
     if constexpr (MT != MASS_CARTPOLE) {
       float m[3], w[3];
@@ -1498,11 +1605,7 @@
       f32x4 z = {y[0], y[1], m[0] * y[2] + m[1] * y[3], m[1] * y[2] + m[2] * y[3]};
       HTape<HID> tp;
       f32x4 dH = hnet_grad<HID, WANT_H, MM, kInHFwd, ACT>(L + oH, ln, z, tp, Hval);
-      if (ST) {
-        store_act<T>(stash, ln, tp.a2);
-        store_act<T>(stash + T * 256, ln, tp.q1);
-        if (ln.q == 0) PHNN_NT_STORE(dH, reinterpret_cast<f32x4*>(stash + 2 * T * 256) + ln.i);
-      }
+      if (ST) hnet_tape_store<HID, CT>(stash, oTapeC, L + oP, ln, tp, dH);
       float dp0 = (-dH[0] - L[oC + 6] * dH[2]) + Base_Gu(L, 2, u);
       float dp1 = (-dH[1] - L[oC + 7] * dH[3]) + Base_Gu(L, 3, u);
       return f32x4{w[0] * z[2] + w[1] * z[3], w[1] * z[2] + w[2] * z[3], w[0] * dp0 + w[1] * dp1, w[1] * dp0 + w[2] * dp1};
@@ -1514,11 +1617,7 @@
     f32x4 z = {y[0], y[1], a * y[2] + bc * y[3], bc * y[2] + c * y[3]};
     HTape<HID> tp;
     f32x4 dH = hnet_grad<HID, WANT_H, MM, kInHFwd, ACT>(L + oH, ln, z, tp, Hval);
-    if (ST) {
-      store_act<T>(stash, ln, tp.a2);
-      store_act<T>(stash + T * 256, ln, tp.q1);
-      if (ln.q == 0) PHNN_NT_STORE(dH, reinterpret_cast<f32x4*>(stash + 2 * T * 256) + ln.i);
-    }
+    if (ST) hnet_tape_store<HID, CT>(stash, oTapeC, L + oP, ln, tp, dH);
     float dp0 = (-dH[0] - L[oC + 6] * dH[2]) + Base_Gu(L, 2, u);
     float dp1 = (-dH[1] - L[oC + 7] * dH[3]) + Base_Gu(L, 3, u);
     float det = (a * c - bc * bc) + 1e-6f;
@@ -1533,6 +1632,8 @@
   template <bool ST = false, bool WG = false, int INH = -1>
   DEV static void vjp(const float* L, float* scr, Lane ln, f32x4 y, f32x4 u, f32x4 lam, f32x4& ybar, f32x4& ubar,
                       const float* stash = nullptr, float* rec = nullptr, float Hbar = 0.f) {
+    constexpr bool CQ = CURV && !WG;
+    Curv cv;
     keep_lds_reads_local();
     if constexpr (MT != MASS_CARTPOLE) {
       float m[3], w[3];
@@ -1543,12 +1644,12 @@
       float Hdummy;
       f32x4 dH;
       if (ST) {
-        dH = PHNN_NT_LOAD(reinterpret_cast<const f32x4*>(stash + 2 * T * 256) + ln.i);
-        load_act<T>(stash, ln, tp.a2);
-        load_act<T>(stash + T * 256, ln, tp.q1);
+        dH = tape_load_dH<T, CQ>(stash, ln);
+        hnet_tape_load<HID, CQ>(stash, oTapeC, ln, tp, cv);
         hnet_layer1<HID, MM, ACT>(L + oH, ln, z, tp.a1);
       } else {
         dH = hnet_grad<HID, false, MM, INH & kInHRecomp, ACT>(L + oH, ln, z, tp, Hdummy);
+        if constexpr (CQ) spread_curv(hnet_curv<HID>(L + oP, ln, tp), ln, cv);
       }
       const float Rd2 = L[oC + 6], Rd3 = L[oC + 7];
       const float dp0 = (-dH[0] - Rd2 * dH[2]) + Base_Gu(L, 2, u);
@@ -1573,7 +1674,7 @@
           sm[9] = f32x4{Hbar, 0.f, 0.f, 0.f};
         }
       }
-      f32x4 zb = hnet_hvp<HID, MM, WG, ACT, INH & kInHHvp>(L + oH, ln, tp, v, rec);
+      f32x4 zb = hnet_hvp<HID, MM, WG, ACT, INH & kInHHvp, CQ>(L + oH, ln, tp, v, rec, &cv);
       if (WG) zb = zb + Hbar * dH;
       zb[2] += pb0;
       zb[3] += pb1;
@@ -1613,12 +1714,12 @@
     float Hdummy;
     f32x4 dH;
     if (ST) {
-      dH = PHNN_NT_LOAD(reinterpret_cast<const f32x4*>(stash + 2 * T * 256) + ln.i);
-      load_act<T>(stash, ln, tp.a2);
-      load_act<T>(stash + T * 256, ln, tp.q1);
+      dH = tape_load_dH<T, CQ>(stash, ln);
+      hnet_tape_load<HID, CQ>(stash, oTapeC, ln, tp, cv);
       hnet_layer1<HID, MM, ACT>(L + oH, ln, z, tp.a1);
     } else {
       dH = hnet_grad<HID, false, MM, INH & kInHRecomp, ACT>(L + oH, ln, z, tp, Hdummy);
+      if constexpr (CQ) spread_curv(hnet_curv<HID>(L + oP, ln, tp), ln, cv);
     }
     float Rd2 = L[oC + 6], Rd3 = L[oC + 7];
     float dp0 = (-dH[0] - Rd2 * dH[2]) + Base_Gu(L, 2, u);
@@ -1649,7 +1750,7 @@
         sm[9] = f32x4{Hbar, 0.f, 0.f, 0.f};
       }
     }
-    f32x4 zb = hnet_hvp<HID, MM, WG, ACT, INH & kInHHvp>(L + oH, ln, tp, v, rec);
+    f32x4 zb = hnet_hvp<HID, MM, WG, ACT, INH & kInHHvp, CQ>(L + oH, ln, tp, v, rec, &cv);
     if (WG) zb = zb + Hbar * dH;
     zb[2] += pb0;
     zb[3] += pb1;
@@ -1735,6 +1836,15 @@
 struct HTapeW {
   ActW a1, a2, q1;
 };
+DEV void curv_put_w(const float* P, Lane ln, const HTapeW& tp) {
+  Split2<2> sp;
+  hnet_curv_operand<2>(tp.q1, tp.a1, sp);
+  xch_put_partial(ln.xch + kXP1, ln, hnet_curv_kstep<128>(P, ln, ln.w, sp.h[0], sp.l[0]));
+}
+DEV f32x4 curv_get_w(const float* P, Lane ln) {
+  const f32x4* p = reinterpret_cast<const f32x4*>(ln.xch + kXP1) + ln.lane;
+  return (((p[0] + p[64]) + p[128]) + p[192]) * P[CurvImg<128>::oConst];
+}
 
 template <int SITE = kInHFwd, class PreBarrier>
 DEV f32x4 hnet_grad_w(const float* L, Lane ln, f32x4 z, HTapeW& tp, PreBarrier pre_barrier) {
@@ -1790,7 +1900,7 @@
   return to4_group<2>(L + Y::oW1T + (ln.i & 3) * Y::LR + 16 * t0, ln, g.v);
 }
 
-DEV f32x4 hnet_hvp_w(const float* L, Lane ln, HTapeW& tp, f32x4 v, float& scale) {
+DEV f32x4 hnet_hvp_w(const float* L, Lane ln, HTapeW& tp, f32x4 v, float& scale, float& unscale, f32x4& vn) {
   using Y = LayH2<128, MM_F16X2>;
   const int t0 = 2 * ln.w;
   float mx = fmaxf(fmaxf(__builtin_fabsf(v[0]), __builtin_fabsf(v[1])), fmaxf(__builtin_fabsf(v[2]), __builtin_fabsf(v[3])));
@@ -1798,14 +1908,13 @@
   (void)__builtin_frexpf(mx, &e);
   e = (mx > 0.f && mx < 3.0e38f) ? e : 0;
   v = v * __builtin_ldexpf(1.0f, -e);
-  const float unscale = __builtin_ldexpf(1.0f, e);
+  vn = v;
+  unscale = __builtin_ldexpf(1.0f, e);
   ActW ad1, w;
   zero_act<2>(ad1);
   in_layer_mm<2, MM_F16X2, kInHHvp>(ad1, L, Y::oW1f, Y::oW1h, ln, v, t0);
 #pragma unroll
   for (int t = 0; t < 2; ++t) ad1.v[t] = dtanh(tp.a1.v[t]) * ad1.v[t];
-#pragma unroll
-  for (int t = 0; t < 2; ++t) tp.q1.v[t] = tp.q1.v[t] * (tp.a1.v[t] * ad1.v[t]);
   {
     Split2<2> sp;
     split_act_h<2>(ad1, sp);
@@ -1840,8 +1949,8 @@
     sq_bwd_h_w(qd, L + Y::oW2, ln, all);
   }
 #pragma unroll
-  for (int t = 0; t < 2; ++t) qd.v[t] = __builtin_elementwise_fma(qd.v[t], dtanh(tp.a1.v[t]), tp.q1.v[t]);
-  scale = -2.0f * unscale * L[Y::oB3 + 2];
+  for (int t = 0; t < 2; ++t) qd.v[t] = qd.v[t] * dtanh(tp.a1.v[t]);
+  scale = -2.0f * L[Y::oB3 + 2];
   keep_lds_reads_local();
   return to4_group<2>(L + Y::oW1T + (ln.i & 3) * Y::LR + 16 * t0, ln, qd.v);
 }
@@ -1851,7 +1960,8 @@
   using Base = PhnnModel<N_, 128, true, MM_F16X2>;
   static constexpr int N = N_, HID = 128, T = 8, MM = MM_F16X2;
   static constexpr bool FIXG = true, SPLIT = true;
-  static constexpr int SCR = Base::SCR, IMG = Base::IMG, STASH = Base::STASH, MI = 1;
+  static constexpr int SCR = Base::SCR, IMG = Base::IMG, STASH = Base::STASH, TAPE_C = Base::TAPE_C, MI = 1;
+  static constexpr bool CURV = true;
   static constexpr int oH = Base::oH, oR = Base::oR, oJ = Base::oJ, oG = Base::oG;
   using YR = LayH1<128, MM_F16X2>;
 
@@ -1877,23 +1987,26 @@
     gather16(scr, ln, o, rf);
   }
 
-  template <bool WANT_H, bool ST = false>
+  template <bool WANT_H, int TK = TAPE_NONE>
   DEV static f32x4 f(const float* L, float* scr, Lane ln, f32x4 x, f32x4 u, float& Hval, float* stash = nullptr) {
     static_assert(!WANT_H, "the split-tile kernels are rollout kernels");
+    constexpr bool ST = TK != TAPE_NONE, CT = TK == TAPE_MPC;
     keep_lds_reads_local();
     HTapeW tp;
     ActW hR;
     f32x4 P = hnet_grad_w(L + oH, ln, x, tp, [&]() { rnet_layer1(L, ln, x, hR); });
     xch_put_partial(ln.xch + kXP0, ln, P);
+    if (CT) curv_put_w(L + Base::oP, ln, tp);
     float rf[16];
-    rnet_out(L, scr, ln, rf, ST ? stash + Base::oStashRf : nullptr);
+    rnet_out(L, scr, ln, rf, ST ? stash + (CT ? Base::oTapeRf : Base::oStashRf) : nullptr);
     if (ST) {
       store_act<2>(stash + 2 * ln.w * 256, ln, tp.a2);
-      store_act<2>(stash + T * 256 + 2 * ln.w * 256, ln, tp.q1);
+      if (!CT) store_act<2>(stash + T * 256 + 2 * ln.w * 256, ln, tp.q1);
     }
     __syncthreads();
     f32x4 dH = xch_sum_partials(ln.xch + kXP0, ln);
-    if (ST && ln.q == 0 && ln.w == 0) PHNN_NT_STORE(dH, reinterpret_cast<f32x4*>(stash + 2 * T * 256) + ln.i);
+    if (ST && ln.q == 0 && ln.w == 0) PHNN_NT_STORE(dH, reinterpret_cast<f32x4*>(stash + (CT ? 1 : 2) * T * 256) + ln.i);
+    if (CT) store_rf(stash + Base::oTapeC, ln, curv_get_w(L + Base::oP, ln));
     float G[N];
 #pragma unroll
     for (int i = 0; i < N; ++i) G[i] = L[oG + i];
@@ -1908,13 +2021,14 @@
     const int t0 = 2 * ln.w;
     HTapeW tp;
     ActW hR;
+    Curv cv;
     f32x4 dH;
     float rf[16];
     if (ST) {
-      dH = PHNN_NT_LOAD(reinterpret_cast<const f32x4*>(stash + 2 * T * 256) + ln.i);
-      load_rf(stash + Base::oStashRf, ln, rf);
+      dH = tape_load_dH<T, true>(stash, ln);
+      load_rf(stash + Base::oTapeRf, ln, rf);
       load_act<2>(stash + t0 * 256, ln, tp.a2);
-      load_act<2>(stash + T * 256 + t0 * 256, ln, tp.q1);
+      load_curv(stash + Base::oTapeC, ln, cv);
       using Y = LayH2<128, MM_F16X2>;
       load_vec<2>(tp.a1, L + oH + Y::oB1 + 16 * t0, ln);
       in_layer_mm<2, MM_F16X2, kInHRecomp>(tp.a1, L + oH, Y::oW1f, Y::oW1h, ln, x, t0);
@@ -1923,9 +2037,11 @@
     } else {
       f32x4 P = hnet_grad_w<kInHRecomp>(L + oH, ln, x, tp, [&]() { rnet_layer1<kInHNet1Adj>(L, ln, x, hR); });
       xch_put_partial(ln.xch + kXP0, ln, P);
+      curv_put_w(L + Base::oP, ln, tp);
       rnet_out(L, scr, ln, rf);
       __syncthreads();
       dH = xch_sum_partials(ln.xch + kXP0, ln);
+      spread_curv(curv_get_w(L + Base::oP, ln), ln, cv);
     }
     float S[N][N], Stl[N], StdH[N];
     sym_from_rf<N>(rf, S);
@@ -1974,14 +2090,15 @@
       for (int k = 0; k < N; ++k) acc = __builtin_fmaf(-S[j][k], Stl[k], acc);
       v[j] = acc;
     }
-    float scaleH;
-    f32x4 PH = hnet_hvp_w(L + oH, ln, tp, v, scaleH);
+    float scaleH, unscaleH;
+    f32x4 vn;
+    f32x4 PH = hnet_hvp_w(L + oH, ln, tp, v, scaleH, unscaleH, vn);
     xch_put_partial(ln.xch + kXP0, ln, PR);
     xch_put_partial(ln.xch + kXP1, ln, PH);
     __syncthreads();
     f32x4 xb = splat4(0.f);
     xb += xch_sum_partials(ln.xch + kXP0, ln) * unscaleR;
-    xbar = xb + xch_sum_partials(ln.xch + kXP1, ln) * scaleH;
+    xbar = xb + (xch_sum_partials(ln.xch + kXP1, ln) * scaleH + curv_apply(cv, vn)) * unscaleH;
   }
 };
 
@@ -1990,13 +2107,15 @@
   using Base = CanonModel<128, MM_F16X2>;
   static constexpr int N = 4, HID = 128, T = 8, MM = MM_F16X2;
   static constexpr bool SPLIT = true;
-  static constexpr int SCR = 0, IMG = Base::IMG, STASH = Base::STASH, oH = Base::oH, oC = Base::oC, MI = 1;
+  static constexpr int SCR = 0, IMG = Base::IMG, STASH = Base::STASH, TAPE_C = Base::TAPE_C, oH = Base::oH, oC = Base::oC, MI = 1;
+  static constexpr bool CURV = true;
   DEV static float Base_Gu(const float* L, int row, f32x4 u) { return Base::Base_Gu(L, row, u); }
   DEV static f32x4 Base_Gt(const float* L, float dpb0, float dpb1) { return Base::Base_Gt(L, dpb0, dpb1); }
 
-  template <bool WANT_H, bool ST = false>
+  template <bool WANT_H, int TK = TAPE_NONE>
   DEV static f32x4 f(const float* L, float* scr, Lane ln, f32x4 y, f32x4 u, float& Hval, float* stash = nullptr) {
     static_assert(!WANT_H, "the split-tile kernels are rollout kernels");
+    constexpr bool ST = TK != TAPE_NONE, CT = TK == TAPE_MPC;
     keep_lds_reads_local();
     float a = L[oC + 0], b = L[oC + 1], c = L[oC + 2];
     float sn, cs;
@@ -2006,13 +2125,15 @@
     HTapeW tp;
     f32x4 P = hnet_grad_w(L + oH, ln, z, tp, []() {});
     xch_put_partial(ln.xch + kXP0, ln, P);
+    if (CT) curv_put_w(L + Base::oP, ln, tp);
     if (ST) {
       store_act<2>(stash + 2 * ln.w * 256, ln, tp.a2);
-      store_act<2>(stash + T * 256 + 2 * ln.w * 256, ln, tp.q1);
+      if (!CT) store_act<2>(stash + T * 256 + 2 * ln.w * 256, ln, tp.q1);
     }
     __syncthreads();
     f32x4 dH = xch_sum_partials(ln.xch + kXP0, ln);
-    if (ST && ln.q == 0 && ln.w == 0) PHNN_NT_STORE(dH, reinterpret_cast<f32x4*>(stash + 2 * T * 256) + ln.i);
+    if (ST && ln.q == 0 && ln.w == 0) PHNN_NT_STORE(dH, reinterpret_cast<f32x4*>(stash + (CT ? 1 : 2) * T * 256) + ln.i);
+    if (CT) store_rf(stash + Base::oTapeC, ln, curv_get_w(L + Base::oP, ln));
     float dp0 = (-dH[0] - L[oC + 6] * dH[2]) + Base_Gu(L, 2, u);
     float dp1 = (-dH[1] - L[oC + 7] * dH[3]) + Base_Gu(L, 3, u);
     float det = (a * c - bc * bc) + 1e-6f;
@@ -2033,11 +2154,12 @@
     float bc = b * cs;
     f32x4 z = {y[0], y[1], a * y[2] + bc * y[3], bc * y[2] + c * y[3]};
     HTapeW tp;
+    Curv cv;
     f32x4 dH;
     if (ST) {
-      dH = PHNN_NT_LOAD(reinterpret_cast<const f32x4*>(stash + 2 * T * 256) + ln.i);
+      dH = tape_load_dH<T, true>(stash, ln);
       load_act<2>(stash + t0 * 256, ln, tp.a2);
-      load_act<2>(stash + T * 256 + t0 * 256, ln, tp.q1);
+      load_curv(stash + Base::oTapeC, ln, cv);
       using Y = LayH2<128, MM_F16X2>;
       load_vec<2>(tp.a1, L + oH + Y::oB1 + 16 * t0, ln);
       in_layer_mm<2, MM_F16X2, kInHRecomp>(tp.a1, L + oH, Y::oW1f, Y::oW1h, ln, z, t0);
@@ -2045,8 +2167,10 @@
     } else {
       f32x4 P = hnet_grad_w<kInHRecomp>(L + oH, ln, z, tp, []() {});
       xch_put_partial(ln.xch + kXP0, ln, P);
+      curv_put_w(L + Base::oP, ln, tp);
       __syncthreads();
       dH = xch_sum_partials(ln.xch + kXP0, ln);
+      spread_curv(curv_get_w(L + Base::oP, ln), ln, cv);
     }
     float Rd2 = L[oC + 6], Rd3 = L[oC + 7];
     float dp0 = (-dH[0] - Rd2 * dH[2]) + Base_Gu(L, 2, u);
@@ -2061,11 +2185,12 @@
     float mb11 = lam[1] * z[3] + lam[3] * dp1;
     f32x4 v = {-dpb0, -dpb1, -Rd2 * dpb0, -Rd3 * dpb1};
     ubar = Base_Gt(L, dpb0, dpb1);
-    float scaleH;
-    f32x4 PH = hnet_hvp_w(L + oH, ln, tp, v, scaleH);
+    float scaleH, unscaleH;
+    f32x4 vn;
+    f32x4 PH = hnet_hvp_w(L + oH, ln, tp, v, scaleH, unscaleH, vn);
     xch_put_partial(ln.xch + kXP1, ln, PH);
     __syncthreads();
-    f32x4 zb = xch_sum_partials(ln.xch + kXP1, ln) * scaleH;
+    f32x4 zb = (xch_sum_partials(ln.xch + kXP1, ln) * scaleH + curv_apply(cv, vn)) * unscaleH;
     zb[2] += pb0;
     zb[3] += pb1;
     float bcb = zb[2] * y[3] + zb[3] * y[2];
@@ -2163,9 +2288,11 @@
 
   static constexpr int VEC24 = ACT == ACT_TANH ? T * 192 : T * 256;
   static constexpr int STASH = 2 * VEC24;
-
-  template <bool WANT_H, bool ST = false>
+  static constexpr bool CURV = false;
+
+  template <bool WANT_H, int TK = TAPE_NONE>
   DEV static f32x4 f(const float* L, float* scr, Lane ln, f32x4 x, f32x4 uv, float& Hval, float* stash = nullptr) {
+    constexpr bool ST = TK != TAPE_NONE;
     const float u = uv[0];
     Tape tp;
     if (WANT_H) Hval = 0.f;
@@ -2401,10 +2528,11 @@
   return cost;
 }
 
-template <class M, int INTEG>
+template <class M, int INTEG, int TK = TAPE_MPC>
 struct StashStep {
-  static constexpr int SLOT = M::STASH + 64;
-  static constexpr int FLOATS = INTEG == PHNN_INTEG_EULER ? M::STASH : 4 * SLOT;
+  static constexpr int TAPE = tape_floats<M, TK>();
+  static constexpr int SLOT = TAPE + 64;
+  static constexpr int FLOATS = INTEG == PHNN_INTEG_EULER ? TAPE : 4 * SLOT;
 };
 DEV void store_stage(float* dst, Lane ln, f32x4 y) {
   if (ln.q == 0 && ln.w == 0) PHNN_NT_STORE(y, reinterpret_cast<f32x4*>(dst) + ln.i);
@@ -2460,9 +2588,11 @@
   }
 };
 
-template <class M, int INTEG, bool STASH, bool REF = false>
+template <class M, int INTEG, int TK, bool REF = false>
 DEV void fwd_march(const RollParams& p, const float* L, const TileCtx& tc) {
   constexpr int N = M::N;
+  constexpr bool STASH = TK != TAPE_NONE;
+  using SS = StashStep<M, INTEG, STASH ? TK : TAPE_MPC>;
   const Lane ln = tc.ln;
   float* scr = tc.scr;
   const long long tile = tc.tile, b = tc.b;
@@ -2486,20 +2616,20 @@
     f32x4 u = clamp_u4<MI>(p.c, load_u<MI>(up, t));
     if (MI == 1) cost = __builtin_fmaf(u[0] * p.c.R[0], u[0], cost);
     else cost += control_cost<MI>(p.c, u);
-    float* sl = STASH ? p.stash + (tile * p.H + t) * (long long)StashStep<M, INTEG>::FLOATS : nullptr;
-    f32x4 k1 = M::template f<false, STASH>(L, scr, ln, x, u, Hd, sl);
+    float* sl = STASH ? p.stash + (tile * p.H + t) * (long long)SS::FLOATS : nullptr;
+    f32x4 k1 = M::template f<false, TK>(L, scr, ln, x, u, Hd, sl);
     if (p.dx_out && writer) store_state<N>(p.dx_out + (b * p.H + t) * N, k1);
     if (INTEG == PHNN_INTEG_EULER) {
       x = x + p.dt * k1;
     } else {
-      constexpr int SLOT = StashStep<M, INTEG>::SLOT;
+      constexpr int SLOT = SS::SLOT;
       f32x4 acc = k1, kp = k1;
 #pragma unroll 1
       for (int s = 1; s < 4; ++s) {
         const f32x4 y = x + (s == 3 ? p.dt : p.half_dt) * kp;
         float* ss = STASH ? sl + s * SLOT : nullptr;
-        if (STASH) store_stage(ss + M::STASH, ln, y);
-        kp = M::template f<false, STASH>(L, scr, ln, y, u, Hd, ss);
+        if (STASH) store_stage(ss + SS::TAPE, ln, y);
+        kp = M::template f<false, TK>(L, scr, ln, y, u, Hd, ss);
         acc = acc + (s == 3 ? 1.0f : 2.0f) * kp;
       }
       x = x + p.sixth_dt * acc;
@@ -2511,18 +2641,19 @@
   if (writer && p.cost) p.cost[b] = cost;
 }
 
-template <class M, int INTEG, bool STASH, bool REF = false>
+template <class M, int INTEG, int TK, bool REF = false>
 __global__ __launch_bounds__(64 * kMaxWaves) void k_rollout_fwd(RollParams p) {
   extern __shared__ __attribute__((aligned(16))) float lds[];
   stage_image<M::IMG>(lds, p.img);
   TileCtx tc;
   if (!tile_ctx<M>(tc, lds, p.B)) return;
-  fwd_march<M, INTEG, STASH, REF>(p, lds, tc);
+  fwd_march<M, INTEG, TK, REF>(p, lds, tc);
 }
 
 template <class M, int INTEG, bool STASH, bool WG = false, bool REF = false>
 DEV void grad_march(const RollParams& p, const float* L, const TileCtx& tc) {
   constexpr int N = M::N;
+  using SS = StashStep<M, INTEG, WG ? TAPE_TRAIN : TAPE_MPC>;
   const Lane ln = tc.ln;
   float* scr = tc.scr;
   const long long tile = tc.tile, b = tc.b;
@@ -2560,16 +2691,16 @@
     if constexpr (INTEG == PHNN_INTEG_EULER) {
       if constexpr (WG) {
         M::template vjp<STASH, true>(L, scr, ln, x, u, p.dt * lam + dxb, xb, ub,
-                                     STASH ? p.stash + (tile * p.H + t) * (long long)M::STASH : nullptr, rec);
+                                     STASH ? p.stash + (tile * p.H + t) * (long long)SS::TAPE : nullptr, rec);
       } else {
         M::template vjp<STASH>(L, scr, ln, x, u, p.dt * lam + dxb, xb, ub,
-                               STASH ? p.stash + (tile * p.H + t) * (long long)M::STASH : nullptr);
+                               STASH ? p.stash + (tile * p.H + t) * (long long)SS::TAPE : nullptr);
       }
       lam = lam + xb;
       utot = ub;
     } else {
-      constexpr int SLOT = StashStep<M, INTEG>::SLOT;
-      const float* sl = STASH ? p.stash + (tile * p.H + t) * (long long)StashStep<M, INTEG>::FLOATS : nullptr;
+      constexpr int SLOT = SS::SLOT;
+      const float* sl = STASH ? p.stash + (tile * p.H + t) * (long long)SS::FLOATS : nullptr;
       f32x4 y2 = x, y3 = x, y4 = x;
       if constexpr (!STASH) {
         f32x4 y = x;
@@ -2587,7 +2718,7 @@
 #pragma unroll 1
       for (int s = 3; s >= 0; --s) {
         f32x4 y;
-        if constexpr (STASH) y = s == 0 ? load_state<N>(tr + (long long)t * N) : load_stage(sl + s * SLOT + M::STASH, ln);
+        if constexpr (STASH) y = s == 0 ? load_state<N>(tr + (long long)t * N) : load_stage(sl + s * SLOT + SS::TAPE, ln);
         else y = s == 0 ? load_state<N>(tr + (long long)t * N) : (s == 1 ? y2 : (s == 2 ? y3 : y4));
         const f32x4 us = p.no_cost ? load_u<MI>(up, t) : clamp_u4<MI>(p.c, load_u<MI>(up, t));
         f32x4 in = ((s == 0 || s == 3) ? p.sixth_dt : 2.0f * p.sixth_dt) * lam;
diff --git a/phnn_mpc_amd/csrc/phnn_mpc.hip b/phnn_mpc_amd/csrc/phnn_mpc.hip
--- a/phnn_mpc_amd/csrc/phnn_mpc.hip
+++ b/phnn_mpc_amd/csrc/phnn_mpc.hip
@@ -33,8 +33,8 @@
 KernelSet make_set(const char* name) {
   KernelSet k;
   fill_fwd<M>(k.fwd);
-  k.stash_floats[0] = StashStep<M, PHNN_INTEG_EULER>::FLOATS;
-  k.stash_floats[1] = StashStep<M, PHNN_INTEG_RK4>::FLOATS;
+  k.stash_floats[0] = StashStep<M, PHNN_INTEG_EULER, TAPE_MPC>::FLOATS;
+  k.stash_floats[1] = StashStep<M, PHNN_INTEG_RK4, TAPE_MPC>::FLOATS;
   k.scr_floats = M::SCR;
   k.mfwd = k_model_forward<M>;
   k.img_floats = M::IMG;
@@ -447,9 +447,13 @@
 }
 
 int launch_roll(phnn_handle* h, bool grad, bool ref, bool stash, int integrator, const RollParams& p, long long tiles,
-                hipStream_t st) {
-  if (!use_split(h, tiles)) return launch(h, (grad ? h->ks.grad : h->ks.fwd)[ref][stash][integrator], p, tiles, false, st);
-  RollKernel kern = (grad ? h->sp.grad : h->sp.fwd)[ref][stash][integrator];
+                hipStream_t st, bool train_tape = false) {
+  train_tape = train_tape && h->has_wgrad && h->wg.fwd_t[integrator];
+  if (!use_split(h, tiles)) {
+    RollKernel whole = train_tape ? h->wg.fwd_t[integrator] : (grad ? h->ks.grad : h->ks.fwd)[ref][stash][integrator];
+    return launch(h, whole, p, tiles, false, st);
+  }
+  RollKernel kern = train_tape ? h->sp.fwd_t[integrator] : (grad ? h->sp.grad : h->sp.fwd)[ref][stash][integrator];
   hipLaunchKernelGGL(kern, dim3((unsigned)tiles), dim3(256), sizeof(float) * (size_t)h->sp.lds_floats, st, p);
   hipError_t e = hipGetLastError();
   if (e != hipSuccess) return hip_fail(h, e, "kernel launch (split-tile)");
@@ -590,6 +594,12 @@
     if (e == hipSuccess) e = allow_big_lds(h->wg.grad_t[0]);
     if (e == hipSuccess) e = allow_big_lds(h->wg.grad_t[1]);
     if (e == hipSuccess) e = allow_big_lds(h->wg.reduce_t);
+    if (e == hipSuccess) e = allow_big_lds(h->wg.fwd_t[0]);
+    if (e == hipSuccess) e = allow_big_lds(h->wg.fwd_t[1]);
+  }
+  if (h->has_split) {
+    if (e == hipSuccess) e = allow_big_lds(h->sp.fwd_t[0]);
+    if (e == hipSuccess) e = allow_big_lds(h->sp.fwd_t[1]);
   }
   if (h->has_split && (size_t)h->sp.lds_floats * sizeof(float) > 160 * 1024) h->has_split = false;
   if (e != hipSuccess) {
@@ -913,7 +923,7 @@
   const long long tiles = (B + kTileB - 1) / kTileB;
   const bool tapes = wgrad_workspace_dev != nullptr;
   if (tapes) p.stash = (float*)wgrad_workspace_dev + wgrad_tape_offset(h, wgrad_records(B, H, integrator));
-  return launch_roll(h, false, false, tapes, integrator, p, tiles, (hipStream_t)stream);
+  return launch_roll(h, false, false, tapes, integrator, p, tiles, (hipStream_t)stream, tapes);
 }
 
 int phnn_rollout_wgrad(phnn_handle* h, const float* x0_dev, const float* u_dev, int64_t B, int32_t H, int32_t integrator,
diff --git a/phnn_mpc_amd/csrc/phnn_pack.h b/phnn_mpc_amd/csrc/phnn_pack.h
--- a/phnn_mpc_amd/csrc/phnn_pack.h
+++ b/phnn_mpc_amd/csrc/phnn_pack.h
@@ -126,7 +126,7 @@
 }
 
 template <int HID, int MM, bool FOLD = true>
-PK_HD const float* pack_h2(float* dst, const float* p, int nin, float* red) {
+PK_HD const float* pack_h2(float* dst, const float* p, int nin, float* red, float* ssb = nullptr) {
   using Y = LayH2<HID, MM>;
   const float* W1 = p; p += (size_t)HID * nin;
   const float* b1 = p; p += HID;
@@ -165,6 +165,7 @@
     dst[Y::oW3B + k] = W3[k] * Sb;
     dst[Y::oW3S + k] = W3[k] * Sb / S;
   }
+  if (ssb) *ssb = S * Sb;
   pack_cols_as_rows(dst + Y::oW1T, W1, HID, nin, Y::LR, S * Sb);
   PK_FOR(k, 1) {
     dst[Y::oB3] = b3[0];
@@ -173,6 +174,28 @@
     dst[Y::oB3 + 3] = Sb;
   }
   return p;
+}
+
+template <int HID>
+PK_HD void pack_curv(float* dst, const float* W1, int nin, float ssb, float* red) {
+  using I = CurvImg<HID>;
+  auto pval = [&](int row, int u) {
+    int i = 0, r = row;
+    while (r >= 4 - i) { r -= 4 - i; ++i; }
+    const int j = i + r;
+    return j < nin ? W1[(size_t)u * nin + i] * W1[(size_t)u * nin + j] : 0.f;
+  };
+  const float pmx = pk_max(10 * HID, red, [&](int e) { return __builtin_fabsf(pval(e / HID, e % HID)); });
+  const float Sp = pk_pow2_scale(pmx, true);
+  _Float16* pw = reinterpret_cast<_Float16*>(dst);
+  PK_FOR(e, 10 * HID) {
+    const int row = e / HID, pos = e % HID;
+    const float x = pval(row, pk_unit_of_pos(pos)) * Sp;
+    const _Float16 h = (_Float16)x, l = (_Float16)(x - (float)h);
+    pw[(size_t)row * I::RS + pos] = h;
+    pw[(size_t)I::PART / 2 + (size_t)row * I::RS + pos] = l;
+  }
+  PK_FOR(k, 1) dst[I::oConst] = -2.0f / (ssb * Sp);
 }
 
 template <int HID, int MM, bool FOLD = true>
@@ -226,7 +249,10 @@
     if (d->fixed_G) { G = p; p += N * MI; }
     constexpr bool FOLD = ACT == ACT_TANH;
     p = pack_h1<HID, MM, FOLD>(img + M::oR, p, N, N * N, red);
-    p = pack_h2<HID, MM, FOLD>(img + M::oH, p, N, red);
+    const float* W1h = p;
+    float ssb = 1.0f;
+    p = pack_h2<HID, MM, FOLD>(img + M::oH, p, N, red, &ssb);
+    if constexpr (M::CURV) pack_curv<HID>(img + M::oP, W1h, N, ssb, red);
     if (!d->fixed_G) p = pack_h1<HID, MM, FOLD>(img + M::oGn, p, N, N * MI, red);
     PK_FOR(e, N * N) {
       const int i = e / N, j = e % N;
@@ -284,7 +310,10 @@
       pack_in_frag_T<64>(dm + LayM::oWoTf, Wo, nout);
       pack_cols_as_rows(dm + LayM::oW1T, W1, 64, 2, LayM::LR);
     }
-    p = pack_h2<HID, MM, ACT == ACT_TANH>(img + M::oH, p, 4, red);
+    const float* W1h = p;
+    float ssb = 1.0f;
+    p = pack_h2<HID, MM, ACT == ACT_TANH>(img + M::oH, p, 4, red, &ssb);
+    if constexpr (M::CURV) pack_curv<HID>(img + M::oP, W1h, 4, ssb, red);
     PK_FOR(i, 4) {
       c[4 + i] = pk_softplus(Rd[i]) + 1e-4f;
       c[8 + i] = Rd[i] > 20.f ? 1.0f : (float)(1.0 / (1.0 + exp(-(double)Rd[i])));
diff --git a/phnn_mpc_amd/csrc/phnn_split.hip b/phnn_mpc_amd/csrc/phnn_split.hip
--- a/phnn_mpc_amd/csrc/phnn_split.hip
+++ b/phnn_mpc_amd/csrc/phnn_split.hip
@@ -6,6 +6,7 @@
   SplitSet g;
   fill_fwd<M>(g.fwd);
   fill_grad<M>(g.grad);
+  fill_fwd_train<M>(g.fwd_t);
   g.lds_floats = M::IMG + 4 * M::SCR + kXchFloats;
   return g;
 }
diff --git a/phnn_mpc_amd/csrc/phnn_variants.h b/phnn_mpc_amd/csrc/phnn_variants.h
--- a/phnn_mpc_amd/csrc/phnn_variants.h
+++ b/phnn_mpc_amd/csrc/phnn_variants.h
@@ -111,14 +111,23 @@
 
 template <class M>
 void fill_fwd(RollTable t) {
-  t[0][0][0] = k_rollout_fwd<M, PHNN_INTEG_EULER, false>;
-  t[0][0][1] = k_rollout_fwd<M, PHNN_INTEG_RK4, false>;
-  t[0][1][0] = k_rollout_fwd<M, PHNN_INTEG_EULER, true>;
-  t[0][1][1] = k_rollout_fwd<M, PHNN_INTEG_RK4, true>;
-  t[1][0][0] = k_rollout_fwd<M, PHNN_INTEG_EULER, false, true>;
-  t[1][0][1] = k_rollout_fwd<M, PHNN_INTEG_RK4, false, true>;
-  t[1][1][0] = k_rollout_fwd<M, PHNN_INTEG_EULER, true, true>;
-  t[1][1][1] = k_rollout_fwd<M, PHNN_INTEG_RK4, true, true>;
+  t[0][0][0] = k_rollout_fwd<M, PHNN_INTEG_EULER, TAPE_NONE>;
+  t[0][0][1] = k_rollout_fwd<M, PHNN_INTEG_RK4, TAPE_NONE>;
+  t[0][1][0] = k_rollout_fwd<M, PHNN_INTEG_EULER, TAPE_MPC>;
+  t[0][1][1] = k_rollout_fwd<M, PHNN_INTEG_RK4, TAPE_MPC>;
+  t[1][0][0] = k_rollout_fwd<M, PHNN_INTEG_EULER, TAPE_NONE, true>;
+  t[1][0][1] = k_rollout_fwd<M, PHNN_INTEG_RK4, TAPE_NONE, true>;
+  t[1][1][0] = k_rollout_fwd<M, PHNN_INTEG_EULER, TAPE_MPC, true>;
+  t[1][1][1] = k_rollout_fwd<M, PHNN_INTEG_RK4, TAPE_MPC, true>;
+}
+
+template <class M>
+void fill_fwd_train(RollKernel (&t)[2]) {
+  t[0] = t[1] = nullptr;
+  if constexpr (M::CURV) {
+    t[0] = k_rollout_fwd<M, PHNN_INTEG_EULER, TAPE_TRAIN>;
+    t[1] = k_rollout_fwd<M, PHNN_INTEG_RK4, TAPE_TRAIN>;
+  }
 }
 
 template <class M>
@@ -142,6 +151,7 @@
 
 struct SplitSet {
   RollTable fwd, grad;
+  RollKernel fwd_t[2];
   int lds_floats;
 };
 bool phnn_split_kernels(int variant, SplitSet* g);
@@ -149,6 +159,7 @@
 struct WgradSet {
   void (*grad[2])(RollParams);
   void (*grad_t[2])(RollParams);
+  RollKernel fwd_t[2];
   void (*mvjp)(PointParams);
   void (*reduce)(WgradParams);
   void (*reduce_t)(WgradParams);
diff --git a/phnn_mpc_amd/csrc/phnn_wgrad.hip b/phnn_mpc_amd/csrc/phnn_wgrad.hip
--- a/phnn_mpc_amd/csrc/phnn_wgrad.hip
+++ b/phnn_mpc_amd/csrc/phnn_wgrad.hip
@@ -12,8 +12,9 @@
   g.mvjp = k_model_vjp<M, true>;
   g.reduce = k_wgrad_reduce<M, false>;
   g.reduce_t = k_wgrad_reduce<M, true>;
-  g.tape_floats[0] = StashStep<M, PHNN_INTEG_EULER>::FLOATS;
-  g.tape_floats[1] = StashStep<M, PHNN_INTEG_RK4>::SLOT;
+  fill_fwd_train<M>(g.fwd_t);
+  g.tape_floats[0] = StashStep<M, PHNN_INTEG_EULER, TAPE_TRAIN>::FLOATS;
+  g.tape_floats[1] = StashStep<M, PHNN_INTEG_RK4, TAPE_TRAIN>::SLOT;
   g.rec_floats = M::Rec::SIZE;
   g.blob_floats = BlobOf<M>::SIZE;
   g.reduce_waves = M::T;
```
